# zuds-survey/zuds-pipeline

Hardware: AMD Instinct MI355X
Metric: Mpix/s resample->coadd->subtract, 3072x3072 frames (higher is better)
Workload: dtype f32; 1 GPU; configs[1]+[2]: 32x 3072x3072 TPV frames/GPU, mesh background + weight rescale + Lanczos-3 resample + WEIGHTED coadd (+ AND mask coadd, int16 masks); then 1 science frame/GPU: align ref, hotpants 3x3 regions x 10x10 stamps, r=10, ko=4, subtract; frames_per_gpu=32, size=3072, mask_dtype=int16, combine=WEIGHTED, subtract=True

## Files before the change

include/zudsmi.h:

```cpp
#ifndef ZUDSMI_H
#define ZUDSMI_H

#include <stdint.h>

#ifdef __cplusplus
extern "C" {
#endif

typedef struct zm_ctx zm_ctx;

#define ZM_NPV 40

typedef struct zm_wcs {
    double crpix[2];
    double crval[2];
    double cd[4];
    double pv1[ZM_NPV];
    double pv2[ZM_NPV];
    int32_t naxis[2];
    int32_t flags;
    int32_t pad_;
} zm_wcs;

enum { ZM_RESAMPLE_NEAREST = 0, ZM_RESAMPLE_BILINEAR = 1, ZM_RESAMPLE_LANCZOS3 = 3 };
// ... 42 lines not shown
    const float* img;
    const float* wgt;
    const void* mask;
    zm_wcs wcs;
    double flxscale;
    int32_t mask_type;
    int32_t pad_;
} zm_frame;

typedef struct zm_coadd_params {
    int32_t combine;
    int32_t mask_combine;
    int32_t resample;
    int32_t subtract_back;
    int32_t back_size;
    int32_t back_filtersize;
    int32_t rescale_weights;
    int32_t pad_;
    double clip_sigma;
    double clip_ampfrac;
    double weight_thresh;
} zm_coadd_params;

void zm_coadd_params_default(zm_coadd_params* p);

int zm_coadd(zm_ctx* ctx, int nframes, const zm_frame* frames,
             const zm_wcs* wout, const zm_coadd_params* params, float* out_img,
             float* out_wgt, int32_t* out_mask, float* out_mask_wgt);

typedef struct zm_hp_params {
    double tu, tl, iu, il;
    double r;
    double rss;
    double fin;
    double fi;
    int32_t nsx, nsy;
    int32_t nrx, nry;
    int32_t ko, bgo;
    int32_t nss;
    int32_t normalize;
    double ft;
    double ks;
    int32_t ngauss;
    int32_t deg[4];
    int32_t pad_[3];
    double sigma[4];
    const double* limits_dev;
    double limits_nsigma;
    int32_t* flag_mask_dev;
    int32_t flag_bit;
    int32_t async_info;
} zm_hp_params;

void zm_hp_params_default(zm_hp_params* p);

typedef struct zm_hp_info {
    int32_t nstamps_total, nstamps_used;
    int32_t niter, ncoeff;
    double kernel_sum;
    double chi2;
    int32_t nmasked;
    int32_t status;
    int32_t nunsolved;
    int32_t retries;
} zm_hp_info;
#define ZM_HP_UNSOLVED 1
#define ZM_HP_TIMEOUT 2
#define ZM_HP_PENDING 4

int zm_subtract(zm_ctx* ctx, const float* sci, const float* sci_rms,
                const float* ref, const float* ref_rms, const uint8_t* bpm,
                int nx, int ny, const zm_hp_params* params, float* out_diff,
                float* out_rms, zm_hp_info* out_info);

int zm_median_mad(zm_ctx* ctx, const float* img, const int32_t* mask, int64_t n,
                  double* out_median, double* out_mad_sigma);
int zm_median_mad_dev(zm_ctx* ctx, const float* img, const int32_t* mask,
                      int64_t n, double* out_median, double* out_mad_sigma);
int zm_median_mad2_dev(zm_ctx* ctx, const float* img_a, const int32_t* mask_a,
                       const float* img_b, const int32_t* mask_b, int64_t n,
                       double* out4);
int zm_median_mad2_async_dev(zm_ctx* ctx, const float* img_a, const int32_t* mask_a,
                             const float* img_b, const int32_t* mask_b, int64_t n, double* out6_dev);

int zm_aperture_photometry(zm_ctx* ctx, const float* img, const float* rms,
                           const int32_t* mask, int nx, int ny, int npos,
                           const double* x, const double* y, double radius,
                           double* out_flux, double* out_err, int32_t* out_flags);
int zm_aperture_photometry_dev(zm_ctx* ctx, const float* img, const float* rms,
                               const int32_t* mask, int nx, int ny, int npos,
                               const double* x, const double* y, double radius,
                               double* out_flux, double* out_err, int32_t* out_flags);

typedef struct zm_dframe {
    const float* img;
    const float* wgt;
    const void* mask;
    zm_wcs wcs;
    double flxscale;
    int32_t mask_type;
    int32_t pad_;
} zm_dframe;

int zm_coadd_dev(zm_ctx* ctx, int nframes, const zm_dframe* frames,
                 const zm_wcs* wout, const zm_coadd_params* params,
                 int partial, float* out_img, float* out_wgt, int32_t* out_mask,
                 float* out_mask_wgt);
int zm_coadd_finalize_dev(zm_ctx* ctx, float* s1_to_img, const float* s0,
                          int64_t npix);
int zm_mask_accum_dev(zm_ctx* ctx, int32_t* acc, const int32_t* m, int64_t npix,
                      int kind, int first);
int zm_mask_finalize_dev(zm_ctx* ctx, int32_t* acc, float* cov, int64_t npix);
#define ZM_COMM_ID_BYTES 128
typedef struct zm_comm zm_comm;
int zm_comm_unique_id(void* id128);
int zm_comm_init(zm_ctx* ctx, int nranks, int rank, const void* id128, zm_comm** out);
int zm_comm_destroy(zm_comm* comm);
int zm_coadd_reduce_dev(zm_ctx* ctx, zm_comm* comm, float* s1s0, int64_t npix);
int zm_mask_reduce_dev(zm_ctx* ctx, zm_comm* comm, int32_t* mask, int nx, int ny, int kind,
                       float* cov);
#define ZM_COMM_MAX_RANKS 64
typedef struct {
    int32_t world, rank;
    int64_t band_px;
    int64_t my_px;
    int64_t send_off[ZM_COMM_MAX_RANKS];
    int64_t send_cnt[ZM_COMM_MAX_RANKS];
    int64_t recv_off[ZM_COMM_MAX_RANKS];
    int64_t recv_cnt[ZM_COMM_MAX_RANKS];
    int64_t gather_off[ZM_COMM_MAX_RANKS];
} zm_mask_plan;
int zm_comm_band_bounds(int nrows, int world, int32_t* bounds);
int zm_comm_mask_plan(int nx, int ny, int world, int rank, zm_mask_plan* plan);
int zm_resample_stack_dev(zm_ctx* ctx, int nframes, const zm_dframe* frames,
                          const zm_wcs* wout, const zm_coadd_params* params,
                          float* stack, int32_t* out_mask_partial);
int zm_combine_stack_dev(zm_ctx* ctx, int nframes, const float* stack,
                         int64_t frame_stride_px, int64_t npix,
                         const zm_coadd_params* params, float* out_img,
                         float* out_wgt);
int zm_subtract_dev(zm_ctx* ctx, const float* sci, const float* sci_rms,
                    const float* ref, const float* ref_rms, const uint8_t* bpm,
                    int nx, int ny, const zm_hp_params* params, float* out_diff,
                    float* out_rms, zm_hp_info* out_info_host);
int zm_subtract_info(zm_ctx* ctx, zm_hp_info* out_info);
#define ZM_SUB_BATCH_MAX 64
typedef struct zm_sub_job {
    const float* sci;
    const float* sci_rms;
    const float* ref;
    const float* ref_rms;
    const uint8_t* bpm;
    const zm_hp_params* params;
    float* out_diff;
    float* out_rms;
} zm_sub_job;
int zm_subtract_batch_dev(zm_ctx* ctx, int njobs, const zm_sub_job* jobs, int nx, int ny,
                          zm_hp_info* out_info_host);
int zm_subtract_batch(zm_ctx* ctx, int njobs, const zm_sub_job* jobs, int nx, int ny,
                      zm_hp_info* out_info);
int zm_background_dev(zm_ctx* ctx, const float* img, const float* wgt, int nx,
                      int ny, int mesh, int filtersize, float* out_bkg,
                      float* out_rms, float* out_sub, double* out_stats_host);
int zm_resample_dev(zm_ctx* ctx, const float* img, const float* wgt,
                    const int32_t* mask, const zm_wcs* win, const zm_wcs* wout,
                    int kernel, double fscale, float* out_img, float* out_wgt,
                    int32_t* out_mask);

int zm_align_pair_dev(zm_ctx* ctx, const float* img_a, const float* img_b, const int32_t* mask,
                      const zm_wcs* win, const zm_wcs* wout, int kernel, double fscale_a, double fscale_b,
                      float* out_a, float* out_b, int32_t* out_mask);
int zm_resample_i16(zm_ctx* ctx, const float* img, const float* wgt,
                    const int16_t* mask, const zm_wcs* win, const zm_wcs* wout,
                    int kernel, double fscale, float* out_img, float* out_wgt,
                    int32_t* out_mask);
int zm_resample_i16_dev(zm_ctx* ctx, const float* img, const float* wgt,
                        const int16_t* mask, const zm_wcs* win, const zm_wcs* wout,
                        int kernel, double fscale, float* out_img, float* out_wgt,
                        int32_t* out_mask);
int zm_mask_widen_dev(zm_ctx* ctx, const int16_t* in, int64_t n, int32_t* out);

int zm_rms_from_weight_dev(zm_ctx* ctx, const float* wgt, const uint8_t* bad,
                           int64_t n, float big_rms, float* out);
int zm_weight_from_rms_dev(zm_ctx* ctx, const float* rms, const uint8_t* bad,
                           const float* img, float satur, int64_t n, float* out);
int zm_false_weight_dev(zm_ctx* ctx, const void* mask, int mask_type, int32_t badsum, int border,
                        int nx, int ny, float* out_wgt, uint8_t* out_bpm);
int zm_mask_bad_dev(zm_ctx* ctx, const int32_t* a, const int32_t* b,
                    int32_t badsum, int64_t n, int32_t* out_or, uint8_t* out_bpm);
int zm_mask_flag_dev(zm_ctx* ctx, int32_t* mask, const float* img, float value,
                     int32_t bit, int64_t n);
int zm_add_scalar_dev(zm_ctx* ctx, float* img, float v, int64_t n);
int zm_copy_probe_dev(zm_ctx* ctx, const void* src, void* dst, int64_t nbytes);

int zm_find_stars(zm_ctx* ctx, const float* img, const uint8_t* bad, int nx, int ny,
                  float thresh_lo, float thresh_hi, int isolation, int border,
                  int max_out, int* out_x, int* out_y, float* out_peak, int* out_n);
int zm_star_fwhm(zm_ctx* ctx, const float* img, int nx, int ny, int nstar,
                 const int* x, const int* y, int half, double* out_fwhm,
                 double* out_cx, double* out_cy);
int zm_negpix_test(zm_ctx* ctx, const float* img, int nx, int ny, int npos,
                   const double* x, const double* y, double median, double sigma,
                   int32_t* out_bad);
int zm_find_stars_dev(zm_ctx* ctx, const float* img, const uint8_t* bad, int nx, int ny,
                      float thresh_lo, float thresh_hi, int isolation, int border,
                      int max_out, int* out_x, int* out_y, float* out_peak, int* out_n);
int zm_star_fwhm_dev(zm_ctx* ctx, const float* img, int nx, int ny, int nstar,
                     const int* x, const int* y, int half, double* out_fwhm,
                     double* out_cx, double* out_cy);
int zm_candidate_cuts_dev(zm_ctx* ctx, const float* d_img, const float* d_rms, const int32_t* d_mask,
                          int32_t bad_bits, int nx, int ny, int npos, const double* x, const double* y,
                          double* out_bpmcut, double* out_rmscut, int32_t* out_negpix, double* out_stats);

typedef struct zm_extract_params {
    float detect_thresh;
    float satur_level;
    int32_t detect_minarea;
    int32_t filter;
    double aper_radius;
} zm_extract_params;
void zm_extract_params_default(zm_extract_params* p);

#define ZM_EXTRACT_CHAIN 1

typedef struct zm_object {
    int32_t number;
    int32_t npix;
    int32_t xmin, xmax, ymin, ymax;
    int32_t flags;
    int32_t flags_weight;
    int32_t imaflags_iso;
    int32_t first;
    int32_t nthresh;
    int32_t pad_;
    double x_image, y_image;
    double x2, y2, xy;
    double a_image, b_image, theta_image, elongation;
    double fwhm_image;
    double flux_iso, flux_max;
    double peak;
    double flux_aper, fluxerr_aper;
    double x_world, y_world;
} zm_object;

int zm_extract_dev(zm_ctx* ctx, const float* img, const float* sigma, const uint8_t* bad,
                   const int32_t* flag, int nx, int ny, const zm_wcs* wcs,
                   const zm_extract_params* params, int max_objects, zm_object* out_rows,
                   int32_t* segm_dev, float* filtered_dev, int* out_nwritten, int* out_nfound,
                   int* out_status);
int zm_extract(zm_ctx* ctx, const float* img, const float* sigma, const uint8_t* bad,
               const int32_t* flag, int nx, int ny, const zm_wcs* wcs,
               const zm_extract_params* params, int max_objects, zm_object* out_rows,
               int32_t* out_segm, float* out_filtered, int* out_nwritten, int* out_nfound,
               int* out_status);

typedef struct zm_measure_params {
    double kron_fact;
    double kron_min_radius;
    int32_t filter;
    int32_t pad_;
} zm_measure_params;
void zm_measure_params_default(zm_measure_params* p);

#define ZM_AUTO_SKIPPED 1
#define ZM_AUTO_OFFFRAME 2
#define ZM_AUTO_MINRADIUS 4
#define ZM_WIN_FALLBACK 1
#define ZM_WIN_NOTCONVERGED 2

typedef struct zm_object_ext {
    int32_t number;
    int32_t npix_auto;
// ... 60 lines not shown
```

zuds-pipeline_amd/_lib.py:

```python
import ctypes as C
from pathlib import Path

import numpy as np

HERE = Path(__file__).resolve().parent
LIBPATH = HERE / 'lib' / 'libzudsmi.so'

NPV = 40

RESAMPLE = {'NEAREST': 0, 'BILINEAR': 1, 'LANCZOS3': 3}
COMBINE = {'WEIGHTED': 0, 'MEDIAN': 1, 'CLIPPED': 2, 'AVERAGE': 3}
MASKCOMB = {'AND': 0, 'OR': 1}


class ZMError(RuntimeError):
    """A libzudsmi call returned non-zero (message from zm_last_error)."""


class zm_wcs(C.Structure):
    _fields_ = [('crpix', C.c_double * 2), ('crval', C.c_double * 2),
                ('cd', C.c_double * 4), ('pv1', C.c_double * NPV),
                ('pv2', C.c_double * NPV), ('naxis', C.c_int32 * 2),
                ('flags', C.c_int32), ('pad_', C.c_int32)]

# ... 51 lines not shown


COMM_MAX_RANKS = 64


class zm_mask_plan(C.Structure):
    _fields_ = [('world', C.c_int32), ('rank', C.c_int32), ('band_px', C.c_int64), ('my_px', C.c_int64),
                ('send_off', C.c_int64 * COMM_MAX_RANKS), ('send_cnt', C.c_int64 * COMM_MAX_RANKS),
                ('recv_off', C.c_int64 * COMM_MAX_RANKS), ('recv_cnt', C.c_int64 * COMM_MAX_RANKS),
                ('gather_off', C.c_int64 * COMM_MAX_RANKS)]


class zm_extract_params(C.Structure):
    _fields_ = [('detect_thresh', C.c_float), ('satur_level', C.c_float),
                ('detect_minarea', C.c_int32), ('filter', C.c_int32),
                ('aper_radius', C.c_double)]


class zm_object(C.Structure):
    _fields_ = [('number', C.c_int32), ('npix', C.c_int32), ('xmin', C.c_int32), ('xmax', C.c_int32),
                ('ymin', C.c_int32), ('ymax', C.c_int32), ('flags', C.c_int32), ('flags_weight', C.c_int32),
                ('imaflags_iso', C.c_int32), ('first', C.c_int32), ('nthresh', C.c_int32), ('pad_', C.c_int32),
                ('x_image', C.c_double), ('y_image', C.c_double), ('x2', C.c_double), ('y2', C.c_double),
                ('xy', C.c_double), ('a_image', C.c_double), ('b_image', C.c_double), ('theta_image', C.c_double),
                ('elongation', C.c_double), ('fwhm_image', C.c_double), ('flux_iso', C.c_double),
                ('flux_max', C.c_double), ('peak', C.c_double), ('flux_aper', C.c_double),
                ('fluxerr_aper', C.c_double), ('x_world', C.c_double), ('y_world', C.c_double)]


class zm_measure_params(C.Structure):
    _fields_ = [('kron_fact', C.c_double), ('kron_min_radius', C.c_double), ('filter', C.c_int32), ('pad_', C.c_int32)]


class zm_object_ext(C.Structure):
    _fields_ = [('number', C.c_int32), ('npix_auto', C.c_int32), ('nskip_auto', C.c_int32), ('flags_auto', C.c_int32),
                ('flags_win', C.c_int32), ('niter_win', C.c_int32),
                ('kron_radius', C.c_double), ('flux_auto', C.c_double), ('fluxerr_auto', C.c_double),
                ('mag_auto', C.c_double), ('magerr_auto', C.c_double), ('sigma_win', C.c_double),
                ('xwin_image', C.c_double), ('ywin_image', C.c_double),
                ('x2win', C.c_double), ('y2win', C.c_double), ('xywin', C.c_double),
                ('errx2win', C.c_double), ('erry2win', C.c_double), ('errxywin', C.c_double),
                ('awin_image', C.c_double), ('bwin_image', C.c_double), ('thetawin_image', C.c_double),
                ('errawin_image', C.c_double), ('errbwin_image', C.c_double), ('errthetawin_image', C.c_double),
                ('errx2', C.c_double), ('erry2', C.c_double), ('errxy', C.c_double),
                ('xwin_world', C.c_double), ('ywin_world', C.c_double),
                ('erra_world', C.c_double), ('errb_world', C.c_double), ('errtheta_world', C.c_double)]


class zm_stamp_plane(C.Structure):
    _fields_ = [('img', C.c_void_p), ('wcs', zm_wcs), ('fscale', C.c_double),
                ('on_grid', C.c_int32), ('pad_', C.c_int32)]


STAMP_MAX, STAMP_PLANES_MAX = 256, 8
STAMP_NOT_FINITE, STAMP_NO_OVERLAP = 1, 2
EXTRACT_CHAIN = 1
HP_UNSOLVED, HP_TIMEOUT, HP_PENDING = 1, 2, 4


_P = C.c_void_p
_SIGS = {
    'zm_ctx_create': (C.c_int, [C.c_int, C.POINTER(_P)]),
    'zm_ctx_destroy': (C.c_int, [_P]),
    'zm_ctx_set_stream': (C.c_int, [_P, _P]),
    'zm_ctx_synchronize': (C.c_int, [_P]),
    'zm_ctx_create_on_stream': (C.c_int, [C.c_int, _P, C.POINTER(C.c_void_p)]),
    'zm_ctx_set_share': (C.c_int, [_P, C.c_int]),
    'zm_ctx_query': (C.c_int, [_P, C.c_char_p, C.POINTER(C.c_int64)]),
    'zm_ctx_set_conventions': (C.c_int, [_P, C.c_int, C.c_int]),
    'zm_last_error': (C.c_char_p, []),
    'zm_version': (C.c_char_p, []),
    'zm_autogrid': (C.c_int, [C.c_int, C.POINTER(zm_wcs), C.POINTER(zm_wcs)]),
    'zm_wcs_pix2sky': (C.c_int, [C.POINTER(zm_wcs), C.c_int, _P, _P, _P, _P]),
    'zm_wcs_sky2pix': (C.c_int, [C.POINTER(zm_wcs), C.c_int, _P, _P, _P, _P]),
    'zm_wcs_map': (C.c_int, [C.POINTER(zm_wcs), C.POINTER(zm_wcs), C.c_int,
                             _P, _P, _P, _P]),
    'zm_flux_scale': (C.c_int, [C.POINTER(zm_wcs), C.POINTER(zm_wcs),
                                C.c_double, C.POINTER(C.c_double)]),
    'zm_resample': (C.c_int, [_P, _P, _P, _P, C.POINTER(zm_wcs),
                              C.POINTER(zm_wcs), C.c_int, C.c_double,
                              _P, _P, _P]),
    'zm_align_pair_dev': (C.c_int, [_P, _P, _P, _P, C.POINTER(zm_wcs), C.POINTER(zm_wcs), C.c_int, C.c_double,
                                    C.c_double, _P, _P, _P]),
    'zm_resample_dev': (C.c_int, [_P, _P, _P, _P, C.POINTER(zm_wcs),
                                  C.POINTER(zm_wcs), C.c_int, C.c_double,
                                  _P, _P, _P]),
    'zm_resample_i16': (C.c_int, [_P, _P, _P, _P, C.POINTER(zm_wcs),
                                  C.POINTER(zm_wcs), C.c_int, C.c_double,
                                  _P, _P, _P]),
    'zm_resample_i16_dev': (C.c_int, [_P, _P, _P, _P, C.POINTER(zm_wcs),
                                      C.POINTER(zm_wcs), C.c_int, C.c_double,
                                      _P, _P, _P]),
    'zm_mask_widen_dev': (C.c_int, [_P, _P, C.c_int64, _P]),
    'zm_coadd_params_default': (None, [C.POINTER(zm_coadd_params)]),
    'zm_coadd': (C.c_int, [_P, C.c_int, C.POINTER(zm_frame), C.POINTER(zm_wcs),
                           C.POINTER(zm_coadd_params), _P, _P, _P, _P]),
    'zm_coadd_dev': (C.c_int, [_P, C.c_int, C.POINTER(zm_frame),
                               C.POINTER(zm_wcs), C.POINTER(zm_coadd_params),
                               C.c_int, _P, _P, _P, _P]),
    'zm_coadd_finalize_dev': (C.c_int, [_P, _P, _P, C.c_int64]),
    'zm_resample_stack_dev': (C.c_int, [_P, C.c_int, C.POINTER(zm_frame),
                                        C.POINTER(zm_wcs),
                                        C.POINTER(zm_coadd_params), _P, _P]),
    'zm_combine_stack_dev': (C.c_int, [_P, C.c_int, _P, C.c_int64, C.c_int64,
                                       C.POINTER(zm_coadd_params), _P, _P]),
    'zm_background': (C.c_int, [_P, _P, _P, C.c_int, C.c_int, C.c_int, C.c_int,
                                _P, _P, _P, _P]),
    'zm_background_dev': (C.c_int, [_P, _P, _P, C.c_int, C.c_int, C.c_int,
                                    C.c_int, _P, _P, _P, _P]),
    'zm_hp_params_default': (None, [C.POINTER(zm_hp_params)]),
    'zm_subtract': (C.c_int, [_P, _P, _P, _P, _P, _P, C.c_int, C.c_int,
                              C.POINTER(zm_hp_params), _P, _P,
                              C.POINTER(zm_hp_info)]),
    'zm_subtract_dev': (C.c_int, [_P, _P, _P, _P, _P, _P, C.c_int, C.c_int,
                                  C.POINTER(zm_hp_params), _P, _P,
                                  C.POINTER(zm_hp_info)]),
    'zm_subtract_info': (C.c_int, [_P, C.POINTER(zm_hp_info)]),
    'zm_subtract_batch_dev': (C.c_int, [_P, C.c_int, C.POINTER(zm_sub_job), C.c_int, C.c_int,
                                        C.POINTER(zm_hp_info)]),
    'zm_subtract_batch': (C.c_int, [_P, C.c_int, C.POINTER(zm_sub_job), C.c_int, C.c_int,
                                    C.POINTER(zm_hp_info)]),
    'zm_median_mad': (C.c_int, [_P, _P, _P, C.c_int64, C.POINTER(C.c_double),
                                C.POINTER(C.c_double)]),
    'zm_median_mad_dev': (C.c_int, [_P, _P, _P, C.c_int64, C.POINTER(C.c_double),
                                    C.POINTER(C.c_double)]),
    'zm_find_stars': (C.c_int, [_P, _P, _P, C.c_int, C.c_int, C.c_float, C.c_float, C.c_int, C.c_int,
                                C.c_int, _P, _P, _P, C.POINTER(C.c_int)]),
    'zm_star_fwhm': (C.c_int, [_P, _P, C.c_int, C.c_int, C.c_int, _P, _P, C.c_int, _P, _P, _P]),
    'zm_find_stars_dev': (C.c_int, [_P, _P, _P, C.c_int, C.c_int, C.c_float, C.c_float, C.c_int, C.c_int,
                                    C.c_int, _P, _P, _P, C.POINTER(C.c_int)]),
    'zm_star_fwhm_dev': (C.c_int, [_P, _P, C.c_int, C.c_int, C.c_int, _P, _P, C.c_int, _P, _P, _P]),
    'zm_negpix_test': (C.c_int, [_P, _P, C.c_int, C.c_int, C.c_int, _P, _P, C.c_double, C.c_double, _P]),
    'zm_candidate_cuts_dev': (C.c_int, [_P, _P, _P, _P, C.c_int32, C.c_int, C.c_int, C.c_int, _P, _P, _P, _P, _P, _P]),
    'zm_fits_decode_dev': (C.c_int, [_P, _P, C.c_int, C.c_double, C.c_double, C.c_int64, C.c_int, _P]),
    'zm_fits_encode_dev': (C.c_int, [_P, _P, C.c_int, C.c_int64, _P]),
    'zm_mask_accum_dev': (C.c_int, [_P, _P, _P, C.c_int64, C.c_int, C.c_int]),
    'zm_mask_finalize_dev': (C.c_int, [_P, _P, _P, C.c_int64]),
    'zm_comm_unique_id': (C.c_int, [_P]),
    'zm_comm_init': (C.c_int, [_P, C.c_int, C.c_int, _P, C.POINTER(C.c_void_p)]),
    'zm_comm_destroy': (C.c_int, [_P]),
    'zm_coadd_reduce_dev': (C.c_int, [_P, _P, _P, C.c_int64]),
    'zm_mask_reduce_dev': (C.c_int, [_P, _P, _P, C.c_int, C.c_int, C.c_int, _P]),
    'zm_comm_band_bounds': (C.c_int, [C.c_int, C.c_int, _P]),
    'zm_comm_mask_plan': (C.c_int, [C.c_int, C.c_int, C.c_int, C.c_int, C.POINTER(zm_mask_plan)]),
    'zm_median_mad2_dev': (C.c_int, [_P, _P, _P, _P, _P, C.c_int64, C.POINTER(C.c_double)]),
    'zm_median_mad2_async_dev': (C.c_int, [_P, _P, _P, _P, _P, C.c_int64, _P]),
    'zm_rms_from_weight_dev': (C.c_int, [_P, _P, _P, C.c_int64, C.c_float, _P]),
    'zm_weight_from_rms_dev': (C.c_int, [_P, _P, _P, _P, C.c_float, C.c_int64, _P]),
    'zm_false_weight_dev': (C.c_int, [_P, _P, C.c_int, C.c_int32, C.c_int, C.c_int, C.c_int, _P, _P]),
    'zm_mask_bad_dev': (C.c_int, [_P, _P, _P, C.c_int32, C.c_int64, _P, _P]),
    'zm_mask_flag_dev': (C.c_int, [_P, _P, _P, C.c_float, C.c_int32, C.c_int64]),
    'zm_add_scalar_dev': (C.c_int, [_P, _P, C.c_float, C.c_int64]),
    'zm_copy_probe_dev': (C.c_int, [_P, _P, _P, C.c_int64]),
    'zm_aperture_photometry': (C.c_int, [_P, _P, _P, _P, C.c_int, C.c_int, C.c_int, _P, _P,
                                         C.c_double, _P, _P, _P]),
    'zm_aperture_photometry_dev': (C.c_int, [_P, _P, _P, _P, C.c_int, C.c_int, C.c_int, _P, _P,
                                             C.c_double, _P, _P, _P]),
    'zm_extract_params_default': (None, [C.POINTER(zm_extract_params)]),
    'zm_extract_dev': (C.c_int, [_P, _P, _P, _P, _P, C.c_int, C.c_int, C.POINTER(zm_wcs), C.POINTER(zm_extract_params),
                                 C.c_int, _P, _P, _P, C.POINTER(C.c_int), C.POINTER(C.c_int), C.POINTER(C.c_int)]),
    'zm_extract': (C.c_int, [_P, _P, _P, _P, _P, C.c_int, C.c_int, C.POINTER(zm_wcs), C.POINTER(zm_extract_params),
                             C.c_int, _P, _P, _P, C.POINTER(C.c_int), C.POINTER(C.c_int), C.POINTER(C.c_int)]),
    'zm_measure_params_default': (None, [C.POINTER(zm_measure_params)]),
    'zm_extract_measure_dev': (C.c_int, [_P, _P, _P, _P, _P, C.c_int, C.c_int, C.POINTER(zm_wcs),
                                         C.POINTER(zm_measure_params), C.c_int, _P, _P]),
    'zm_extract_measure': (C.c_int, [_P, _P, _P, _P, _P, C.c_int, C.c_int, C.POINTER(zm_wcs),
                                     C.POINTER(zm_measure_params), C.c_int, _P, _P]),
    'zm_stamp_origin': (C.c_int, [C.POINTER(zm_wcs), C.c_int, _P, _P, C.c_int, _P, _P, _P]),
    'zm_stamps_dev': (C.c_int, [_P, C.c_int, C.POINTER(zm_stamp_plane), C.POINTER(zm_wcs), C.c_int, C.c_int, _P, _P,
                                C.c_int, _P, _P]),
    'zm_stamps': (C.c_int, [_P, C.c_int, C.POINTER(zm_stamp_plane), C.POINTER(zm_wcs), C.c_int, C.c_int, _P, _P,
                            C.c_int, _P, _P]),
    'zm_timing_enable': (C.c_int, [_P, C.c_int]),
    'zm_timing_filter': (C.c_int, [_P, C.c_char_p]),
    'zm_timing_reset': (C.c_int, [_P]),
    'zm_timing_read': (C.c_int, [_P, C.c_char_p, C.POINTER(C.c_double),
                                 C.POINTER(C.c_int64)]),
    'zm_debug_lanczos3': (None, [C.c_float, _P]),
}

_lib = None


def exported_symbols():
    return [k for k in _SIGS if k != 'zm_debug_lanczos3']


def _one_hip_runtime():
    import importlib.util
    import os
    import sys
    if 'torch' in sys.modules:
        return
    try:
        spec = importlib.util.find_spec('torch')
    except (ImportError, ValueError):
        spec = None
    if not spec or not spec.origin:
        return
    if not os.environ.get('ZM_NO_TORCH'):
        try:
            import torch
            return
        except Exception:
            pass
    d = os.path.join(os.path.dirname(spec.origin), 'lib')
    for name in ('libhsa-runtime64.so', 'libamdhip64.so'):
        p = os.path.join(d, name)
        if os.path.exists(p):
            try:
                C.CDLL(p, mode=C.RTLD_GLOBAL)
            except OSError:
                return


def lib():
    global _lib
    if _lib is not None:
        return _lib
    _one_hip_runtime()
    if not LIBPATH.exists():
        raise ZMError(f'{LIBPATH} is missing: run __graft_entry__.build() '
                      f'(python zuds-pipeline_amd/build.py). There is no CPU '
                      f'fallback for this path.')
    L = C.CDLL(str(LIBPATH))
    for name, (res, args) in _SIGS.items():
        try:
            fn = getattr(L, name)
        except AttributeError:
            raise ZMError(f'{LIBPATH} does not export {name}; rebuild it '
                          f'(python zuds-pipeline_amd/build.py --force)')
        fn.restype = res
        fn.argtypes = args
# ... 54 lines not shown
```

zuds-pipeline_amd/csrc/api_coadd.hip:

```cpp
#include <algorithm>
#include <cmath>
#include <cstdlib>

#include "zm_internal.h"
#include "wcs_math.h"

extern "C" void zm_coadd_params_default(zm_coadd_params* p) {
    if (!p) return;
    memset(p, 0, sizeof(*p));
    p->combine = ZM_COMBINE_CLIPPED;
    p->mask_combine = ZM_MASK_AND;
    p->resample = ZM_RESAMPLE_LANCZOS3;
    p->subtract_back = 1;
    p->back_size = 128;
    p->back_filtersize = 3;
    p->rescale_weights = 1;
    p->clip_sigma = 4.0;
    p->clip_ampfrac = 0.3;
    p->weight_thresh = 1e-30;
}

static int check_wcs(const zm_wcs* w, const char* what) {
    ZM_CHECK(w != nullptr, "%s: WCS is NULL", what);
    ZM_CHECK(w->naxis[0] > 0 && w->naxis[1] > 0, "%s: NAXIS must be positive (got %d x %d)", what,
// ... 372 lines not shown
                                    const zm_coadd_params* params, float* out_img,
                                    float* out_wgt) {
    ZM_CHECK(ctx && stack && params && out_img && out_wgt, "zm_combine_stack_dev: null argument");
    ZM_HIP(hipSetDevice(ctx->device));
    return zm_launch_combine(ctx, nframes, (const float2*)stack, frame_stride_px, npix,
                             params->combine, (float)params->clip_sigma,
                             (float)params->clip_ampfrac, out_img, out_wgt, 0);
}

extern "C" int zm_coadd_dev(zm_ctx* ctx, int nframes, const zm_dframe* frames,
                            const zm_wcs* wout, const zm_coadd_params* params, int partial,
                            float* out_img, float* out_wgt, int32_t* out_mask,
                            float* out_mask_wgt) {
    ZM_CHECK(ctx && frames && wout && params && out_img && out_wgt, "zm_coadd_dev: null argument");
    ZM_CHECK(nframes >= 1, "zm_coadd_dev: need at least one frame");
    ZM_HIP(hipSetDevice(ctx->device));
    ZM_TRY(check_wcs(wout, "output grid"));
    const int64_t opix = (int64_t)wout->naxis[0] * wout->naxis[1];
    if (fused_ok(ctx, params))
        return coadd_fused(ctx, nframes, frames, wout, params, partial, out_img, out_wgt, out_mask, out_mask_wgt);
    float2* stack = nullptr;
    ZM_TRY(ctx->get("stack", sizeof(float2) * (size_t)opix * nframes, (void**)&stack));
    ZM_TRY(resample_frames(ctx, nframes, frames, wout, params, stack, out_mask, -1,
                           params->mask_combine));
    ZM_TRY(zm_launch_combine(ctx, nframes, stack, opix, opix, params->combine,
                             (float)params->clip_sigma, (float)params->clip_ampfrac, out_img,
                             out_wgt, partial));
    if (out_mask && !partial) ZM_TRY(zm_launch_mask_finalize(ctx, out_mask, out_mask_wgt, opix));
    return 0;
}

extern "C" int zm_mask_accum_dev(zm_ctx* ctx, int32_t* acc, const int32_t* m, int64_t npix, int kind,
                                 int first) {
    ZM_CHECK(ctx && acc && m, "zm_mask_accum_dev: null argument");
    ZM_CHECK(kind == ZM_MASK_AND || kind == ZM_MASK_OR, "zm_mask_accum_dev: unknown combine %d", kind);
    ZM_HIP(hipSetDevice(ctx->device));
    return zm_launch_mask_accum(ctx, acc, m, npix, kind, first);
}

extern "C" int zm_mask_finalize_dev(zm_ctx* ctx, int32_t* acc, float* cov, int64_t npix) {
    ZM_CHECK(ctx && acc, "zm_mask_finalize_dev: null argument");
    ZM_HIP(hipSetDevice(ctx->device));
    return zm_launch_mask_finalize(ctx, acc, cov, npix);
}

extern "C" int zm_resample_dev(zm_ctx* ctx, const float* img, const float* wgt,
                               const int32_t* mask, const zm_wcs* win, const zm_wcs* wout,
                               int kernel, double fscale, float* out_img, float* out_wgt,
                               int32_t* out_mask) {
    ZM_CHECK(ctx && win && wout, "zm_resample_dev: null argument");
    ZM_CHECK(img || mask, "zm_resample_dev: need an image or a mask");
    ZM_CHECK(!img || (out_img && out_wgt), "zm_resample_dev: out_img/out_wgt required");
    ZM_CHECK(!mask || out_mask, "zm_resample_dev: out_mask required");
    ZM_HIP(hipSetDevice(ctx->device));
    ZM_TRY(check_wcs(win, "input frame"));
    ZM_TRY(check_wcs(wout, "output grid"));
    ZM_CHECK(kernel == ZM_RESAMPLE_LANCZOS3 || kernel == ZM_RESAMPLE_BILINEAR ||
             kernel == ZM_RESAMPLE_NEAREST, "zm_resample_dev: unknown RESAMPLING_TYPE %d", kernel);
    const int onx = wout->naxis[0], ony = wout->naxis[1];
    const int nx = win->naxis[0], ny = win->naxis[1];
    const int64_t opix = (int64_t)onx * ony;
    const int lnx = (onx - 1) / ZM_LATTICE_STEP + 2, lny = (ony - 1) / ZM_LATTICE_STEP + 2;
    zm_map_params mp_host;
    zm_make_map(wout, win, &mp_host);
    int lds = std::min(plan_lds(&mp_host, onx, ony, ntaps_of(kernel)), 8000);
    double2* lat = nullptr;
    ZM_TRY(ctx->get("lattice", sizeof(double2) * (size_t)lnx * lny, (void**)&lat));
    ZM_TRY(zm_launch_lattice(ctx, &mp_host, lnx, lny, lat));
    if (img) {
        const int spitch = (nx + 1) & ~1;
        float2 *src = nullptr, *dst = nullptr;
        ZM_TRY(ctx->get("prep", sizeof(float2) * (size_t)spitch * ny, (void**)&src));
        ZM_TRY(ctx->get("stack", sizeof(float2) * (size_t)opix, (void**)&dst));
        ZM_TRY(zm_launch_prep(ctx, img, wgt, nx, ny, nullptr, 0, 0, 0, nullptr, 1e-30f, src, spitch));
        ZM_TRY(zm_launch_resample(ctx, src, nx, ny, spitch, lat, lnx, lny, kernel, (float)fscale,
                                  dst, onx, ony, lds, mask, out_mask, mask ? 1 : 0, 0, 1, out_img, out_wgt));
    } else if (mask) {
        ZM_TRY(zm_launch_resample_mask(ctx, mask, nx, ny, lat, lnx, lny, kernel, out_mask, onx,
                                       ony, 0));
    }
    return 0;
}

extern "C" int zm_align_pair_dev(zm_ctx* ctx, const float* img_a, const float* img_b, const int32_t* mask,
                                 const zm_wcs* win, const zm_wcs* wout, int kernel, double fscale_a, double fscale_b,
                                 float* out_a, float* out_b, int32_t* out_mask) {
    ZM_CHECK(ctx && img_a && img_b && win && wout && out_a && out_b, "zm_align_pair_dev: null argument");
    ZM_CHECK(!mask || out_mask, "zm_align_pair_dev: out_mask required");
    ZM_CHECK(kernel == ZM_RESAMPLE_LANCZOS3 || kernel == ZM_RESAMPLE_BILINEAR, "zm_align_pair_dev: LANCZOS3 or BILINEAR (got %d)", kernel);
    ZM_CHECK(fscale_b != 0.0, "zm_align_pair_dev: fscale_b must not be 0");
    ZM_CHECK(ctx->edge == ZM_EDGE_ZERO && ctx->mask_resample == ZM_MASKRES_OR, "zm_align_pair_dev: default conventions only");
    ZM_HIP(hipSetDevice(ctx->device));
    ZM_TRY(check_wcs(win, "input frame"));
    ZM_TRY(check_wcs(wout, "output grid"));
    const int onx = wout->naxis[0], ony = wout->naxis[1];
    const int nx = win->naxis[0], ny = win->naxis[1];
    const int lnx = (onx - 1) / ZM_LATTICE_STEP + 2, lny = (ony - 1) / ZM_LATTICE_STEP + 2;
    zm_map_params mp_host;
    zm_make_map(wout, win, &mp_host);
    const int lds = std::min(plan_lds(&mp_host, onx, ony, ntaps_of(kernel)), 8000);
    double2* lat = nullptr;
    ZM_TRY(ctx->get("lattice", sizeof(double2) * (size_t)lnx * lny, (void**)&lat));
    ZM_TRY(zm_launch_lattice(ctx, &mp_host, lnx, lny, lat));
    const int spitch = (nx + 1) & ~1;
    float2* src = nullptr;
    ZM_TRY(ctx->get("prep", sizeof(float2) * (size_t)spitch * ny, (void**)&src));
    ZM_TRY(zm_launch_prep_pair(ctx, img_a, img_b, nx, ny, src, spitch));
    return zm_launch_resample(ctx, src, nx, ny, spitch, lat, lnx, lny, kernel, (float)fscale_a, nullptr, onx, ony, lds,
                              mask, out_mask, mask ? 1 : 0, 0, 1, out_a, out_b, (float)fscale_b);
}

extern "C" int zm_resample_i16_dev(zm_ctx* ctx, const float* img, const float* wgt, const int16_t* mask,
                                   const zm_wcs* win, const zm_wcs* wout, int kernel, double fscale,
                                   float* out_img, float* out_wgt, int32_t* out_mask) {
    ZM_CHECK(ctx && win && wout, "zm_resample_i16_dev: null argument");
    ZM_HIP(hipSetDevice(ctx->device));
    int32_t* w = nullptr;
    if (mask) {
        ZM_TRY(check_wcs(win, "input frame"));
        const int64_t n = (int64_t)win->naxis[0] * win->naxis[1];
        ZM_TRY(ctx->get("mask_widen", sizeof(int32_t) * (size_t)n, (void**)&w));
        ZM_TRY(zm_launch_mask_widen(ctx, mask, n, w));
    }
    return zm_resample_dev(ctx, img, wgt, w, win, wout, kernel, fscale, out_img, out_wgt, out_mask);
}

static int resample_host(zm_ctx* ctx, const float* img, const float* wgt, const void* mask, int mask_type,
                         const zm_wcs* win, const zm_wcs* wout, int kernel, double fscale,
                         float* out_img, float* out_wgt, int32_t* out_mask);
extern "C" int zm_resample(zm_ctx* ctx, const float* img, const float* wgt, const int32_t* mask,
                           const zm_wcs* win, const zm_wcs* wout, int kernel, double fscale,
                           float* out_img, float* out_wgt, int32_t* out_mask) {
    return resample_host(ctx, img, wgt, mask, ZM_MASKTYPE_I32, win, wout, kernel, fscale, out_img, out_wgt, out_mask);
}
extern "C" int zm_resample_i16(zm_ctx* ctx, const float* img, const float* wgt, const int16_t* mask,
                               const zm_wcs* win, const zm_wcs* wout, int kernel, double fscale,
                               float* out_img, float* out_wgt, int32_t* out_mask) {
    return resample_host(ctx, img, wgt, mask, ZM_MASKTYPE_I16, win, wout, kernel, fscale, out_img, out_wgt, out_mask);
}
static int resample_host(zm_ctx* ctx, const float* img, const float* wgt, const void* mask, int mask_type,
                         const zm_wcs* win, const zm_wcs* wout, int kernel, double fscale,
                         float* out_img, float* out_wgt, int32_t* out_mask) {
    ZM_CHECK(ctx && win && wout, "zm_resample: null argument");
    ZM_HIP(hipSetDevice(ctx->device));
    ZM_TRY(check_wcs(win, "input frame"));
    ZM_TRY(check_wcs(wout, "output grid"));
    const size_t ipix = (size_t)win->naxis[0] * win->naxis[1];
    const size_t opix = (size_t)wout->naxis[0] * wout->naxis[1];
    const size_t mb = mask_type == ZM_MASKTYPE_I16 ? 2 : 4;
    float *d_img = nullptr, *d_wgt = nullptr, *d_oimg = nullptr, *d_owgt = nullptr;
    void* d_mask = nullptr;
    int32_t* d_omask = nullptr;
    if (img) {
        ZM_TRY(ctx->get("h_img", ipix * 4, (void**)&d_img));
        ZM_HIP(hipMemcpyAsync(d_img, img, ipix * 4, hipMemcpyHostToDevice, ctx->stream));
        if (wgt) {
            ZM_TRY(ctx->get("h_wgt", ipix * 4, (void**)&d_wgt));
            ZM_HIP(hipMemcpyAsync(d_wgt, wgt, ipix * 4, hipMemcpyHostToDevice, ctx->stream));
        }
        ZM_TRY(ctx->get("h_oimg", opix * 4, (void**)&d_oimg));
        ZM_TRY(ctx->get("h_owgt", opix * 4, (void**)&d_owgt));
    }
    if (mask) {
        ZM_TRY(ctx->get("h_mask", ipix * mb, &d_mask));
        ZM_HIP(hipMemcpyAsync(d_mask, mask, ipix * mb, hipMemcpyHostToDevice, ctx->stream));
        ZM_TRY(ctx->get("h_omask", opix * 4, (void**)&d_omask));
    }
    if (mask_type == ZM_MASKTYPE_I16)
        ZM_TRY(zm_resample_i16_dev(ctx, d_img, d_wgt, (const int16_t*)d_mask, win, wout, kernel, fscale, d_oimg,
                                   d_owgt, d_omask));
    else
        ZM_TRY(zm_resample_dev(ctx, d_img, d_wgt, (const int32_t*)d_mask, win, wout, kernel, fscale, d_oimg, d_owgt,
                               d_omask));
    if (img) {
        ZM_HIP(hipMemcpyAsync(out_img, d_oimg, opix * 4, hipMemcpyDeviceToHost, ctx->stream));
        ZM_HIP(hipMemcpyAsync(out_wgt, d_owgt, opix * 4, hipMemcpyDeviceToHost, ctx->stream));
    }
    if (mask)
        ZM_HIP(hipMemcpyAsync(out_mask, d_omask, opix * 4, hipMemcpyDeviceToHost, ctx->stream));
    ZM_HIP(hipStreamSynchronize(ctx->stream));
    return 0;
}

extern "C" int zm_coadd(zm_ctx* ctx, int nframes, const zm_frame* frames, const zm_wcs* wout,
                        const zm_coadd_params* params, float* out_img, float* out_wgt,
                        int32_t* out_mask, float* out_mask_wgt) {
    ZM_CHECK(ctx && frames && wout && params && out_img && out_wgt, "zm_coadd: null argument");
    ZM_CHECK(nframes >= 1, "zm_coadd: need at least one frame");
    ZM_HIP(hipSetDevice(ctx->device));
    ZM_TRY(check_wcs(wout, "output grid"));
    std::vector<zm_dframe> df(nframes);
    size_t total = 0;
// ... 55 lines not shown
```

zuds-pipeline_amd/csrc/api_subtract.hip:

```cpp
#include "select_dev.h"

#define RS_BINS 2048

struct rs_state {
    uint32_t prefix[2];
    uint32_t pmask;
    uint32_t pad_;
    unsigned long long k[2];
    unsigned long long count;
    float centre;
    float median;
    double out[3];
};

__global__ void k_rsel_init(rs_state* __restrict__ st, unsigned int* __restrict__ hist) {
    const int im = blockIdx.x;
    for (int k = threadIdx.x; k < 2 * RS_BINS; k += blockDim.x) hist[(size_t)im * 2 * RS_BINS + k] = 0;
    if (threadIdx.x == 0) {
        rs_state z;
        memset(&z, 0, sizeof(z));
        st[im] = z;
    }
}

__global__ __launch_bounds__(1024) void k_rsel_hist(const rs_batch B, int vec_ok, int mode, int shift,
                                                    int nbins, const rs_state* __restrict__ st,
                                                    unsigned int* __restrict__ hist,
                                                    unsigned long long* __restrict__ vbits, int vmode) {
    __shared__ unsigned int lh[2][RS_BINS];
    const int im = blockIdx.y;
    const float* __restrict__ img = B.im[im].img;
    const int32_t* __restrict__ mask = B.im[im].mask;
    const rs_state S = st[im];
    const bool two = S.prefix[1] != S.prefix[0];
    for (int k = threadIdx.x; k < nbins; k += blockDim.x) { lh[0][k] = 0; lh[1][k] = 0; }
    __syncthreads();
    int cur = -1;
    unsigned int run = 0;
    auto put = [&](float v, int32_t m) {
        if (m != 0 || !(v == v)) return;
        if (mode == 1) v = fabsf(v - S.centre);
        const uint32_t key = f2key(v);
        const uint32_t hi = key & S.pmask;
        const int b = (int)((key >> shift) & (uint32_t)(nbins - 1));
        if (hi == S.prefix[0]) {
            if (b == cur) { ++run; }
            else {
                if (run) atomicAdd(&lh[0][cur], run);
                cur = b;
                run = 1;
            }
        } else if (two && hi == S.prefix[1]) {
            atomicAdd(&lh[1][b], 1u);
        }
    };
    const int64_t n = B.n;
    const int64_t n4 = vec_ok ? n / 4 : 0;
    const int64_t stride = (int64_t)gridDim.x * blockDim.x;
    unsigned long long* vb = vbits ? vbits + (size_t)im * (size_t)((n4 + 63) / 64) * 4 : nullptr;
    const int lane = threadIdx.x & 63;
    const int64_t n4w = vb ? ((n4 + 63) / 64) * 64 : n4;
    for (int64_t q = (int64_t)blockIdx.x * blockDim.x + threadIdx.x; q < n4w; q += stride) {
        const bool in = q < n4;
        float4 v = make_float4(0.f, 0.f, 0.f, 0.f);
        if (in) v = reinterpret_cast<const float4*>(img)[q];
        int4 m = make_int4(0, 0, 0, 0);
        if (vb && vmode == 2) {
            const unsigned long long* w = vb + (q >> 6) * 4;
            m.x = ((w[0] >> lane) & 1ull) ? 0 : 1;
            m.y = ((w[1] >> lane) & 1ull) ? 0 : 1;
            m.z = ((w[2] >> lane) & 1ull) ? 0 : 1;
            m.w = ((w[3] >> lane) & 1ull) ? 0 : 1;
        } else {
            if (mask && in) m = reinterpret_cast<const int4*>(mask)[q];
            if (!in) m = make_int4(1, 1, 1, 1);
            if (vb) {
                const unsigned long long b0 = __ballot(m.x == 0 && v.x == v.x), b1 = __ballot(m.y == 0 && v.y == v.y);
                const unsigned long long b2 = __ballot(m.z == 0 && v.z == v.z), b3 = __ballot(m.w == 0 && v.w == v.w);
                if (lane == 0) {
                    unsigned long long* w = vb + (q >> 6) * 4;
                    w[0] = b0; w[1] = b1; w[2] = b2; w[3] = b3;
                }
            }
        }
        put(v.x, m.x); put(v.y, m.y); put(v.z, m.z); put(v.w, m.w);
    }
    for (int64_t p = 4 * n4 + (int64_t)blockIdx.x * blockDim.x + threadIdx.x; p < n; p += stride)
        put(img[p], mask ? mask[p] : 0);
    if (run) atomicAdd(&lh[0][cur], run);
    __syncthreads();
    unsigned int* h = hist + (size_t)im * 2 * RS_BINS;
    for (int k = threadIdx.x; k < nbins; k += blockDim.x) {
        if (lh[0][k]) atomicAdd(&h[k], lh[0][k]);
        if (two && lh[1][k]) atomicAdd(&h[RS_BINS + k], lh[1][k]);
    }
}

__global__ __launch_bounds__(256) void k_rsel_scan(int pass, int mode, int shift, int nbins,
                                                   rs_state* __restrict__ st,
                                                   unsigned int* __restrict__ hist) {
    __shared__ unsigned long long wtot[4];
    __shared__ rs_state S;
    const int im = blockIdx.x, tid = threadIdx.x;
    const int lane = tid & 63, wave = tid >> 6;
    unsigned int* h = hist + (size_t)im * 2 * RS_BINS;
    if (tid == 0) S = st[im];
    __syncthreads();
    const bool two = S.prefix[1] != S.prefix[0];
    const int per = nbins / 256;
    for (int t = 0; t < 2; ++t) {
        const unsigned int* ht = h + (two && t == 1 ? RS_BINS : 0);
        unsigned int hl[8];
        unsigned long long loc = 0;
#pragma unroll
        for (int j = 0; j < 8; ++j) {
            hl[j] = j < per ? ht[tid * per + j] : 0u;
            loc += hl[j];
        }
        unsigned long long inc = loc;
#pragma unroll
        for (int o = 1; o < 64; o <<= 1) {
            const unsigned long long up = __shfl_up(inc, o);
            if (lane >= o) inc += up;
        }
        if (lane == 63) wtot[wave] = inc;
        __syncthreads();
        unsigned long long off = 0, tot = 0;
#pragma unroll
        for (int w = 0; w < 4; ++w) {
            if (w < wave) off += wtot[w];
            tot += wtot[w];
        }
        const unsigned long long excl = off + inc - loc;
        if (pass == 0 && t == 0 && tid == 0) {
            S.count = tot;
            S.k[0] = tot ? (tot - 1) / 2 : 0;
            S.k[1] = tot / 2 < tot ? tot / 2 : (tot ? tot - 1 : 0);
        }
        __syncthreads();
        const unsigned long long k = S.k[t];
        __syncthreads();
        const bool hit = (tid == 255) ? (k >= excl) : (k >= excl && k < excl + loc);
        if (hit) {
            unsigned long long runsum = excl;
            int jsel = per - 1;
            bool found = false;
#pragma unroll
            for (int j = 0; j < 7; ++j)
                if (!found && j < per - 1) {
                    if (runsum + hl[j] > k) { jsel = j; found = true; }
                    else runsum += hl[j];
                }
            S.k[t] = k - runsum;
            S.prefix[t] |= (uint32_t)(tid * per + jsel) << shift;
        }
        __syncthreads();
    }
    for (int k = tid; k < 2 * RS_BINS; k += 256) h[k] = 0;
    if (tid == 0) {
        S.pmask |= (uint32_t)(nbins - 1) << shift;
        if (pass == 2) {
            const float a = key2f_dev(S.prefix[0]), b = key2f_dev(S.prefix[1]);
            const float med = S.count ? 0.5f * (a + b) : 0.f;
            if (mode == 0) {
                S.median = med;
                S.centre = med;
                S.out[0] = med;
                S.out[2] = (double)S.count;
            } else {
                S.out[1] = 1.4826 * (double)med;
            }
// ... 4 lines not shown
        st[im] = S;
    }
}

__global__ void k_rsel_out(const rs_state* __restrict__ st, int nimg, double* __restrict__ out) {
    const int t = threadIdx.x;
    if (t < 3 * nimg) out[t] = st[t / 3].out[t % 3];
}

static int median_mad_batch(zm_ctx* ctx, int nimg, const rs_image* ims, int64_t n, double* out3, double* out_dev = nullptr) {
    ZM_CHECK(nimg >= 1 && nimg <= ZM_RS_MAXIMG, "median_mad_batch: 1..%d images", ZM_RS_MAXIMG);
    rs_state* d_st = nullptr;
    unsigned int* d_hist = nullptr;
    ZM_TRY(ctx->get("rs_state", sizeof(rs_state) * ZM_RS_MAXIMG, (void**)&d_st));
    ZM_TRY(ctx->get("rs_hist", sizeof(unsigned int) * 2 * RS_BINS * ZM_RS_MAXIMG, (void**)&d_hist));
    unsigned long long* d_vbits = nullptr;
    rs_batch B;
    memset(&B, 0, sizeof(B));
    B.n = n;
    int vec_ok = 1;
    for (int i = 0; i < nimg; ++i) {
        B.im[i] = ims[i];
        if (((uintptr_t)ims[i].img & 15) || ((uintptr_t)ims[i].mask & 15)) vec_ok = 0;
    }
    static const int rs_threads = ZM_DEVENV("ZM_RS_THREADS") ? atoi(ZM_DEVENV("ZM_RS_THREADS")) : 1024;
    static const int rs_grid = ZM_DEVENV("ZM_RS_GRID") ? atoi(ZM_DEVENV("ZM_RS_GRID")) : 256;
    int grid = (int)std::min<int64_t>((n / 4 + rs_threads - 1) / rs_threads, rs_grid);
    if (grid < 1) grid = 1;
    bool any_mask = false;
    for (int i = 0; i < nimg; ++i) any_mask = any_mask || ims[i].mask != nullptr;
    static const bool bits_off = ZM_DEVENV("ZM_RS_BITS") && ZM_DEVENV("ZM_RS_BITS")[0] == '0';
    if (vec_ok && any_mask && n >= 4096 && !bits_off)
        ZM_TRY(ctx->get("rs_vbits", sizeof(unsigned long long) * 4 * (size_t)((n / 4 + 63) / 64) * ZM_RS_MAXIMG, (void**)&d_vbits));
    const int shifts[3] = {21, 10, 0}, bits[3] = {11, 11, 10};
    hipStream_t s = ctx->stream;
    static const bool classic = ZM_DEVENV("ZM_RS_CLASSIC") && ZM_DEVENV("ZM_RS_CLASSIC")[0] == '1';
    if (vec_ok && n >= ZM_RS2_MIN_N && !classic) {
        double* d_out = out_dev;
        if (!d_out) ZM_TRY(ctx->get("rs2_out", sizeof(double) * 3 * ZM_RS_MAXIMG, (void**)&d_out));
        {
            zm_scope_timer t(ctx, "median_mad");
            ZM_TRY(zm_rs2_median_mad(ctx, nimg, B, d_vbits, d_out));
        }
        if (!out3) return 0;
        double* h_out = nullptr;
        ZM_TRY(ctx->get_pinned("rs2_out_h", sizeof(double) * 3 * ZM_RS_MAXIMG, (void**)&h_out));
        ZM_HIP(hipMemcpyAsync(h_out, d_out, sizeof(double) * 3 * nimg, hipMemcpyDeviceToHost, s));
        ZM_HIP(hipStreamSynchronize(s));
        for (int k = 0; k < 3 * nimg; ++k) out3[k] = h_out[k];
        return 0;
    }
    {
        zm_scope_timer t(ctx, "median_mad");
        hipLaunchKernelGGL(k_rsel_init, dim3(nimg), dim3(256), 0, s, d_st, d_hist);
        for (int mode = 0; mode < 2; ++mode)
            for (int pass = 0; pass < 3; ++pass) {
                const int nb = 1 << bits[pass];
                hipLaunchKernelGGL(k_rsel_hist, dim3(grid, nimg), dim3(rs_threads), 0, s, B, vec_ok, mode,
                                   shifts[pass], nb, d_st, d_hist, d_vbits, (mode == 0 && pass == 0) ? 1 : 2);
                hipLaunchKernelGGL(k_rsel_scan, dim3(nimg), dim3(256), 0, s, pass, mode, shifts[pass], nb,
                                   d_st, d_hist);
            }
        ZM_HIP(hipGetLastError());
    }
    if (!out3) {
        hipLaunchKernelGGL(k_rsel_out, dim3(1), dim3(64), 0, s, d_st, nimg, out_dev);
        ZM_HIP(hipGetLastError());
        return 0;
    }
    rs_state* h_st = nullptr;
    ZM_TRY(ctx->get_pinned("rs_state_h", sizeof(rs_state) * ZM_RS_MAXIMG, (void**)&h_st));
    ZM_HIP(hipMemcpyAsync(h_st, d_st, sizeof(rs_state) * nimg, hipMemcpyDeviceToHost, s));
    ZM_HIP(hipStreamSynchronize(s));
    for (int i = 0; i < nimg; ++i)
        for (int k = 0; k < 3; ++k) out3[3 * i + k] = h_st[i].out[k];
    return 0;
}

extern "C" int zm_median_mad_dev(zm_ctx* ctx, const float* img, const int32_t* mask, int64_t n,
                                 double* out_median, double* out_mad_sigma) {
    ZM_CHECK(ctx && img && out_median && out_mad_sigma, "zm_median_mad_dev: null argument");
    ZM_CHECK(n > 0, "zm_median_mad_dev: empty image");
    ZM_HIP(hipSetDevice(ctx->device));
    rs_image im = {img, mask};
    double o[3];
    ZM_TRY(median_mad_batch(ctx, 1, &im, n, o));
    ZM_CHECK(o[2] > 0, "zm_median_mad: every pixel is masked");
    *out_median = o[0];
    *out_mad_sigma = o[1];
    return 0;
}

extern "C" int zm_median_mad2_dev(zm_ctx* ctx, const float* img_a, const int32_t* mask_a,
                                  const float* img_b, const int32_t* mask_b, int64_t n,
                                  double* out4) {
    ZM_CHECK(ctx && img_a && img_b && out4, "zm_median_mad2_dev: null argument");
    ZM_CHECK(n > 0, "zm_median_mad2_dev: empty image");
    ZM_HIP(hipSetDevice(ctx->device));
    rs_image im[2] = {{img_a, mask_a}, {img_b, mask_b}};
    double o[6];
    ZM_TRY(median_mad_batch(ctx, 2, im, n, o));
    ZM_CHECK(o[2] > 0 && o[5] > 0, "zm_median_mad2: every pixel is masked");
    out4[0] = o[0]; out4[1] = o[1]; out4[2] = o[3]; out4[3] = o[4];
    return 0;
}

extern "C" int zm_median_mad2_async_dev(zm_ctx* ctx, const float* img_a, const int32_t* mask_a,
                                        const float* img_b, const int32_t* mask_b, int64_t n,
                                        double* out6_dev) {
    ZM_CHECK(ctx && img_a && img_b && out6_dev, "zm_median_mad2_async_dev: null argument");
    ZM_CHECK(n > 0, "zm_median_mad2_async_dev: empty image");
    ZM_HIP(hipSetDevice(ctx->device));
    rs_image im[2] = {{img_a, mask_a}, {img_b, mask_b}};
    return median_mad_batch(ctx, 2, im, n, nullptr, out6_dev);
}

extern "C" int zm_median_mad(zm_ctx* ctx, const float* img, const int32_t* mask, int64_t n,
                             double* out_median, double* out_mad_sigma) {
    ZM_CHECK(ctx && img && out_median && out_mad_sigma, "zm_median_mad: null argument");
    ZM_CHECK(n > 0, "zm_median_mad: empty image");
    ZM_HIP(hipSetDevice(ctx->device));
    float* d_img = nullptr;
    int32_t* d_mask = nullptr;
    ZM_TRY(ctx->get("h_img", (size_t)n * 4, (void**)&d_img));
    ZM_HIP(hipMemcpyAsync(d_img, img, (size_t)n * 4, hipMemcpyHostToDevice, ctx->stream));
    if (mask) {
        ZM_TRY(ctx->get("h_mask", (size_t)n * 4, (void**)&d_mask));
        ZM_HIP(hipMemcpyAsync(d_mask, mask, (size_t)n * 4, hipMemcpyHostToDevice, ctx->stream));
    }
    return zm_median_mad_dev(ctx, d_img, d_mask, n, out_median, out_mad_sigma);
}
```

zuds-pipeline_amd/csrc/elementwise.hip:

```cpp
#include <algorithm>
#include "zm_internal.h"

#define EW_GRID(n) dim3((unsigned)(((n) + 255) / 256)), dim3(256), 0, ctx->stream

__global__ void k_rms_from_weight(const float* __restrict__ w, const uint8_t* __restrict__ bad,
                                  int64_t n, float big, float* __restrict__ out) {
    int64_t p = (int64_t)blockIdx.x * blockDim.x + threadIdx.x;
    if (p >= n) return;
    float ww = w[p];
    bool b = !(ww > 0.f) || (bad && bad[p]);
    out[p] = b ? big : 1.0f / sqrtf(ww);
}

__global__ void k_weight_from_rms(const float* __restrict__ rms, const uint8_t* __restrict__ bad,
                                  const float* __restrict__ img, float satur, int64_t n,
                                  float* __restrict__ out) {
    int64_t p = (int64_t)blockIdx.x * blockDim.x + threadIdx.x;
    if (p >= n) return;
    float r = rms[p];
    bool b = (bad && bad[p]) || (img && satur > 0.f && img[p] >= satur);
    out[p] = b ? 0.f : 1.0f / (r * r);
}

template <typename T>
__global__ void k_false_weight(const T* __restrict__ m, int32_t badsum, int border, int nx, int ny,
                               float* __restrict__ out_w, uint8_t* __restrict__ out_bpm) {
    const int64_t p = (int64_t)blockIdx.x * blockDim.x + threadIdx.x;
    if (p >= (int64_t)nx * ny) return;
    const int y = (int)(p / nx), x = (int)(p - (int64_t)y * nx);
    const bool bad = ((int32_t)m[p] & badsum) != 0;
    const bool edge = x < border || x >= nx - border || y < border || y >= ny - border;
    if (out_w) out_w[p] = (bad || edge) ? 0.f : 1.f;
    if (out_bpm) out_bpm[p] = bad ? 1 : 0;
}

extern "C" int zm_false_weight_dev(zm_ctx* ctx, const void* mask, int mask_type, int32_t badsum, int border,
                                   int nx, int ny, float* out_wgt, uint8_t* out_bpm) {
    ZM_CHECK(ctx && mask && nx > 0 && ny > 0 && border >= 0 && (out_wgt || out_bpm), "zm_false_weight_dev: bad argument");
    ZM_CHECK(mask_type == ZM_MASKTYPE_I32 || mask_type == ZM_MASKTYPE_I16, "zm_false_weight_dev: unknown mask_type %d", mask_type);
    ZM_HIP(hipSetDevice(ctx->device));
    const int64_t n = (int64_t)nx * ny;
    if (mask_type == ZM_MASKTYPE_I16)
        hipLaunchKernelGGL(k_false_weight<int16_t>, EW_GRID(n), (const int16_t*)mask, badsum, border, nx, ny, out_wgt, out_bpm);
    else
        hipLaunchKernelGGL(k_false_weight<int32_t>, EW_GRID(n), (const int32_t*)mask, badsum, border, nx, ny, out_wgt, out_bpm);
    ZM_HIP(hipGetLastError());
    return 0;
}

__global__ void k_mask_bad(const int32_t* __restrict__ a, const int32_t* __restrict__ b,
                           int32_t badsum, int64_t n, int32_t* __restrict__ out_or,
                           uint8_t* __restrict__ out_bpm) {
    int64_t p = (int64_t)blockIdx.x * blockDim.x + threadIdx.x;
    if (p >= n) return;
    int32_t m = a[p] | (b ? b[p] : 0);
    if (out_or) out_or[p] = m;
    if (out_bpm) out_bpm[p] = (m & badsum) != 0;
}

__global__ void k_mask_flag(int32_t* __restrict__ mask, const float* __restrict__ img, float value,
                            int32_t bit, int64_t n) {
    int64_t p = (int64_t)blockIdx.x * blockDim.x + threadIdx.x;
    if (p >= n) return;
    if (img[p] == value) mask[p] |= bit;
}

__global__ void k_add_scalar(float* __restrict__ img, float v, int64_t n) {
    int64_t p = (int64_t)blockIdx.x * blockDim.x + threadIdx.x;
    if (p >= n) return;
    img[p] += v;
}

extern "C" int zm_rms_from_weight_dev(zm_ctx* ctx, const float* wgt, const uint8_t* bad, int64_t n,
                                      float big_rms, float* out) {
    ZM_CHECK(ctx && wgt && out && n > 0, "zm_rms_from_weight_dev: bad argument");
    ZM_HIP(hipSetDevice(ctx->device));
    hipLaunchKernelGGL(k_rms_from_weight, EW_GRID(n), wgt, bad, n, big_rms, out);
    ZM_HIP(hipGetLastError());
    return 0;
}

extern "C" int zm_weight_from_rms_dev(zm_ctx* ctx, const float* rms, const uint8_t* bad,
                                      const float* img, float satur, int64_t n, float* out) {
    ZM_CHECK(ctx && rms && out && n > 0, "zm_weight_from_rms_dev: bad argument");
    ZM_HIP(hipSetDevice(ctx->device));
    hipLaunchKernelGGL(k_weight_from_rms, EW_GRID(n), rms, bad, img, satur, n, out);
    ZM_HIP(hipGetLastError());
    return 0;
}

extern "C" int zm_mask_bad_dev(zm_ctx* ctx, const int32_t* a, const int32_t* b, int32_t badsum,
                               int64_t n, int32_t* out_or, uint8_t* out_bpm) {
    ZM_CHECK(ctx && a && n > 0 && (out_or || out_bpm), "zm_mask_bad_dev: bad argument");
    ZM_HIP(hipSetDevice(ctx->device));
    hipLaunchKernelGGL(k_mask_bad, EW_GRID(n), a, b, badsum, n, out_or, out_bpm);
    ZM_HIP(hipGetLastError());
    return 0;
}

extern "C" int zm_mask_flag_dev(zm_ctx* ctx, int32_t* mask, const float* img, float value,
                                int32_t bit, int64_t n) {
    ZM_CHECK(ctx && mask && img && n > 0, "zm_mask_flag_dev: bad argument");
    ZM_HIP(hipSetDevice(ctx->device));
    hipLaunchKernelGGL(k_mask_flag, EW_GRID(n), mask, img, value, bit, n);
    ZM_HIP(hipGetLastError());
    return 0;
}

template <int U, bool NTL>
__global__ __launch_bounds__(256) void k_copy4(const float4* __restrict__ src, float4* __restrict__ dst, int64_t n4) {
    typedef float v4f __attribute__((ext_vector_type(4)));
    const v4f* s = reinterpret_cast<const v4f*>(src);
    v4f* d = reinterpret_cast<v4f*>(dst);
    const int64_t nslab = n4 / (256 * U);
    for (int64_t b = blockIdx.x; b < nslab; b += gridDim.x) {
        const int64_t o = b * (256 * U) + threadIdx.x;
        v4f r[U];
#pragma unroll
        for (int u = 0; u < U; ++u) r[u] = NTL ? __builtin_nontemporal_load(s + o + 256 * u) : s[o + 256 * u];
#pragma unroll
        for (int u = 0; u < U; ++u) __builtin_nontemporal_store(r[u], d + o + 256 * u);
    }
    for (int64_t p = nslab * (256 * U) + (int64_t)blockIdx.x * blockDim.x + threadIdx.x; p < n4;
         p += (int64_t)gridDim.x * blockDim.x)
        d[p] = s[p];
}

extern "C" int zm_copy_probe_dev(zm_ctx* ctx, const void* src, void* dst, int64_t nbytes) {
    ZM_CHECK(ctx && src && dst && nbytes > 0 && nbytes % 16 == 0 && ((uintptr_t)src & 15) == 0 &&
             ((uintptr_t)dst & 15) == 0, "zm_copy_probe_dev: bad argument");
    ZM_HIP(hipSetDevice(ctx->device));
    int ncu = 256;
    ZM_HIP(hipDeviceGetAttribute(&ncu, hipDeviceAttributeMultiprocessorCount, ctx->device));
    const int64_t n4 = nbytes / 16;
    const unsigned grid = (unsigned)std::min<int64_t>((n4 + 255) / 256, (int64_t)ncu * 8);
    const char* cf = ZM_DEVENV("ZM_COPY_FORM");
    const int u = cf ? atoi(cf) : 4;
    const bool ntl = cf ? strchr(cf, 'n') != nullptr : true;
    if (u == 8 && ntl) hipLaunchKernelGGL((k_copy4<8, true>), dim3(grid), dim3(256), 0, ctx->stream, (const float4*)src, (float4*)dst, n4);
    else if (u == 8) hipLaunchKernelGGL((k_copy4<8, false>), dim3(grid), dim3(256), 0, ctx->stream, (const float4*)src, (float4*)dst, n4);
    else if (ntl) hipLaunchKernelGGL((k_copy4<4, true>), dim3(grid), dim3(256), 0, ctx->stream, (const float4*)src, (float4*)dst, n4);
    else hipLaunchKernelGGL((k_copy4<4, false>), dim3(grid), dim3(256), 0, ctx->stream, (const float4*)src, (float4*)dst, n4);
    ZM_HIP(hipGetLastError());
    return 0;
}

extern "C" int zm_add_scalar_dev(zm_ctx* ctx, float* img, float v, int64_t n) {
    ZM_CHECK(ctx && img && n > 0, "zm_add_scalar_dev: bad argument");
    ZM_HIP(hipSetDevice(ctx->device));
    hipLaunchKernelGGL(k_add_scalar, EW_GRID(n), img, v, n);
    ZM_HIP(hipGetLastError());
    return 0;
}

__global__ __launch_bounds__(256) void k_mask_widen(const int16_t* __restrict__ in, int64_t n, int32_t* __restrict__ out) {
    const int64_t stride = (int64_t)gridDim.x * blockDim.x * 4;
    for (int64_t p = ((int64_t)blockIdx.x * blockDim.x + threadIdx.x) * 4; p < n; p += stride) {
        if (p + 4 <= n && ((uintptr_t)in & 7) == 0 && ((uintptr_t)out & 15) == 0) {
            const short4 v = *reinterpret_cast<const short4*>(in + p);
            *reinterpret_cast<int4*>(out + p) = make_int4(v.x, v.y, v.z, v.w);
        } else {
            for (int64_t q = p; q < n && q < p + 4; ++q) out[q] = in[q];
        }
    }
}

int zm_launch_mask_widen(zm_ctx* ctx, const int16_t* in, int64_t n, int32_t* out) {
    int ncu = 256;
    ZM_HIP(hipDeviceGetAttribute(&ncu, hipDeviceAttributeMultiprocessorCount, ctx->device));
    const unsigned grid = (unsigned)std::max<int64_t>(1, std::min<int64_t>((n / 4 + 255) / 256, (int64_t)ncu * 8));
    hipLaunchKernelGGL(k_mask_widen, dim3(grid), dim3(256), 0, ctx->stream, in, n, out);
    ZM_HIP(hipGetLastError());
    return 0;
}

extern "C" int zm_mask_widen_dev(zm_ctx* ctx, const int16_t* in, int64_t n, int32_t* out) {
    ZM_CHECK(ctx && in && out && n > 0, "zm_mask_widen_dev: bad argument");
    ZM_HIP(hipSetDevice(ctx->device));
// ... 3 lines not shown
```

zuds-pipeline_amd/csrc/hotpants.hip:

```cpp
#include "hp_dev.h"
#include <sched.h>
#include "chol_diag.h"

__global__ void k_hp_valid(const float* __restrict__ sci, const float* __restrict__ ref,
                           const uint8_t* __restrict__ bpm, int64_t n, float il, float iu,
                           float tl, float tu, uint8_t* __restrict__ bad,
                           const double* __restrict__ lim, double nsig) {
    int64_t p = (int64_t)blockIdx.x * blockDim.x + threadIdx.x;
    if (lim) {
        il = (float)(lim[0] - nsig * lim[1]);
        tl = (float)(lim[3] - nsig * lim[4]);
    }
    if (p >= n) return;
    float s = sci[p], t = ref[p];
    bool ok = (s == s) && (t == t) && fabsf(s) < 3e38f && fabsf(t) < 3e38f;
    ok = ok && s >= il && s <= iu && t >= tl && t <= tu;
    if (bpm) ok = ok && bpm[p] == 0;
    bad[p] = ok ? 0 : 1;
}

#define HP_ROWMAX 16384
__global__ __launch_bounds__(256) void k_hp_rowany(const uint8_t* __restrict__ in, int nx, int ny, int hw,
                                                   uint8_t* __restrict__ out) {
    extern __shared__ int ra_pre[];
// ... 70 lines not shown
        int off = inc - v;
        for (int w = 0; w < wave; ++w) off += wtot[w];
        if (tid < 4 * nch) wsum[tid] = off;
    }
    __syncthreads();
    for (int c = 0; c < nch; ++c) {
        const int x = 256 * c + tid;
        if (x < nx) ra_pre[x + 1] += wsum[4 * c + wave];
    }
    __syncthreads();
    for (int x = tid; x < nx; x += 256) {
        const int a1 = max(x - hw1, 0), b1 = min(x + hw1, nx - 1);
        const int a2 = max(x - hw2, 0), b2 = min(x + hw2, nx - 1);
        out1[r0 + x] = (ra_pre[b1 + 1] - ra_pre[a1]) > 0;
        out2[r0 + x] = (ra_pre[b2 + 1] - ra_pre[a2]) > 0;
    }
}

#define HP_COLSTRIP 96
__global__ __launch_bounds__(256) void k_hp_colany(const uint8_t* __restrict__ in, int nx, int ny, int hw,
                                                   int edge, uint8_t* __restrict__ out) {
    const int x = blockIdx.x * blockDim.x + threadIdx.x;
    const int y0 = blockIdx.y * HP_COLSTRIP, y1 = min(y0 + HP_COLSTRIP, ny);
    if (x >= nx) return;
    int cnt = 0;
    for (int j = max(y0 - hw, 0); j <= min(y0 + hw, ny - 1); ++j) cnt += in[(size_t)j * nx + x] ? 1 : 0;
    for (int y = y0; y < y1; ++y) {
        uint8_t v = cnt > 0;
        if (edge && (x < hw || x >= nx - hw || y < hw || y >= ny - hw)) v = 1;
        out[(size_t)y * nx + x] = v;
        const int add = y + 1 + hw, sub = y - hw;
        if (add < ny) cnt += in[(size_t)add * nx + x] ? 1 : 0;
        if (sub >= 0) cnt -= in[(size_t)sub * nx + x] ? 1 : 0;
    }
}

#define HP_COLSTRIP4 32
__global__ __launch_bounds__(256) void k_hp_colany4(const uint8_t* __restrict__ in, int nx, int ny, int hw,
                                                    int edge, uint8_t* __restrict__ out) {
    const int x = (blockIdx.x * blockDim.x + threadIdx.x) * 4;
    const int y0 = blockIdx.y * HP_COLSTRIP4, y1 = min(y0 + HP_COLSTRIP4, ny);
    if (x >= nx) return;
    const unsigned* in4 = reinterpret_cast<const unsigned*>(in + x);
    const size_t pitch = (size_t)nx / 4;
    auto nz = [](unsigned w, int k) -> int { return ((w >> (8 * k)) & 0xffu) ? 1 : 0; };
    int cnt[4] = {0, 0, 0, 0};
    {
        const int j0 = max(y0 - hw, 0), j1 = min(y0 + hw, ny - 1);
        for (int jb = j0; jb <= j1; jb += 8) {
            unsigned w[8];
#pragma unroll
            for (int u = 0; u < 8; ++u) w[u] = (jb + u <= j1) ? in4[(size_t)(jb + u) * pitch] : 0u;
#pragma unroll
            for (int u = 0; u < 8; ++u)
#pragma unroll
                for (int k = 0; k < 4; ++k) cnt[k] += nz(w[u], k);
        }
    }
    for (int yb = y0; yb < y1; yb += 8) {
        unsigned wa[8], ws[8];
#pragma unroll
        for (int u = 0; u < 8; ++u) {
            const int add = yb + u + 1 + hw, sub = yb + u - hw;
            wa[u] = (add < ny) ? in4[(size_t)add * pitch] : 0u;
            ws[u] = (sub >= 0) ? in4[(size_t)sub * pitch] : 0u;
        }
#pragma unroll
        for (int u = 0; u < 8; ++u) {
            const int y = yb + u;
            if (y < y1) {
                unsigned o = 0;
#pragma unroll
                for (int k = 0; k < 4; ++k) {
                    unsigned v = cnt[k] > 0;
                    if (edge && (x + k < hw || x + k >= nx - hw || y < hw || y >= ny - hw)) v = 1;
                    o |= v << (8 * k);
                }
                *reinterpret_cast<unsigned*>(out + (size_t)y * nx + x) = o;
            }
#pragma unroll
            for (int k = 0; k < 4; ++k) cnt[k] += nz(wa[u], k) - nz(ws[u], k);
        }
    }
}

__global__ __launch_bounds__(256) void k_hp_cells(const hp_plan P, const float* __restrict__ ref,
                                                  const uint8_t* __restrict__ bad,
                                                  const uint8_t* __restrict__ dirty,
                                                  int2* __restrict__ centres) {
    __shared__ double red[4];
    __shared__ float bval[4];
    __shared__ int bidx[4];
    __shared__ int2 chosen[HP_MAXNSS];
    const int cell = blockIdx.x, tid = threadIdx.x;
    const int r = cell / P.ncellr, c = cell - r * P.ncellr;
    const int sy = c / P.nsx, sx = c - sy * P.nsx;
    const int cw = (P.rx1[r] - P.rx0[r]) / P.nsx, ch = (P.ry1[r] - P.ry0[r]) / P.nsy;
    const int cx0 = P.rx0[r] + sx * cw, cy0 = P.ry0[r] + sy * ch;
    const int n = cw * ch;
    double m = 0.0, s = 0.0;
    for (int pass = 0; pass < 4; ++pass) {
        double s0 = 0, s1 = 0;
        for (int k = tid; k < n; k += 256) {
            int yy = k / cw, xx = k - yy * cw;
            size_t idx = (size_t)(cy0 + yy) * P.nx + cx0 + xx;
            if (bad[idx]) continue;
            double v = ref[idx];
            if (pass == 0 || fabs(v - m) <= 3.0 * s) { s0 += 1.0; s1 += v; }
        }
        s0 = block_sum256(s0, red);
        s1 = block_sum256(s1, red);
        if (s0 < 1.0) break;
        double mn = s1 / s0;
        double s2 = 0;
        for (int k = tid; k < n; k += 256) {
            int yy = k / cw, xx = k - yy * cw;
            size_t idx = (size_t)(cy0 + yy) * P.nx + cx0 + xx;
            if (bad[idx]) continue;
            double v = ref[idx];
            if (pass == 0 || fabs(v - m) <= 3.0 * s) s2 += (v - mn) * (v - mn);
        }
        s2 = block_sum256(s2, red);
        m = mn;
        s = sqrt(s2 / s0);
    }
    const double thr = m + P.ft * s;
    for (int k = 0; k < P.nss; ++k) {
        float best = -__builtin_inff();
        int bi = 0x7fffffff;
        for (int q = tid; q < n; q += 256) {
            int yy = q / cw, xx = q - yy * cw;
            int x = cx0 + xx, y = cy0 + yy;
            size_t idx = (size_t)y * P.nx + x;
            if (dirty[idx]) continue;
            float v = ref[idx];
            if (!((double)v >= thr)) continue;
            bool excl = false;
            for (int e = 0; e < k; ++e)
                excl |= (abs(x - chosen[e].x) <= P.hwss) && (abs(y - chosen[e].y) <= P.hwss);
            if (excl) continue;
            if (v > best || (v == best && q < bi)) { best = v; bi = q; }
        }
#pragma unroll
        for (int o = 32; o >= 1; o >>= 1) {
            float ov = __shfl_xor(best, o);
            int oi = __shfl_xor(bi, o);
            if (ov > best || (ov == best && oi < bi)) { best = ov; bi = oi; }
        }
        __syncthreads();
        if ((tid & 63) == 0) { bval[tid >> 6] = best; bidx[tid >> 6] = bi; }
        __syncthreads();
        if (tid == 0) {
            for (int w = 1; w < 4; ++w)
                if (bval[w] > best || (bval[w] == best && bidx[w] < bi)) { best = bval[w]; bi = bidx[w]; }
            int2 cc = make_int2(-1, -1);
            if (bi != 0x7fffffff) { int yy = bi / cw; cc = make_int2(cx0 + bi - yy * cw, cy0 + yy); }
            chosen[k] = cc;
            centres[cell * P.nss + k] = cc;
        }
        __syncthreads();
        if (chosen[k].x < 0) {
            if (tid == 0)
                for (int e = k + 1; e < P.nss; ++e) centres[cell * P.nss + e] = make_int2(-1, -1);
            break;
        }
    }
// ... 2135 lines not shown
                P->tsub0[nc] = (ee && nc > 0) ? 1 : 0;
                ++nc;
            }
    P->nc = nc;
    for (int f = 0; f < HP_MAXF1; ++f) { P->tf0[f] = 0; P->tfn[f] = 0; }
    for (int n = 0; n < nc; ++n) {
        const int f = P->tfx[n];
        if (P->tfn[f] == 0) P->tf0[f] = n;
        P->tfn[f] += 1;
    }
    int nkp = 0;
    for (int i = 0; i <= P->ko; ++i)
        for (int j = 0; j <= P->ko - i; ++j) { P->kpi[nkp] = i; P->kpj[nkp] = j; ++nkp; }
    P->nkp = nkp;
    int nbg = 0;
    for (int i = 0; i <= P->bgo; ++i)
        for (int j = 0; j <= P->bgo - i; ++j) { P->bpi[nbg] = i; P->bpj[nbg] = j; ++nbg; }
    P->nbg = nbg;
    P->nE = nc + nbg;
    P->nX = P->nE + 1;
    ZM_CHECK(P->nX <= HP_MAXX, "zm_subtract: %d basis + %d background terms exceed the %d-row Gram tile", nc, nbg, HP_MAXX);
    P->nunk = 1 + (nc - 1) * nkp + nbg;
    basis->assign((size_t)nc * step * step, 0.0);
    for (int n = 0; n < nc; ++n) {
        const double* fx = filt->data() + (size_t)P->tfx[n] * step;
        const double* fy = filt->data() + (size_t)P->tfy[n] * step;
        for (int v = 0; v < step; ++v)
            for (int u = 0; u < step; ++u) {
                double k = fy[v] * fx[u] * P->tscale[n];
                if (P->tsub0[n]) k -= (*basis)[(size_t)v * step + u];
                (*basis)[((size_t)n * step + v) * step + u] = k;
            }
    }
    return 0;
}

static __device__ __forceinline__ void hp_solved_body(int nreg, int nunk, const double* __restrict__ stats, const int* __restrict__ fail,
                            const int* __restrict__ tmo, const double* __restrict__ x,
                            unsigned long long* __restrict__ mask, double* __restrict__ x0out = nullptr) {
    unsigned long long m = 0;
    const int reg = threadIdx.x;
    if (reg < nreg) {
        const double x0 = x[(size_t)reg * nunk];
        if (x0out) x0out[reg] = x0;
        const bool ok = stats[2 * reg + 1] >= 1.0 && fail[reg] == 0 && tmo[reg] == 0 && isfinite(x0);
        m = ok ? 1ull << reg : 0ull;
    }
#pragma unroll
    for (int o = 32; o >= 1; o >>= 1) m |= __shfl_xor(m, o);
    if (threadIdx.x == 0) *mask = m;
}
__global__ void k_hp_solved(int nreg, int nunk, const double* __restrict__ stats, const int* __restrict__ fail,
                            const int* __restrict__ tmo, const double* __restrict__ x,
                            unsigned long long* __restrict__ mask, double* __restrict__ x0out = nullptr) {
    hp_solved_body(nreg, nunk, stats, fail, tmo, x, mask, x0out);
}


static int hp_launch_masks(zm_ctx* ctx, const hp_plan& P, const zm_hp_params* hp, const float* sci, const float* ref,
                           const uint8_t* bpm, uint8_t* bad, uint8_t* tmp8, uint8_t* dirty, uint8_t* outbad) {
    const int nx = P.nx, ny = P.ny;
    const int64_t np = (int64_t)nx * ny;
    hipStream_t st = ctx->stream;
    const dim3 b256(256);
    zm_scope_timer t(ctx, "hp_masks");
    ZM_CHECK(nx <= HP_ROWMAX, "zm_subtract: frames wider than %d pixels are not supported", HP_ROWMAX);
    const size_t rsh = sizeof(int) * ((size_t)nx + 1);
    dim3 gc(zm_div_up(nx, 256), zm_div_up(ny, HP_COLSTRIP));
    if (!ctx->hp_rset && rsh > 65536) {
        ZM_HIP(hipFuncSetAttribute((const void*)k_hp_rowany, hipFuncAttributeMaxDynamicSharedMemorySize,
                                   (int)(sizeof(int) * (HP_ROWMAX + 1))));
        ZM_HIP(hipFuncSetAttribute((const void*)k_hp_valid_rows, hipFuncAttributeMaxDynamicSharedMemorySize,
                                   (int)(sizeof(int) * (HP_ROWMAX + 1))));
        ctx->hp_rset = true;
    }
    const bool col4 = (nx % 4 == 0) && (((uintptr_t)tmp8 | (uintptr_t)dirty | (uintptr_t)outbad) & 3) == 0;
    dim3 gc4(zm_div_up(nx / 4, 256), zm_div_up(ny, HP_COLSTRIP4));
    static const bool split = ZM_DEVENV("ZM_HP_MASKS") && !strcmp(ZM_DEVENV("ZM_HP_MASKS"), "split");
    uint8_t* tmp8b = nullptr;
    if (!split) ZM_TRY(ctx->get("hp_tmp8b", np, (void**)&tmp8b));
    if (!split && (((uintptr_t)tmp8b & 3) == 0)) {
        hipLaunchKernelGGL(k_hp_valid_rows, dim3(ny), b256, rsh, st, sci, ref, bpm, nx, ny, (float)P.il, (float)P.iu,
                           (float)P.tl, (float)P.tu, hp->limits_dev, hp->limits_nsigma, P.hw, P.hwk, bad, tmp8, tmp8b);
        if (col4) {
            hipLaunchKernelGGL(k_hp_colany4, gc4, b256, 0, st, tmp8, nx, ny, P.hw, 1, dirty);
            hipLaunchKernelGGL(k_hp_colany4, gc4, b256, 0, st, tmp8b, nx, ny, P.hwk, 1, outbad);
        } else {
            hipLaunchKernelGGL(k_hp_colany, gc, b256, 0, st, tmp8, nx, ny, P.hw, 1, dirty);
            hipLaunchKernelGGL(k_hp_colany, gc, b256, 0, st, tmp8b, nx, ny, P.hwk, 1, outbad);
        }
    } else {
        hipLaunchKernelGGL(k_hp_valid, dim3((unsigned)((np + 255) / 256)), b256, 0, st, sci, ref, bpm, np,
                           (float)P.il, (float)P.iu, (float)P.tl, (float)P.tu, bad, hp->limits_dev, hp->limits_nsigma);
        hipLaunchKernelGGL(k_hp_rowany, dim3(ny), b256, rsh, st, bad, nx, ny, P.hw, tmp8);
        if (col4) hipLaunchKernelGGL(k_hp_colany4, gc4, b256, 0, st, tmp8, nx, ny, P.hw, 1, dirty);
        else hipLaunchKernelGGL(k_hp_colany, gc, b256, 0, st, tmp8, nx, ny, P.hw, 1, dirty);
        hipLaunchKernelGGL(k_hp_rowany, dim3(ny), b256, rsh, st, bad, nx, ny, P.hwk, tmp8);
        if (col4) hipLaunchKernelGGL(k_hp_colany4, gc4, b256, 0, st, tmp8, nx, ny, P.hwk, 1, outbad);
        else hipLaunchKernelGGL(k_hp_colany, gc, b256, 0, st, tmp8, nx, ny, P.hwk, 1, outbad);
    }
    ZM_HIP(hipGetLastError());
    return 0;
}

static int hp_launch_cells(zm_ctx* ctx, const hp_plan& P, const float* ref, const uint8_t* bad, const uint8_t* dirty,
                           int2* centres, int* active, int* need, int* ntotal) {
    hipStream_t st = ctx->stream;
    const dim3 b256(256);
    zm_scope_timer t(ctx, "hp_cells");
    int maxcell = 0;
    for (int r = 0; r < P.nreg; ++r)
        maxcell = std::max(maxcell, ((P.rx1[r] - P.rx0[r]) / P.nsx) * ((P.ry1[r] - P.ry0[r]) / P.nsy));
    const char* cf = getenv("ZM_CELLS_FORM");
    if (maxcell <= HC_THREADS * HC_PX && !(cf && !strcmp(cf, "global")))
        hipLaunchKernelGGL(k_hp_cells_reg, dim3(P.ncell), dim3(HC_THREADS), 0, st, P, ref, bad, dirty, centres);
    else
        hipLaunchKernelGGL(k_hp_cells, dim3(P.ncell), b256, 0, st, P, ref, bad, dirty, centres);
    hipLaunchKernelGGL(k_hp_init_active, dim3(zm_div_up(P.ncell, 256)), b256, 0, st, P, centres, active, need, ntotal);
    ZM_HIP(hipGetLastError());
    return 0;
}

static std::atomic<int> g_hp_fitting[64];
struct hp_fit_guard {
    std::atomic<int>* c;
    int others;
    explicit hp_fit_guard(std::atomic<int>* cc) : c(cc), others(cc->fetch_add(1)) {}
    bool shared() const { return c && (others > 0 || c->load(std::memory_order_relaxed) > 1); }
    void release() { if (c) c->fetch_sub(1); c = nullptr; }
    ~hp_fit_guard() { release(); }
};

#define HP_NIBUF_ (4 * HP_MAXREG + 4)
#define HP_SUMBYTES_ (sizeof(int) * HP_NIBUF_ + sizeof(double) * 3 * HP_MAXREG)
static void hp_fill_info(const char* h_sum, int nreg, int nunk, int rounds, int retries, zm_hp_info* info) {
    const int* h_int = reinterpret_cast<const int*>(h_sum);
    const double* h_stats = reinterpret_cast<const double*>(h_sum + sizeof(int) * HP_NIBUF_);
    const double* h_x0 = h_stats + 2 * HP_MAXREG;
    auto reg_solved = [&](int reg) {
        return h_stats[2 * reg + 1] >= 1.0 && h_int[2 * HP_MAXREG + reg] == 0 &&
               h_int[3 * HP_MAXREG + 4 + reg] == 0 && std::isfinite(h_x0[reg]);
    };
    memset(info, 0, sizeof(*info));
    double ks = 0, chi = 0;
    int nsolved = 0;
    for (int r = 0; r < nreg; ++r) {
        info->nstamps_total += h_int[HP_MAXREG + r];
        info->nstamps_used += (int)h_stats[2 * r + 1];
        if (reg_solved(r)) {
            ks += h_x0[r];
            chi += h_stats[2 * r];
            ++nsolved;
        }
    }
    info->niter = rounds;
    info->ncoeff = nunk;
    info->kernel_sum = nsolved ? ks / nsolved : 0.0;
    info->chi2 = nsolved ? chi / nsolved : 0.0;
    info->nmasked = h_int[3 * HP_MAXREG];
    info->status = (nsolved == nreg ? 0 : ZM_HP_UNSOLVED);
    info->nunsolved = nreg - nsolved;
    info->retries = retries;
}

extern "C" int zm_subtract_dev(zm_ctx* ctx, const float* sci, const float* sci_rms, const float* ref,
                               const float* ref_rms, const uint8_t* bpm, int nx, int ny,
                               const zm_hp_params* hp, float* out_diff, float* out_rms,
// ... 713 lines not shown
```

zuds-pipeline_amd/csrc/resample.hip:

```cpp
#include "resample_dev.h"

__global__ __launch_bounds__(256) void k_lattice(const zm_map_params mp, int lnx, int lny, double2* __restrict__ lat) {
    int gx = blockIdx.x * blockDim.x + threadIdx.x;
    int gy = blockIdx.y * blockDim.y + threadIdx.y;
    if (gx >= lnx || gy >= lny) return;
    double xi, yi;
    zm_map_out_to_in(&mp.wout, &mp.win, mp.rot, 1.0 + (double)gx * LSTEP,
                     1.0 + (double)gy * LSTEP, &xi, &yi);
    lat[(size_t)gy * lnx + gx] = make_double2(xi - 1.0, yi - 1.0);
}

__global__ void k_lattice_batch(const zm_map_params* __restrict__ mps, int lnx, int lny,
                                double2* __restrict__ lat) {
    int gx = blockIdx.x * blockDim.x + threadIdx.x;
    int gy = blockIdx.y * blockDim.y + threadIdx.y;
    if (gx >= lnx || gy >= lny) return;
    const zm_map_params* mp = mps + blockIdx.z;
    double xi, yi;
    zm_map_out_to_in(&mp->wout, &mp->win, mp->rot, 1.0 + (double)gx * LSTEP,
                     1.0 + (double)gy * LSTEP, &xi, &yi);
    lat[((size_t)blockIdx.z * lny + gy) * lnx + gx] = make_double2(xi - 1.0, yi - 1.0);
}

int zm_launch_lattice_batch(zm_ctx* ctx, const zm_map_params* mp_host, int n, int lnx, int lny,
// ... 183 lines not shown
            if (x + 2 < spitch) __builtin_nontemporal_store((zm_nt4){o[1].x, o[1].y, o[1].z, o[1].w}, &d4[1]);
        }
    }
#pragma unroll
    for (int q = 0; q < NLD; ++q) {
        const int e = tid + 256 * q;
        if (e < IH * IW) t0[(e / IW) * IP + (e % IW)] = mm[q];
    }
    __syncthreads();
    for (int e = tid; e < IH * TWB; e += 256) {
        const int r = e / TWB, c = e - r * TWB;
        int32_t o = 0;
#pragma unroll
        for (int k = 0; k < NT; ++k) o |= t0[r * IP + c + k];
        h[e] = o;
    }
    __syncthreads();
    for (int e = tid; e < THB * TWB; e += 256) {
        const int r = e / TWB, c = e - r * TWB;
        const int x = x0 + c, y = y0 + r;
        if (x + NT <= nx && y + NT <= ny) {
            int32_t o = 0;
#pragma unroll
            for (int k = 0; k < NT; ++k) o |= h[(r + k) * TWB + c];
            B[(size_t)y * bpitch + x] = box_entry(o);
        }
    }
}

int zm_launch_prep(zm_ctx* ctx, const float* img, const float* wgt, int nx, int ny,
                   const float* bknodes, int nbx, int nby, int mesh, const float* var_scale_dev,
                   float wthresh, float2* dst, int spitch, const int32_t* mask_for_box, int box_nt,
                   uint16_t* mbox_out, int mbox_pitch) {
    if (mbox_pitch <= 0) mbox_pitch = nx;
    const float invmesh = mesh > 0 ? 1.0f / mesh : 0.f;
    const int vec_ok = (nx % 4 == 0) && (((uintptr_t)img & 15) == 0) && (((uintptr_t)wgt & 15) == 0);
    ctx->box_ready_for = nullptr;
    if (mask_for_box && (box_nt == 6 || box_nt == 2)) {
        uint16_t* mbox = mbox_out;
        if (!mbox) ZM_TRY(ctx->get("mask_box", sizeof(uint16_t) * (size_t)nx * ny, (void**)&mbox));
        dim3 grd(zm_div_up(spitch, 64), zm_div_up(ny, 16), 1);
        zm_scope_timer t(ctx, "prep");
        if (box_nt == 6)
            hipLaunchKernelGGL(k_prep_box<6>, grd, dim3(256), 0, ctx->stream, img, wgt, nx, ny, bknodes, nbx,
                               nby, invmesh, var_scale_dev, wthresh, vec_ok, dst, spitch, mask_for_box, mbox, mbox_pitch);
        else
            hipLaunchKernelGGL(k_prep_box<2>, grd, dim3(256), 0, ctx->stream, img, wgt, nx, ny, bknodes, nbx,
                               nby, invmesh, var_scale_dev, wthresh, vec_ok, dst, spitch, mask_for_box, mbox, mbox_pitch);
        ZM_HIP(hipGetLastError());
        if (!mbox_out) {
            ctx->box_ready_for = mask_for_box;
            ctx->box_ready_nt = box_nt;
        }
        return 0;
    }
    dim3 blk(256, 1, 1), grd(zm_div_up(zm_div_up(spitch, 4), 256), ny, 1);
    zm_scope_timer t(ctx, "prep");
    hipLaunchKernelGGL(k_prep, grd, blk, 0, ctx->stream, img, wgt, nx, ny, bknodes, nbx, nby, invmesh,
                       var_scale_dev, wthresh, vec_ok, dst, spitch);
    ZM_HIP(hipGetLastError());
    return 0;
}

__global__ __launch_bounds__(256) void k_prep_pair(const float* __restrict__ a, const float* __restrict__ b, int nx, int ny,
                                                   float2* __restrict__ dst, int spitch) {
    const int x = blockIdx.x * 256 + threadIdx.x, y = blockIdx.y;
    if (x >= spitch) return;
    const size_t k = (size_t)y * nx + x;
    dst[(size_t)y * spitch + x] = x < nx ? make_float2(a[k], b[k]) : make_float2(0.f, 0.f);
}
int zm_launch_prep_pair(zm_ctx* ctx, const float* a, const float* b, int nx, int ny, float2* dst, int spitch) {
    zm_scope_timer t(ctx, "prep");
    hipLaunchKernelGGL(k_prep_pair, dim3(zm_div_up(spitch, 256), ny), dim3(256), 0, ctx->stream, a, b, nx, ny, dst, spitch);
    ZM_HIP(hipGetLastError());
    return 0;
}

template <int KIND, int MASKOP>
__global__ __launch_bounds__(256, 4) void k_resample(
    const float2* __restrict__ src, int nx, int ny, int spitch, const double2* __restrict__ lat,
    int lnx, int lny, float fscale, float2* __restrict__ dst, int onx, int ony, int lds_cap,
    const int32_t* __restrict__ mask, const uint16_t* __restrict__ mbox, int32_t* __restrict__ macc,
    int mkind, int mfirst, int ntx, int ntiles, const float* __restrict__ taptab,
    float* __restrict__ plane_a, float* __restrict__ plane_b, float pair_scale) {
    extern __shared__ float4 smem4[];
    rs_hdr* HR = reinterpret_cast<rs_hdr*>(smem4);
    constexpr int TABF = (KIND == ZM_RESAMPLE_LANCZOS3) ? LZ_FLOATS : 0;
    const float* ltab = reinterpret_cast<const float*>(smem4) + HDR_FLOATS;
    float2* tile = reinterpret_cast<float2*>(smem4) + (HDR_FLOATS + TABF) / 2;
    constexpr int NT = taps_traits<KIND>::N;
    constexpr int OFF = taps_traits<KIND>::OFF;
    constexpr int CI = -OFF;
    const int tid = threadIdx.x;
    const int G = gridDim.x;
    const float fscale2 = fscale * fscale;
    const float4 fill = make_float4(0.f, ZM_BIGVAR, 0.f, ZM_BIGVAR);

    float4 pf[RS_PF];
    auto prefetch = [&](const rs_hdr* H) {
        if (!H->use_lds) return;
        const int bx0 = H->h.bx0, by0 = H->h.by0, bw2 = H->h.bw >> 1;
        const int n4 = bw2 * H->h.bh;
        const float inv = 1.0f / (float)bw2;
#pragma unroll
        for (int k = 0; k < RS_PF; ++k) {
            const int e = tid + 256 * k;
            pf[k] = fill;
            if (e < n4) {
                const int r = (int)(((float)e + 0.5f) * inv);
                const int c2 = e - r * bw2;
                const int gy = by0 + r, gx = bx0 + 2 * c2;
                if (gy >= 0 && gy < ny && gx >= 0 && gx < spitch)
                    pf[k] = *reinterpret_cast<const float4*>(src + (size_t)gy * spitch + gx);
            }
        }
    };
    auto store = [&](const rs_hdr* H) {
        if (!H->use_lds) return;
        const int n4 = (H->h.bw >> 1) * H->h.bh;
#pragma unroll
        for (int k = 0; k < RS_PF; ++k) {
            const int e = tid + 256 * k;
            if (e < n4)
                *reinterpret_cast<float4*>(tile + 2 * e) = pf[k];
        }
    };

    int t = blockIdx.x;
    if (t >= ntiles) return;
    if (KIND == ZM_RESAMPLE_LANCZOS3) {
        for (int e = tid; e < LZ_FLOATS / 4; e += 256)
            smem4[HDR_FLOATS / 4 + e] = reinterpret_cast<const float4*>(taptab)[e];
    }
    if (tid < 64) {
        rs_build_header<KIND>(lat, lnx, lny, t, ntx, nx, ny, lds_cap, &HR[0]);
        if (t + G < ntiles) rs_build_header<KIND>(lat, lnx, lny, t + G, ntx, nx, ny, lds_cap, &HR[1]);
    }
    __syncthreads();
    prefetch(&HR[0]);
    int slot = 0;
    for (; t < ntiles; t += G) {
        const rs_hdr* H = &HR[slot];
        const int nslot = slot == 2 ? 0 : slot + 1;
        const int nnslot = nslot == 2 ? 0 : nslot + 1;
        store(H);
        __syncthreads();
        const bool use_lds = H->use_lds, touches = H->touches;
        const int bx0 = H->h.bx0, by0 = H->h.by0, bw = H->h.bw, bh = H->h.bh;
        const int tyi = t / ntx, txi = t - tyi * ntx;
        const int ox0 = txi * TW, oy0 = tyi * RTH;
        const int tx = tid & 63, tyb = tid >> 6;
        const int ox = ox0 + tx;
        int32_t aprev[RTH / 4];
#pragma unroll
        for (int q = 0; q < RTH / 4; ++q) aprev[q] = -1;
        if (MASKOP == 2 && !mfirst) {
#pragma unroll
            for (int q = 0; q < RTH / 4; ++q) {
                const int oy = oy0 + tyb + 4 * q;
                if (ox < onx && oy < ony) aprev[q] = macc[(size_t)oy * onx + ox];
            }
        }
        if (t + G < ntiles) prefetch(&HR[nslot]);
        if (tid < 64 && t + 2 * G < ntiles)
            rs_build_header<KIND>(lat, lnx, lny, t + 2 * G, ntx, nx, ny, lds_cap, &HR[nnslot]);

        float xr[3], yr[3];
// ... 96 lines not shown
                                }
                            }
                        }
                        acc = fmaf(tw[r].y, ra, acc);
                        vacc = fmaf(tw[r].y, rv, vacc);
                        p += spitch;
                    }
                }
                if (MASKOP != 2 && pair_scale != 0.f) {
                    bool bada = false, badb = false;
                    if (!(__builtin_isfinite(acc) && __builtin_isfinite(vacc))) {
                        if (use_lds) {
                            const float2* p = tile + (iyr + OFF) * bw + (ixr + OFF);
                            zm_v2f av = (zm_v2f){0.f, 0.f};
#pragma unroll
                            for (int r = 0; r < NT; ++r) {
                                float2 s[NT];
                                lds_row<NT>::read(p, s);
                                zm_v2f rv2 = (zm_v2f){0.f, 0.f};
#pragma unroll
                                for (int c = 0; c < NT; ++c) {
                                    const bool nz = tw[c].x != 0.f && tw[r].y != 0.f;
                                    const bool fa = __builtin_isfinite(s[c].x), fb = __builtin_isfinite(s[c].y);
                                    bada = bada || (nz && !fa);
                                    badb = badb || (nz && !fb);
                                    rv2 = __builtin_elementwise_fma((zm_v2f){tw[c].x, tw[c].x},
                                                                    (zm_v2f){fa ? s[c].x : 0.f, fb ? s[c].y : 0.f}, rv2);
                                }
                                av = __builtin_elementwise_fma((zm_v2f){tw[r].y, tw[r].y}, rv2, av);
                                p += bw;
                            }
                            acc = av.x;
                            vacc = av.y;
                        } else {
                            const float2* p = src + (size_t)iy * spitch + ix;
                            acc = 0.f;
                            vacc = 0.f;
                            for (int r = 0; r < NT; ++r) {
                                float ra = 0.f, rv = 0.f;
                                if (tw[r].y != 0.f) {
                                    for (int c = 0; c < NT; ++c) {
                                        if (tw[c].x != 0.f) {
                                            const float2 s = p[c];
                                            const bool fa = __builtin_isfinite(s.x), fb = __builtin_isfinite(s.y);
                                            bada = bada || !fa;
                                            badb = badb || !fb;
                                            ra = fmaf(tw[c].x, fa ? s.x : 0.f, ra);
                                            rv = fmaf(tw[c].x, fb ? s.y : 0.f, rv);
                                        }
                                    }
                                }
                                acc = fmaf(tw[r].y, ra, acc);
                                vacc = fmaf(tw[r].y, rv, vacc);
                                p += spitch;
                            }
                        }
                    }
                    res.x = bada ? 0.f : acc * fscale;
                    res.y = badb ? 0.f : vacc * pair_scale;
                } else if (vacc > 0.f && vacc < ZM_BADVAR_TEST) {
                    res.x = acc * fscale;
                    res.y = __builtin_amdgcn_rcpf(vacc * fscale2);
                }
                if (MASKOP && !(ddx || ddy)) {
                    if (m16 != ZM_BOX_RAW) {
                        mres = (int32_t)m16;
                    } else {
                        for (int r = 0; r < NT; ++r) {
                            const int32_t* mp = mask + (size_t)(iy + r) * nx + ix;
                            for (int c = 0; c < NT; ++c) mres |= mp[c];
                        }
                    }
                }
            }
            const size_t oidx = (size_t)oy * onx + ox;
            if (plane_a) {
                plane_a[oidx] = res.x;
                plane_b[oidx] = res.y;
            } else {
                dst[oidx] = res;
            }
            if (MASKOP == 1) {
                macc[oidx] = mres;
            } else if (MASKOP == 2) {
                int32_t a = aprev[0];
#pragma unroll
                for (int k = 1; k < RTH / 4; ++k) a = (q == k) ? aprev[k] : a;
                if (inb) {
                    if (a == -1) a = mres;
                    else a = (mkind == ZM_MASK_AND) ? (a & mres) : (a | mres);
                }
                macc[oidx] = a;
            }
        }
        __syncthreads();
        slot = nslot;
    }
}

__global__ __launch_bounds__(256) void k_resample_nearest(const float2* __restrict__ src, int nx,
                                                          int ny, int spitch,
                                                          const double2* __restrict__ lat,
                                                          int lnx, int lny, float fscale,
                                                          float2* __restrict__ dst, int onx,
                                                          int ony) {
    __shared__ tile_hdr hdr;
    const int tid = threadIdx.x;
    const int ox0 = blockIdx.x * TW, oy0 = blockIdx.y * TH;
    if (tid < 64) build_tile_header(lat, lnx, lny, ox0 / LSTEP, oy0 / LSTEP, 0, 0, &hdr);
    __syncthreads();
    const int tx = tid & 63, tyb = tid >> 6;
    const int ox = ox0 + tx;
    for (int q = 0; q < 4; ++q) {
        const int ty = tyb + 4 * q, oy = oy0 + ty;
        if (ox >= onx || oy >= ony) continue;
        float px, py;
        tile_position(&hdr, tx, ty, &px, &py);
        int ix = hdr.bx0 + (int)floorf(px + 0.5f), iy = hdr.by0 + (int)floorf(py + 0.5f);
        float2 res = make_float2(0.f, 0.f);
        if (ix >= 0 && ix < nx && iy >= 0 && iy < ny) {
            float2 s = src[(size_t)iy * spitch + ix];
            if (s.y > 0.f && s.y < ZM_BADVAR_TEST) {
                res.x = s.x * fscale;
                res.y = 1.f / (s.y * fscale * fscale);
            }
        }
        dst[(size_t)oy * onx + ox] = res;
    }
}

template <int KIND>
static int launch_resample_kind(zm_ctx* ctx, dim3 grd, size_t shmem, const float2* src, int nx, int ny,
                                int spitch, const double2* lat, int lnx, int lny, float fscale,
                                float2* dst, int onx, int ony, int lds_elems, const int32_t* mask,
                                int32_t* macc, int mop, int mkind, int mfirst, float* plane_a, float* plane_b,
                                float pair_scale) {
    dim3 blk(256, 1, 1);
    const int ntx = grd.x, ntiles = grd.x * grd.y;
    uint16_t* mbox = nullptr;
    if (mop) {
        constexpr int NT = taps_traits<KIND>::N;
        ZM_TRY(ctx->get("mask_box", sizeof(uint16_t) * (size_t)nx * ny, (void**)&mbox));
        if (ctx->box_ready_for != (const void*)mask || ctx->box_ready_nt != NT) {
            zm_scope_timer tb(ctx, "mask_box");
            hipLaunchKernelGGL(k_mask_box<NT>, dim3(zm_div_up(nx, 64), zm_div_up(ny, 16)), blk, 0, ctx->stream,
                               mask, nx, ny, mbox);
        }
        ctx->box_ready_for = nullptr;
    }
    const float* taptab = nullptr;
    if (KIND == ZM_RESAMPLE_LANCZOS3) {
        ZM_TRY(zm_get_lanczos_table(ctx, &taptab));
        shmem += sizeof(float) * LZ_FLOATS;
    }
    zm_scope_timer t(ctx, "resample");
    dim3 pgrd(std::min(ntiles, 256 * 4), 1, 1);
    if (mop == 0)
        hipLaunchKernelGGL((k_resample<KIND, 0>), pgrd, blk, shmem, ctx->stream, src, nx, ny, spitch, lat,
                           lnx, lny, fscale, dst, onx, ony, lds_elems, mask, mbox, macc, mkind, mfirst, ntx, ntiles, taptab, plane_a, plane_b, pair_scale);
    else if (mop == 1)
        hipLaunchKernelGGL((k_resample<KIND, 1>), pgrd, blk, shmem, ctx->stream, src, nx, ny, spitch, lat,
                           lnx, lny, fscale, dst, onx, ony, lds_elems, mask, mbox, macc, mkind, mfirst, ntx, ntiles, taptab, plane_a, plane_b, pair_scale);
    else
        hipLaunchKernelGGL((k_resample<KIND, 2>), pgrd, blk, shmem, ctx->stream, src, nx, ny, spitch, lat,
                           lnx, lny, fscale, dst, onx, ony, lds_elems, mask, mbox, macc, mkind, mfirst, ntx, ntiles, taptab, plane_a, plane_b, pair_scale);
    ZM_HIP(hipGetLastError());
    return 0;
}

int zm_launch_resample(zm_ctx* ctx, const float2* src, int nx, int ny, int spitch,
                       const double2* lat, int lnx, int lny, int kernel, float fscale,
                       float2* dst, int onx, int ony, int lds_elems, const int32_t* mask,
                       int32_t* macc, int mop, int mkind, int mfirst, float* plane_a, float* plane_b, float pair_scale) {
    dim3 blk(256, 1, 1), grd(zm_div_up(onx, TW), zm_div_up(ony, TH), 1);
    ZM_CHECK(pair_scale == 0.f || (kernel != ZM_RESAMPLE_NEAREST && plane_a && plane_b && ctx->edge == ZM_EDGE_ZERO && mop != 2),
             "zm_launch_resample: a pair of images takes LANCZOS3 / BILINEAR, two output planes, the default edge rule and no mask accumulation");
    dim3 rgrd(zm_div_up(onx, TW), zm_div_up(ony, RTH), 1);
    if (!mask || !macc) mop = 0;
    if (lds_elems > RS_PFCAP) lds_elems = RS_PFCAP;
    size_t shmem = (size_t)HDR_FLOATS * 4 + (size_t)lds_elems * sizeof(float2);
    if (kernel == ZM_RESAMPLE_LANCZOS3 || kernel == ZM_RESAMPLE_BILINEAR) {
        const bool lz = mop && ctx->mask_resample == ZM_MASKRES_LANCZOS_ROUND, trunc = ctx->edge == ZM_EDGE_TRUNCATE;
        const int mop_img = lz ? 0 : mop;
        if (kernel == ZM_RESAMPLE_LANCZOS3)
            ZM_TRY(launch_resample_kind<ZM_RESAMPLE_LANCZOS3>(ctx, rgrd, shmem, src, nx, ny, spitch, lat, lnx,
                                                              lny, fscale, dst, onx, ony, lds_elems, mask,
                                                              macc, mop_img, mkind, mfirst, plane_a, plane_b, pair_scale));
        else
            ZM_TRY(launch_resample_kind<ZM_RESAMPLE_BILINEAR>(ctx, rgrd, shmem, src, nx, ny, spitch, lat, lnx,
                                                              lny, fscale, dst, onx, ony, lds_elems, mask,
                                                              macc, mop_img, mkind, mfirst, plane_a, plane_b, pair_scale));
        if (trunc)
            ZM_TRY(zm_launch_resample_rim(ctx, src, nx, ny, spitch, lat, lnx, lny, kernel, fscale, dst, plane_a, plane_b, onx,
                                          ony, mask, macc, mop_img, mkind));
        if (lz) {
            const int64_t opix = (int64_t)onx * ony;
            if (mop == 1) return zm_launch_resample_mask_opts(ctx, mask, nx, ny, lat, lnx, lny, kernel, macc, onx, ony, 0, 1, trunc);
            int32_t* tmp = nullptr;
            ZM_TRY(ctx->get("mask_tmp", sizeof(int32_t) * opix, (void**)&tmp));
            ZM_TRY(zm_launch_resample_mask_opts(ctx, mask, nx, ny, lat, lnx, lny, kernel, tmp, onx, ony, -1, 1, trunc));
            return zm_launch_mask_accum(ctx, macc, tmp, opix, mkind, mfirst);
        }
        return 0;
    }
    if (kernel == ZM_RESAMPLE_NEAREST) {
        zm_scope_timer t(ctx, "resample");
        hipLaunchKernelGGL(k_resample_nearest, grd, blk, 0, ctx->stream, src, nx, ny, spitch, lat, lnx,
                           lny, fscale, dst, onx, ony);
        ZM_HIP(hipGetLastError());
        if (plane_a) ZM_TRY(zm_launch_split_pairs(ctx, dst, (int64_t)onx * ony, plane_a, plane_b));
        if (mop) {
            int32_t* tmp = nullptr;
            const int64_t opix = (int64_t)onx * ony;
            if (mop == 1) return zm_launch_resample_mask(ctx, mask, nx, ny, lat, lnx, lny, kernel, macc,
                                                         onx, ony, 0);
            ZM_TRY(ctx->get("mask_tmp", sizeof(int32_t) * opix, (void**)&tmp));
            ZM_TRY(zm_launch_resample_mask(ctx, mask, nx, ny, lat, lnx, lny, kernel, tmp, onx, ony, -1));
            return zm_launch_mask_accum(ctx, macc, tmp, opix, mkind, mfirst);
        }
        return 0;
    }
    zm_set_error("zm_launch_resample: unknown kernel %d", kernel);
    return 2;
}

template <int KIND>
__global__ __launch_bounds__(256) void k_resample_mask(const int32_t* __restrict__ mask, int nx,
                                                       int ny, const double2* __restrict__ lat,
                                                       int lnx, int lny,
                                                       int32_t* __restrict__ dst, int onx,
                                                       int ony, int32_t fill) {
    __shared__ tile_hdr hdr;
    constexpr int NT = taps_traits<KIND>::N;
    constexpr int OFF = taps_traits<KIND>::OFF;
    const int tid = threadIdx.x;
    const int ox0 = blockIdx.x * TW, oy0 = blockIdx.y * TH;
    if (tid < 64) build_tile_header(lat, lnx, lny, ox0 / LSTEP, oy0 / LSTEP, OFF, OFF + NT - 1, &hdr);
    __syncthreads();
    const int tx = tid & 63, tyb = tid >> 6;
    const int ox = ox0 + tx;
    for (int q = 0; q < 4; ++q) {
        const int ty = tyb + 4 * q, oy = oy0 + ty;
        if (ox >= onx || oy >= ony) continue;
        float px, py;
        tile_position(&hdr, tx, ty, &px, &py);
        int ixr, iyr;
        float dx, dy;
        bool ddx, ddy;
        split_pos(px, &ixr, &dx, &ddx);
        split_pos(py, &iyr, &dy, &ddy);
        const int ix = hdr.bx0 + ixr + OFF, iy = hdr.by0 + iyr + OFF;
        int32_t m = fill;
        const bool inbx = ddx ? (ix - OFF >= 0 && ix - OFF < nx) : (ix >= 0 && ix + NT <= nx);
        const bool inby = ddy ? (iy - OFF >= 0 && iy - OFF < ny) : (iy >= 0 && iy + NT <= ny);
        if (inbx && inby) {
            m = 0;
            int c0 = ddx ? -OFF : 0, c1 = ddx ? -OFF + 1 : NT;
            int r0 = ddy ? -OFF : 0, r1 = ddy ? -OFF + 1 : NT;
            if (KIND == ZM_RESAMPLE_BILINEAR) {
                c0 = 0; c1 = ddx ? 1 : 2; r0 = 0; r1 = ddy ? 1 : 2;
            }
            for (int r = r0; r < r1; ++r) {
                const int32_t* p = mask + (size_t)(iy + r) * nx + ix;
                for (int c = c0; c < c1; ++c) m |= p[c];
            }
        }
        dst[(size_t)oy * onx + ox] = m;
    }
}

__global__ __launch_bounds__(256) void k_resample_mask_nearest(const int32_t* __restrict__ mask,
                                                               int nx, int ny,
                                                               const double2* __restrict__ lat,
                                                               int lnx, int lny,
// ... 47 lines not shown
```

zuds-pipeline_amd/csrc/select_bracket.hip:

```cpp
#include "select_dev.h"

#define RS2_THREADS 1024
#define RS2_WAVES 16
#define RS2_NK 4
#define RS2_SAMPLE4 RS2_THREADS
#define RS2_SBINS 2048
#define RS2_GRID 256
#define RS2_BINS 256
#define RS2_SUB 40
#define RS2_LIST 8192
#define RS2_UNROLL 2
#define RS2_FAIL_MED 1u
#define RS2_FAIL_MAD 2u

struct rs2_state {
    uint32_t lo, span_m1, mul, fail;
    unsigned long long below, valid, count;
    float centre, median;
    double out[3];
    unsigned int hist[RS2_BINS];
    uint32_t kmin[RS2_BINS], kmax[RS2_BINS];
    uint32_t ovf[RS2_BINS / 32];
};

// ... 91 lines not shown
    if (cnt && uniform) atomicAdd(&L.lh[first], cnt);
    else if (cnt) {
#pragma unroll
        for (int j = 0; j < RS2_NK; ++j)
            if ((vm >> j) & 1u) {
                const uint32_t k = key[j];
                if (k >= lo && k - lo <= span_m1) atomicAdd(&L.lh[(k - lo) >> shift], 1u);
            }
    }
    __syncthreads();
    find_ranks_2048<unsigned int>(L.lh, r0, r1, L.wtot, L.res);
    const unsigned int b0 = L.res[0], e0 = L.res[1], b1 = L.res[2];
    const uint32_t new_lo = lo + (b0 << shift);
    const unsigned long long top = (unsigned long long)lo + (((unsigned long long)b1 + 1ull) << shift) - 1ull;
    const unsigned long long lim = (unsigned long long)lo + span_m1;
    const uint32_t hi = (uint32_t)(top < lim ? top : lim);
    r0 -= e0;
    r1 -= e0;
    span_m1 = hi - new_lo;
    lo = new_lo;
    shift_used = shift;
    __syncthreads();
}

__device__ inline void bracket_from_sample(const uint32_t (&key)[RS2_NK], uint32_t vm, rs2_state* S, rs2_lds& L) {
    const int tid = threadIdx.x, lane = tid & 63, wave = tid >> 6;
    unsigned int nv = __popc(vm);
    uint32_t kmin = 0xffffffffu, kmax = 0u;
#pragma unroll
    for (int j = 0; j < RS2_NK; ++j)
        if ((vm >> j) & 1u) { kmin = min(kmin, key[j]); kmax = max(kmax, key[j]); }
#pragma unroll
    for (int o = 32; o; o >>= 1) {
        nv += __shfl_xor(nv, o);
        kmin = min(kmin, (uint32_t)__shfl_xor(kmin, o));
        kmax = max(kmax, (uint32_t)__shfl_xor(kmax, o));
    }
    if (lane == 0) { L.red[0][wave] = nv; L.red[1][wave] = kmin; L.red[2][wave] = kmax; }
    __syncthreads();
    nv = 0; kmin = 0xffffffffu; kmax = 0u;
#pragma unroll
    for (int w = 0; w < RS2_WAVES; ++w) {
        nv += L.red[0][w];
        kmin = min(kmin, L.red[1][w]);
        kmax = max(kmax, L.red[2][w]);
    }
    __syncthreads();
    uint32_t lo = 0u, hi = 0xffffffffu;
    if (nv > 0) {
        const float half = 0.5f * (float)(nv - 1), d = 2.75f * sqrtf((float)nv) + 1.f;
        const unsigned int rl = (unsigned int)fmaxf(0.f, floorf(half - d));
        const unsigned int rh = (unsigned int)fminf((float)(nv - 1), ceilf(half + d));
        uint32_t rlo = kmin, span_m1 = kmax - kmin;
        unsigned int r0 = rl, r1 = rh;
        int sh = 0;
        narrow_sample(key, vm, rlo, span_m1, r0, r1, sh, L);
        if (sh > 0) narrow_sample(key, vm, rlo, span_m1, r0, r1, sh, L);
        lo = rlo;
        hi = rlo + span_m1;
        if (rl == 0) lo = 0u;
        if (rh == nv - 1) hi = 0xffffffffu;
    }
    for (int k = tid; k < RS2_BINS; k += RS2_THREADS) {
        S->hist[k] = 0;
        S->kmin[k] = 0xffffffffu;
        S->kmax[k] = 0u;
    }
    if (tid < RS2_BINS / 32) S->ovf[tid] = 0;
    if (tid == 0) {
        S->lo = lo;
        S->span_m1 = hi - lo;
        S->mul = (hi - lo) < (uint32_t)RS2_BINS ? 0u
                                                : (uint32_t)(((unsigned long long)RS2_BINS << 32) / ((unsigned long long)(hi - lo) + 1ull));
        S->below = 0;
        S->valid = 0;
    }
}

__global__ __launch_bounds__(RS2_THREADS) void k_rsel2_sample(const rs_batch B, rs2_state* __restrict__ st,
                                                              float* __restrict__ samp) {
    __shared__ rs2_lds L;
    const int im = blockIdx.x, tid = threadIdx.x;
    const float4* __restrict__ img = reinterpret_cast<const float4*>(B.im[im].img);
    const int4* __restrict__ mask = reinterpret_cast<const int4*>(B.im[im].mask);
    float4* __restrict__ sp = reinterpret_cast<float4*>(samp) + (size_t)im * RS2_SAMPLE4;
    const int64_t stride = (B.n / 4) / RS2_SAMPLE4;
    const int64_t q = rs2_sample_pos(tid, stride);
    const float4 v = img[q];
    const int4 m = mask ? mask[q] : make_int4(0, 0, 0, 0);
    uint32_t key[RS2_NK];
    uint32_t vm = 0;
    const float qnan = __uint_as_float(0x7fc00000u);
    const float a[4] = {v.x, v.y, v.z, v.w};
    const int b[4] = {m.x, m.y, m.z, m.w};
    float o[4];
#pragma unroll
    for (int c = 0; c < 4; ++c) {
        const bool ok = b[c] == 0 && a[c] == a[c];
        key[c] = f2key(a[c]);
        if (ok) vm |= 1u << c;
        o[c] = ok ? a[c] : qnan;
    }
    sp[tid] = make_float4(o[0], o[1], o[2], o[3]);
    rs2_state* S = st + im;
    if (tid == 0) {
        S->fail = 0;
        S->count = 0;
        S->centre = 0.f;
        S->median = 0.f;
        S->out[0] = S->out[1] = S->out[2] = 0.0;
    }
    bracket_from_sample(key, vm, S, L);
}

template <int VMODE, int MODE>
__global__ __launch_bounds__(RS2_THREADS) __attribute__((amdgpu_waves_per_eu(8, 8)))
void k_rsel2_pass(const rs_batch B, rs2_state* __restrict__ st, uint32_t* __restrict__ seg,
                  unsigned int* __restrict__ wcnt, unsigned long long* __restrict__ vbits) {
    __shared__ unsigned int lh[RS2_BINS];
    __shared__ uint32_t lmin[RS2_BINS], lmax[RS2_BINS];
    __shared__ unsigned int red[2][RS2_WAVES];
    __shared__ __attribute__((aligned(16))) uint32_t stage[RS2_BINS * RS2_SUB];
    const int im = blockIdx.y, tid = threadIdx.x, lane = tid & 63, wave = tid >> 6;
    const float* __restrict__ img = B.im[im].img;
    const int32_t* __restrict__ mask = B.im[im].mask;
    rs2_state* S = st + im;
    const uint32_t lo = S->lo, span_m1 = S->span_m1, mul = S->mul;
    const float centre = S->centre;
    uint32_t* __restrict__ sg = seg + ((size_t)im * RS2_GRID + blockIdx.x) * (RS2_BINS * RS2_SUB);
    for (int k = tid; k < RS2_BINS; k += RS2_THREADS) { lh[k] = 0; lmin[k] = 0xffffffffu; lmax[k] = 0u; }
    __syncthreads();
    unsigned int nvalid = 0, nbelow = 0;
    auto group = [&](const float4 v, const unsigned long long (&ok)[4]) {
        const float a[4] = {v.x, v.y, v.z, v.w};
        uint32_t d[4];
        unsigned long long cm[4], anym = 0ull;
#pragma unroll
        for (int c = 0; c < 4; ++c) {
            const float x = MODE == 1 ? fabsf(a[c] - centre) : a[c];
            const uint32_t u = __float_as_uint(x);
            const uint32_t key = u ^ ((uint32_t)((int32_t)u >> 31) | 0x80000000u);
            nbelow += (unsigned int)__popcll(ok[c] & __builtin_amdgcn_ballot_w64(key < lo));
            d[c] = key - lo;
            cm[c] = ok[c] & __builtin_amdgcn_ballot_w64(d[c] <= span_m1);
            anym |= cm[c];
            nvalid += (unsigned int)__popcll(ok[c]);
        }
        if (anym) {
            unsigned int bin[4], slot[4];
#pragma unroll
            for (int c = 0; c < 4; ++c) {
                bin[c] = mul ? __umulhi(d[c], mul) : d[c];
                slot[c] = 0u;
                if (__builtin_amdgcn_inverse_ballot_w64(cm[c])) slot[c] = atomicAdd(&lh[bin[c]], 1u);
            }
            if (mul) {
#pragma unroll
                for (int c = 0; c < 4; ++c)
                    if (__builtin_amdgcn_inverse_ballot_w64(cm[c])) {
                        const uint32_t key = d[c] + lo;
                        if (slot[c] < RS2_SUB) stage[bin[c] * RS2_SUB + slot[c]] = key;
                        else { atomicMin(&lmin[bin[c]], key); atomicMax(&lmax[bin[c]], key); }
                    }
            }
        }
    };
    const int64_t n = B.n;
    const int64_t n4 = n / 4;
    const int64_t stride = (int64_t)gridDim.x * blockDim.x;
    unsigned long long* vb = VMODE ? vbits + (size_t)im * (size_t)((n4 + 63) / 64) * 4 : nullptr;
    const int64_t n4w = ((n4 + 63) / 64) * 64;
    auto load = [&](int64_t q0, float4 (&v)[RS2_UNROLL], int4 (&m)[RS2_UNROLL], uint32_t& xw) {
        xw = 0u;
        if (VMODE == 2) {
            const int64_t qu = q0 + (int64_t)(lane >> 3) * stride;
            if (lane < 8 * RS2_UNROLL && qu < n4w)
                xw = reinterpret_cast<const uint32_t*>(vb)[(qu >> 6) * 8 + (lane & 7)];
        }
#pragma unroll
        for (int u = 0; u < RS2_UNROLL; ++u) {
            const int64_t q = q0 + u * stride;
            v[u] = make_float4(0.f, 0.f, 0.f, 0.f);
            m[u] = make_int4(0, 0, 0, 0);
            if (q < n4) v[u] = reinterpret_cast<const float4*>(img)[q];
            if (VMODE != 2 && mask && q < n4) m[u] = reinterpret_cast<const int4*>(mask)[q];
        }
    };
    auto work = [&](int64_t q0, const float4 (&v)[RS2_UNROLL], const int4 (&m)[RS2_UNROLL], uint32_t xw) {
#pragma unroll
        for (int u = 0; u < RS2_UNROLL; ++u) {
            const int64_t q = q0 + u * stride;
            if (q >= n4w) break;
            unsigned long long w[4];
            if (VMODE == 2) {
#pragma unroll
                for (int c = 0; c < 4; ++c)
                    w[c] = ((unsigned long long)(uint32_t)__builtin_amdgcn_readlane((int)xw, 8 * u + 2 * c + 1) << 32) |
                           (unsigned long long)(uint32_t)__builtin_amdgcn_readlane((int)xw, 8 * u + 2 * c);
            } else {
                const unsigned long long inm = __builtin_amdgcn_ballot_w64(q < n4);
                w[0] = inm & __builtin_amdgcn_ballot_w64(m[u].x == 0) & __builtin_amdgcn_ballot_w64(v[u].x == v[u].x);
                w[1] = inm & __builtin_amdgcn_ballot_w64(m[u].y == 0) & __builtin_amdgcn_ballot_w64(v[u].y == v[u].y);
                w[2] = inm & __builtin_amdgcn_ballot_w64(m[u].z == 0) & __builtin_amdgcn_ballot_w64(v[u].z == v[u].z);
                w[3] = inm & __builtin_amdgcn_ballot_w64(m[u].w == 0) & __builtin_amdgcn_ballot_w64(v[u].w == v[u].w);
                if (VMODE == 1 && lane == 0) {
                    unsigned long long* wp = vb + (q >> 6) * 4;
                    wp[0] = w[0]; wp[1] = w[1]; wp[2] = w[2]; wp[3] = w[3];
                }
            }
            group(v[u], w);
        }
    };
    {
        float4 vA[RS2_UNROLL], vB[RS2_UNROLL];
        int4 mA[RS2_UNROLL], mB[RS2_UNROLL];
        uint32_t xA, xB;
        const int64_t step = RS2_UNROLL * stride;
        int64_t q = (int64_t)blockIdx.x * blockDim.x + tid;
        if (q < n4w) {
            load(q, vA, mA, xA);
            while (true) {
                const bool more = q + step < n4w;
                if (more) load(q + step, vB, mB, xB);
                work(q, vA, mA, xA);
                if (!more) break;
                q += step;
                const bool more2 = q + step < n4w;
                if (more2) load(q + step, vA, mA, xA);
                work(q, vB, mB, xB);
                if (!more2) break;
                q += step;
            }
        }
    }
    if (blockIdx.x == 0 && wave == 0 && (n & 3)) {
        const int64_t p = 4 * n4 + lane;
        const bool in = lane < (int)(n & 3);
        const float x = in ? img[p] : 0.f;
        const int mk = (in && mask) ? mask[p] : 0;
        unsigned long long ok[4] = {__builtin_amdgcn_ballot_w64(in && mk == 0 && x == x), 0ull, 0ull, 0ull};
        group(make_float4(x, 0.f, 0.f, 0.f), ok);
    }
    if (lane == 0) { red[0][wave] = nvalid; red[1][wave] = nbelow; }
    __syncthreads();
    if (tid == 0) {
        unsigned long long a = 0, b = 0;
        for (int w = 0; w < RS2_WAVES; ++w) { a += red[0][w]; b += red[1][w]; }
        if (a) atomicAdd(&S->valid, a);
        if (b) atomicAdd(&S->below, b);
    }
    unsigned int* __restrict__ wc = wcnt + ((size_t)im * RS2_GRID + blockIdx.x) * RS2_BINS;
    for (int k = tid; k < RS2_BINS; k += RS2_THREADS) {
        const unsigned int c = lh[k];
        wc[k] = c;
        if (c) {
            atomicAdd(&S->hist[k], c);
            if (mul && c > RS2_SUB) {
                uint32_t mn = lmin[k], mx = lmax[k];
                for (unsigned int i = 0; i < RS2_SUB; ++i) {
                    const uint32_t kk = stage[k * RS2_SUB + i];
                    mn = min(mn, kk);
                    mx = max(mx, kk);
                }
                atomicMin(&S->kmin[k], mn);
                atomicMax(&S->kmax[k], mx);
                atomicOr(&S->ovf[k >> 5], 1u << (k & 31));
            }
        }
    }
    if (mul) {
        uint4* __restrict__ o4 = reinterpret_cast<uint4*>(sg);
        const uint4* s4 = reinterpret_cast<const uint4*>(stage);
        for (int k = tid; k < RS2_BINS * RS2_SUB / 4; k += RS2_THREADS) o4[k] = s4[k];
    }
}

__device__ inline uint32_t select_in_list(const uint32_t* list, unsigned int m, uint32_t base, int rem,
                                          unsigned long long r, unsigned int* h256, unsigned long long* res) {
    const int tid = threadIdx.x;
    while (rem > 0) {
        const int nb = rem < 8 ? rem : 8, sh = rem - nb;
        for (int k = tid; k < RS2_BINS; k += RS2_THREADS) h256[k] = 0;
        if (tid == 0) { res[0] = 0; res[1] = 0; }
        __syncthreads();
        const uint32_t width_m1 = (rem >= 32) ? 0xffffffffu : ((1u << rem) - 1u);
        for (unsigned int i = tid; i < m; i += RS2_THREADS) {
            const uint32_t k = list[i];
            if (k >= base && k - base <= width_m1) atomicAdd(&h256[(k - base) >> sh], 1u);
        }
        __syncthreads();
        if (tid < 64) wave_find_256(h256, r, res);
        __syncthreads();
        base += (uint32_t)res[0] << sh;
        r -= res[1];
        rem = sh;
        __syncthreads();
    }
    return base;
}

struct rs2_rescue_lds {
    unsigned int lh[2][RS2_SBINS];
    unsigned long long wtot[RS2_WAVES];
    unsigned long long res[5];
};

__device__ inline float rescue_select(const float* __restrict__ img, const int32_t* __restrict__ mask, int64_t n,
                                      int mode, float centre, unsigned long long& count, rs2_rescue_lds& L) {
    const int tid = threadIdx.x;
    uint32_t prefix[2] = {0u, 0u}, pmask = 0u;
    unsigned long long k[2] = {0ull, 0ull};
    const int shifts[3] = {21, 10, 0}, bits[3] = {11, 11, 10};
    for (int pass = 0; pass < 3; ++pass) {
        const int shift = shifts[pass];
        const uint32_t bm = (1u << bits[pass]) - 1u;
        const bool two = prefix[1] != prefix[0];
        for (int q = tid; q < 2 * RS2_SBINS; q += RS2_THREADS) (&L.lh[0][0])[q] = 0;
        if (tid == 0) for (int q = 0; q < 5; ++q) L.res[q] = 0;
        __syncthreads();
        int cur = -1;
        unsigned int run = 0;
        for (int64_t p = tid; p < n; p += RS2_THREADS) {
            float v = img[p];
            if ((mask && mask[p] != 0) || !(v == v)) continue;
            if (mode == 1) v = fabsf(v - centre);
            const uint32_t key = f2key(v);
            const uint32_t hi = key & pmask;
            const int b = (int)((key >> shift) & bm);
            if (hi == prefix[0]) {
                if (b == cur) ++run;
                else {
                    if (run) atomicAdd(&L.lh[0][cur], run);
                    cur = b;
                    run = 1;
                }
            } else if (two && hi == prefix[1]) {
                atomicAdd(&L.lh[1][b], 1u);
            }
        }
        if (run) atomicAdd(&L.lh[0][cur], run);
        __syncthreads();
        if (pass == 0) {
            find_ranks_2048<unsigned long long>(L.lh[0], ~0ull, ~0ull, L.wtot, L.res);
            count = L.res[4];
            __syncthreads();
            if (count == 0) return 0.f;
            k[0] = (count - 1) / 2;
            k[1] = count / 2;
        }
        if (!two) {
            find_ranks_2048<unsigned long long>(L.lh[0], k[0], k[1], L.wtot, L.res);
            const unsigned long long b0 = L.res[0], e0 = L.res[1], b1 = L.res[2], e1 = L.res[3];
            __syncthreads();
            prefix[0] |= (uint32_t)b0 << shift;
            prefix[1] |= (uint32_t)b1 << shift;
            k[0] -= e0;
            k[1] -= e1;
        } else {
            find_ranks_2048<unsigned long long>(L.lh[0], k[0], ~0ull, L.wtot, L.res);
            const unsigned long long b0 = L.res[0], e0 = L.res[1];
            __syncthreads();
            find_ranks_2048<unsigned long long>(L.lh[1], k[1], ~0ull, L.wtot, L.res);
            const unsigned long long b1 = L.res[0], e1 = L.res[1];
            __syncthreads();
            prefix[0] |= (uint32_t)b0 << shift;
            prefix[1] |= (uint32_t)b1 << shift;
            k[0] -= e0;
            k[1] -= e1;
        }
        pmask |= bm << shift;
    }
    return 0.5f * (key2f_dev(prefix[0]) + key2f_dev(prefix[1]));
}

__global__ __launch_bounds__(RS2_THREADS) void k_rsel2_finish(int mode, const rs_batch B, rs2_state* __restrict__ st,
                                                              const uint32_t* __restrict__ seg,
                                                              const unsigned int* __restrict__ wcnt,
                                                              const float* __restrict__ samp, double* __restrict__ out) {
    __shared__ rs2_lds L;
    __shared__ rs2_rescue_lds R;
    __shared__ uint32_t lfail;
    __shared__ unsigned int h256[RS2_BINS];
    __shared__ uint32_t list[RS2_LIST];
    __shared__ unsigned int ln;
    __shared__ unsigned long long res[2][3];
    __shared__ unsigned long long res2[3];
    __shared__ int failed;
    const int im = blockIdx.x, tid = threadIdx.x;
    rs2_state* S = st + im;
    const uint32_t lo = S->lo, mul = S->mul;
    const unsigned long long below = S->below;
    const unsigned long long count = mode == 0 ? S->valid : S->count;
    const uint32_t failbit = mode ? RS2_FAIL_MAD : RS2_FAIL_MED;
    for (int k = tid; k < RS2_BINS; k += RS2_THREADS) h256[k] = S->hist[k];
    if (tid == 0) {
        failed = (S->fail & failbit) ? 1 : 0;
        for (int t = 0; t < 2; ++t) { res[t][0] = 0; res[t][1] = 0; res[t][2] = 0; }
    }
    __syncthreads();
    const unsigned long long k0 = count ? (count - 1) / 2 : 0, k1 = count ? count / 2 : 0;
    float med = 0.f;
    if (count > 0) {
        if (tid < 64) {
            wave_find_256(h256, k0 >= below ? k0 - below : ~0ull, res[0]);
            wave_find_256(h256, k1 >= below ? k1 - below : ~0ull, res[1]);
        }
        __syncthreads();
// ... 4 lines not shown
        int have = -1;
        unsigned int m = 0;
        uint32_t bmin = 0u, bmax = 0u;
        bool whole = false;
        for (int t = 0; t < 2 && !failed; ++t) {
            if (t == 1 && k1 == k0) { keyout[1] = keyout[0]; break; }
            const unsigned int b = (unsigned int)res[t][0];
            const unsigned long long r = (t ? k1 : k0) - below - res[t][1];
            if (mul == 0) { keyout[t] = lo + b; continue; }
            if ((int)b != have) {
                const bool over = (S->ovf[b >> 5] >> (b & 31)) & 1u;
                __syncthreads();
                if (tid == 0) ln = 0;
                __syncthreads();
                uint32_t mn = 0xffffffffu, mx = 0u;
                {
                    const int w = tid >> 2, part = tid & 3;
                    const uint32_t* __restrict__ sgb = seg + (((size_t)im * RS2_GRID + w) * RS2_BINS + b) * RS2_SUB;
                    unsigned int c = wcnt[((size_t)im * RS2_GRID + w) * RS2_BINS + b];
                    uint32_t first[4];
#pragma unroll
                    for (int j = 0; j < 4; ++j) first[j] = sgb[part + 4 * j];
                    c = c < RS2_SUB ? c : RS2_SUB;
                    auto take = [&](uint32_t kk) {
                        mn = min(mn, kk);
                        mx = max(mx, kk);
                        const unsigned int slot = atomicAdd(&ln, 1u);
                        if (slot < RS2_LIST) list[slot] = kk;
                    };
#pragma unroll
                    for (int j = 0; j < 4; ++j)
                        if ((unsigned int)(part + 4 * j) < c) take(first[j]);
                    for (unsigned int i = part + 16; i < c; i += 4) take(sgb[i]);
                }
#pragma unroll
                for (int o = 32; o; o >>= 1) {
                    mn = min(mn, (uint32_t)__shfl_xor(mn, o));
                    mx = max(mx, (uint32_t)__shfl_xor(mx, o));
                }
                if ((tid & 63) == 0) { L.red[1][tid >> 6] = mn; L.red[2][tid >> 6] = mx; }
                __syncthreads();
                mn = 0xffffffffu; mx = 0u;
#pragma unroll
                for (int w = 0; w < RS2_WAVES; ++w) { mn = min(mn, L.red[1][w]); mx = max(mx, L.red[2][w]); }
                if (over) { mn = min(mn, S->kmin[b]); mx = max(mx, S->kmax[b]); }
                m = ln;
                bmin = mn;
                bmax = mx;
                whole = !over && m <= RS2_LIST;
                have = (int)b;
                __syncthreads();
            }
            if (bmin == bmax) { keyout[t] = bmin; continue; }
            if (!whole) {
                __syncthreads();
                if (tid == 0) failed = 1;
                __syncthreads();
                break;
            }
            keyout[t] = select_in_list(list, m, bmin, nbits(bmax - bmin), r, h256, res2);
        }
        if (!failed) med = 0.5f * (key2f_dev(keyout[0]) + key2f_dev(keyout[1]));
    }
    __syncthreads();
    if (tid == 0) {
        lfail = S->fail | (failed ? failbit : 0u);
        if (failed) atomicOr(&S->fail, failbit);
        if (mode == 0) {
            S->count = count;
            S->median = med;
            S->centre = med;
            S->out[0] = med;
            S->out[2] = (double)count;
        } else {
            S->out[1] = 1.4826 * (double)med;
        }
    }
    if (mode == 1) {
        __syncthreads();
        double o[3] = {S->out[0], 1.4826 * (double)med, S->out[2]};
        if (lfail) {
            unsigned long long cnt = S->count;
            float m0 = S->median;
            if (lfail & RS2_FAIL_MED) m0 = rescue_select(B.im[im].img, B.im[im].mask, B.n, 0, 0.f, cnt, R);
            __syncthreads();
            unsigned long long c2 = 0;
            const float mad = cnt ? rescue_select(B.im[im].img, B.im[im].mask, B.n, 1, m0, c2, R) : 0.f;
            o[0] = m0;
            o[1] = 1.4826 * (double)mad;
            o[2] = (double)cnt;
            if (tid == 0) {
                S->count = cnt;
                S->median = m0;
                S->out[0] = o[0]; S->out[1] = o[1]; S->out[2] = o[2];
            }
        }
        if (tid < 3) out[3 * im + tid] = o[tid];
        return;
    }
    const float4 v = (reinterpret_cast<const float4*>(samp) + (size_t)im * RS2_SAMPLE4)[tid];
    const float a[4] = {v.x, v.y, v.z, v.w};
    uint32_t key[RS2_NK];
    uint32_t vm = 0;
#pragma unroll
    for (int c = 0; c < 4; ++c) {
        if (a[c] == a[c]) vm |= 1u << c;
        key[c] = f2key(fabsf(a[c] - med));
    }
    __syncthreads();
    bracket_from_sample(key, vm, S, L);
}

int zm_rs2_median_mad(zm_ctx* ctx, int nimg, const rs_batch& B, unsigned long long* d_vbits, double* out_dev) {
    ZM_CHECK(nimg >= 1 && nimg <= ZM_RS_MAXIMG && B.n >= ZM_RS2_MIN_N, "zm_rs2_median_mad: shape");
    rs2_state* d_st = nullptr;
    float* d_samp = nullptr;
    uint32_t* d_seg = nullptr;
    unsigned int* d_wcnt = nullptr;
    ZM_TRY(ctx->get("rs2_state", sizeof(rs2_state) * ZM_RS_MAXIMG, (void**)&d_st));
    ZM_TRY(ctx->get("rs2_samp", sizeof(float) * 4 * RS2_SAMPLE4 * (size_t)nimg, (void**)&d_samp));
    ZM_TRY(ctx->get("rs2_seg", sizeof(uint32_t) * (size_t)RS2_SUB * RS2_BINS * RS2_GRID * (size_t)nimg, (void**)&d_seg));
    ZM_TRY(ctx->get("rs2_wcnt", sizeof(unsigned int) * (size_t)RS2_BINS * RS2_GRID * (size_t)nimg, (void**)&d_wcnt));
    const int grid = RS2_GRID;
    hipStream_t s = ctx->stream;
    hipLaunchKernelGGL(k_rsel2_sample, dim3(nimg), dim3(RS2_THREADS), 0, s, B, d_st, d_samp);
    if (d_vbits) hipLaunchKernelGGL((k_rsel2_pass<1, 0>), dim3(grid, nimg), dim3(RS2_THREADS), 0, s, B, d_st, d_seg, d_wcnt, d_vbits);
    else hipLaunchKernelGGL((k_rsel2_pass<0, 0>), dim3(grid, nimg), dim3(RS2_THREADS), 0, s, B, d_st, d_seg, d_wcnt, d_vbits);
    hipLaunchKernelGGL(k_rsel2_finish, dim3(nimg), dim3(RS2_THREADS), 0, s, 0, B, d_st, d_seg, d_wcnt, d_samp, out_dev);
    if (d_vbits) hipLaunchKernelGGL((k_rsel2_pass<2, 1>), dim3(grid, nimg), dim3(RS2_THREADS), 0, s, B, d_st, d_seg, d_wcnt, d_vbits);
    else hipLaunchKernelGGL((k_rsel2_pass<0, 1>), dim3(grid, nimg), dim3(RS2_THREADS), 0, s, B, d_st, d_seg, d_wcnt, d_vbits);
    hipLaunchKernelGGL(k_rsel2_finish, dim3(nimg), dim3(RS2_THREADS), 0, s, 1, B, d_st, d_seg, d_wcnt, d_samp, out_dev);
    ZM_HIP(hipGetLastError());
    return 0;
}
```

zuds-pipeline_amd/csrc/select_dev.h:

```cpp
#pragma once
#include "zm_internal.h"

#define ZM_RS_MAXIMG 4

__device__ inline uint32_t f2key(float f) {
    uint32_t u = __float_as_uint(f);
    return (u & 0x80000000u) ? ~u : (u | 0x80000000u);
}

__device__ inline float key2f_dev(uint32_t k) {
    uint32_t u = (k & 0x80000000u) ? (k & 0x7fffffffu) : ~k;
    return __uint_as_float(u);
}

struct rs_image {
    const float* img;
    const int32_t* mask;
};

struct rs_batch {
    rs_image im[ZM_RS_MAXIMG];
    int64_t n;
};

#define ZM_RS2_MIN_N (1 << 20)
int zm_rs2_median_mad(zm_ctx* ctx, int nimg, const rs_batch& B, unsigned long long* d_vbits, double* out_dev);
```

zuds-pipeline_amd/csrc/zm_internal.h:

```cpp
#pragma once
#include <hip/hip_runtime.h>
#include <cstdint>
#include <cstdio>
#include <cstring>
#include <map>
#include <string>
#include <vector>
#include <stdexcept>

#include "../../include/zudsmi.h"

#define ZM_BIGVAR 1e30f
#define ZM_BADVAR_TEST 1e14f
#define ZM_SNAP 1e-5f

void zm_set_error(const char* fmt, ...);

#ifdef ZM_DEV
#define ZM_DEVENV(name) getenv(name)
#define ZM_DEV_BUILD 1
#else
#define ZM_DEVENV(name) ((const char*)nullptr)
#define ZM_DEV_BUILD 0
#endif
// ... 83 lines not shown
struct zm_map_params {
    zm_wcs wout;
    zm_wcs win;
    double rot[9];
};

void zm_wcs_frame(const zm_wcs* w, double fr[9]);
void zm_make_map(const zm_wcs* wout, const zm_wcs* win, zm_map_params* mp);
void zm_map_point(const zm_map_params* mp, double xo, double yo, double* xi, double* yi);
double zm_pixel_area(const zm_wcs* w, double x, double y);

int zm_launch_lattice(zm_ctx* ctx, const zm_map_params* mp, int lnx, int lny, double2* lat_dev);
int zm_launch_lattice_batch(zm_ctx* ctx, const zm_map_params* mp_host, int n, int lnx, int lny,
                            double2* lat_dev, hipEvent_t after = nullptr);
int zm_launch_prep(zm_ctx* ctx, const float* img, const float* wgt, int nx, int ny,
                   const float* bknodes, int nbx, int nby, int mesh,
                   const float* var_scale_dev, float wthresh, float2* dst, int spitch,
                   const int32_t* mask_for_box = nullptr, int box_nt = 0, uint16_t* mbox_out = nullptr,
                   int mbox_pitch = 0);
struct zm_ff {
    const float* img;
    const float* wgt;
    const float4* ytab;
    const float4* xtab;
    const float* vscale;
    const float2* src;
    const double2* lat;
    const void* mask;
    const uint16_t* mbox;
    const float* bk;
    const int* mboxflag;
    int nx, ny, spitch, nbx, nby, ytp;
    float invmesh, wthresh, fscale, fscale2;
    int vec_ok, mpitch;
    int mask16, pad_;
};
struct zm_bkrows {
    const float* bk;
    float4* out;
    int nbx, nby, ny, ytp;
    float invmesh;
    int nx;
    float4* xout;
};
struct zm_boxjob {
    const void* m;
    uint16_t* B;
    int* rawflag;
    int nx, ny, pitch, is16;
};
void zm_fused_geometry(int* tile_h, int* lds_cap);
int zm_launch_fused_prepass(zm_ctx* ctx, const zm_bkrows* rows, int nrows);
int zm_launch_mask_boxes(zm_ctx* ctx, const zm_boxjob* boxes, int nboxes, hipEvent_t after, hipEvent_t* joined,
                         hipEvent_t after2 = nullptr);
int zm_launch_fused_headers_early(zm_ctx* ctx, const zm_ff* frames_host, int nfr, int lnx, int lny, int onx, int ony,
                                  int lds_elems, bool fits_own);
int zm_launch_coadd_fused(zm_ctx* ctx, const zm_ff* frames_host, int nfr, int lnx, int lny, int onx, int ony,
                          int lds_elems, int combine, int mask_kind, float* out_img, float* out_wgt,
                          int32_t* out_mask, float* out_cov, int partial, int32_t* unmasked_out,
                          float2* stack = nullptr, int64_t fstride = 0, bool fits_own = false);
int zm_get_lanczos_table(zm_ctx* ctx, const float** out);
int zm_check_wcs(const zm_wcs* w, const char* what);
int zm_resample_lds_plan(const zm_map_params* mp, int onx, int ony, int kernel);
int zm_frame_background(zm_ctx* ctx, const float* img, const float* wgt, int nx, int ny,
                        int mesh, int fsize, float wthresh, int mode0, int nmode,
                        float** nodes_dev, float** stats_dev, int* nbx_out, int* nby_out,
                        const char* slot, int index = 0, int count = 1);
int zm_batch_stats(zm_ctx* ctx, int nf, const float* const* imgs, const float* const* wgts, int nx,
                   int ny, int mesh, float wthresh, int mode0, int nmode, const char* slot, int index0,
                   int count, int nslot);
int zm_batch_filter(zm_ctx* ctx, int nf, int nx, int ny, int mesh, int fsize, int nmode,
                    const char* slot, int index0, int count, int nslot);
int zm_frame_products(zm_ctx* ctx, int nx, int ny, int mesh, const char* slot, int index, int count,
                      int nslot, float** nodes_dev, float** stats_dev, int* nbx_out, int* nby_out);
int zm_batch_var_scale(zm_ctx* ctx, int nf, const float* stats, float* out);
int zm_frame_stats(zm_ctx* ctx, const float* img, const float* wgt, int nx, int ny, int mesh,
                   float wthresh, int mode0, int nmode, const char* slot, int index, int count);
int zm_frame_filter(zm_ctx* ctx, int nx, int ny, int mesh, int fsize, int nmode, float** nodes_dev,
                    float** stats_dev, int* nbx_out, int* nby_out, const char* slot, int index,
                    int count);
int zm_get_sync_events(zm_ctx* ctx, int n, hipEvent_t** out);
hipStream_t zm_ctx_aux(zm_ctx* ctx);
int zm_launch_var_scale(zm_ctx* ctx, const float* bstats, const float* vstats, float* out);
int zm_launch_resample(zm_ctx* ctx, const float2* src, int nx, int ny, int spitch,
                       const double2* lat, int lnx, int lny, int kernel, float fscale,
                       float2* dst, int onx, int ony, int lds_elems, const int32_t* mask,
                       int32_t* macc, int mop, int mkind, int mfirst,
                       float* plane_a = nullptr, float* plane_b = nullptr, float pair_scale = 0.f);
int zm_launch_prep_pair(zm_ctx* ctx, const float* a, const float* b, int nx, int ny, float2* dst, int spitch);
int zm_launch_resample_mask(zm_ctx* ctx, const int32_t* mask, int nx, int ny,
                            const double2* lat, int lnx, int lny, int kernel,
                            int32_t* dst, int onx, int ony, int32_t fill);
int zm_launch_combine(zm_ctx* ctx, int n, const float2* stack, int64_t frame_stride,
                      int64_t npix, int kind, float clip_sigma, float clip_ampfrac,
                      float* out_img, float* out_wgt, int partial);
int zm_launch_resample_rim(zm_ctx* ctx, const float2* src, int nx, int ny, int spitch, const double2* lat, int lnx,
                           int lny, int kernel, float fscale, float2* dst, float* plane_a, float* plane_b, int onx,
                           int ony, const int32_t* mask, int32_t* macc, int mop, int mkind);
int zm_launch_resample_mask_opts(zm_ctx* ctx, const int32_t* mask, int nx, int ny, const double2* lat, int lnx, int lny,
                                 int kernel, int32_t* dst, int onx, int ony, int32_t fill, int lanczos, int trunc);
int zm_launch_mask_accum(zm_ctx* ctx, int32_t* acc, const int32_t* m, int64_t npix, int kind,
                         int first);
int zm_launch_mask_finalize(zm_ctx* ctx, int32_t* acc, float* cov, int64_t npix);
int zm_launch_split_pairs(zm_ctx* ctx, const float2* src, int64_t npix, float* a, float* b);
int zm_launch_mask_widen(zm_ctx* ctx, const int16_t* in, int64_t n, int32_t* out);
```

zuds-pipeline_amd/device.py:

```python
import ctypes as C
import os

import numpy as np

from . import _lib
from ._lib import check, wcs_struct
from .engine import coadd_params, get_engine


def _torch():
    import torch
    return torch


class DeviceFrames(object):

    def __init__(self, frames, device):
        torch = _torch()
        self.n = len(frames)
        self.tensors = []
        self.arr = (_lib.zm_dframe * self.n)()
        for i, f in enumerate(frames):
            img = self._dev(f['img'], torch.float32, device)
            wgt = self._dev(f.get('wgt'), torch.float32, device)
            m = f.get('mask')
            m16 = m is not None and (m.dtype == torch.int16 if isinstance(m, torch.Tensor) else np.asarray(m).dtype == np.int16)
            msk = self._dev(m, torch.int16 if m16 else torch.int32, device)
            self.tensors.append((img, wgt, msk))
            self.arr[i].img = img.data_ptr()
            self.arr[i].wgt = wgt.data_ptr() if wgt is not None else None
            self.arr[i].mask = msk.data_ptr() if msk is not None else None
            self.arr[i].mask_type = _lib.MASKTYPE_I16 if m16 else _lib.MASKTYPE_I32
            self.arr[i].wcs = wcs_struct(f['wcs'])
            self.arr[i].flxscale = float(f.get('flxscale', 1.0))

    @staticmethod
    def _dev(a, dtype, device):
        torch = _torch()
        if a is None:
            return None
        if isinstance(a, torch.Tensor):
            return a.to(device=device, dtype=dtype).contiguous()
        return torch.from_numpy(np.ascontiguousarray(a)).to(device=device, dtype=dtype)


class DeviceCoadd(object):

    def __init__(self, wout, params=None, device=0, engine=None, want_mask=False, stream=None):
        torch = _torch()
        self.torch = torch
        self.device = torch.device('cuda', device)
        self.engine = engine or get_engine(device)
        self.stream = stream if stream is not None else torch.cuda.Stream(self.device)
        self.engine.set_stream(self.stream.cuda_stream)
        self.params = params or coadd_params()
        self.wout = wcs_struct(wout)
        onx, ony = self.wout.naxis[0], self.wout.naxis[1]
        self.shape = (ony, onx)
        self._planes = torch.empty((2,) + self.shape, dtype=torch.float32, device=self.device)
        self.img, self.wgt = self._planes[0], self._planes[1]
        self.mask = self.mask_wgt = None
        if want_mask:
            self.mask = torch.empty(self.shape, dtype=torch.int32, device=self.device)
            self.mask_wgt = torch.empty(self.shape, dtype=torch.float32, device=self.device)

    def run(self, dframes, partial=False):
        L = self.engine.L
        self.engine.set_stream(self.stream.cuda_stream)
        self.stream.wait_stream(self.torch.cuda.current_stream(self.device))
        with self.torch.cuda.stream(self.stream):
            check(L.zm_coadd_dev(self.engine.ctx, dframes.n, dframes.arr,
                                 C.byref(self.wout), C.byref(self.params),
                                 int(bool(partial)), self.img.data_ptr(),
                                 self.wgt.data_ptr(),
                                 self.mask.data_ptr() if self.mask is not None else None,
                                 self.mask_wgt.data_ptr() if self.mask_wgt is not None else None),
                  'zm_coadd_dev')
        return self.img, self.wgt

    def run_sharded_weighted(self, dframes, group=None):
        import torch.distributed as dist
        if self.params.combine not in (_lib.COMBINE['WEIGHTED'], _lib.COMBINE['AVERAGE']):
            raise ValueError('a sum-reduce coadd needs COMBINE_TYPE WEIGHTED or AVERAGE; '
                             'use run_sharded_exact for CLIPPED / MEDIAN')
        from .parallel import reduce_masks
        L, ctx = self.engine.L, self.engine.ctx
        self.run(dframes, partial=True)
        import os
        from . import parallel
        if os.environ.get('ZM_NATIVE_RCCL') == '1':
# ... 98 lines not shown
        self.result()
        ny, nx = self.shape
        kw = dict(params)
        if max_objects is not None:
            kw['max_objects'] = max_objects
        with torch.cuda.stream(self.stream):
            bad = ((self.submask & self.BAD_SUM) != 0).to(torch.uint8)
            segm = torch.empty(self.shape, dtype=torch.int32, device=self.device)
            tab, nfound = self.engine.extract_dev(self.diff.data_ptr(), self.noise.data_ptr(), bad.data_ptr(),
                                                  self.submask.data_ptr(), nx, ny,
                                                  wcs=self.wsci if wcs is None else wcs, segm=segm.data_ptr(), **kw)
        return tab, nfound, segm

    def candidates(self, seeing, wcs=None, max_objects=None, **extract_params):
        from .filterobjects import filter_table, pixel_cuts_dev
        tab, nfound, _ = self.extract(wcs=wcs, max_objects=max_objects, **extract_params)
        tab = tab[((tab['IMAFLAGS_ISO'] & self.BAD_SUM) == 0) & (tab['FLAGS_WEIGHT'] == 0)]
        self.engine.set_stream(self.stream.cuda_stream)
        with self.torch.cuda.stream(self.stream):
            pix = pixel_cuts_dev(self.engine, self.diff, self.noise, self.submask, tab['X_IMAGE'], tab['Y_IMAGE'],
                                 bad_bits=self.BAD_SUM)
        return filter_table(tab, float(seeing), pix), nfound

    def stamps(self, ra, dec, sci, ref, size=63, ref_flxscale=1.0, sci_flxscale=1.0, kernel='LANCZOS3'):
        self.result()
        fs = self.engine.flux_scale(self.wsci, self.wref, float(sci_flxscale))
        self.engine.set_stream(self.stream.cuda_stream)
        self.stream.wait_stream(self.torch.cuda.current_stream(self.device))
        planes = [dict(img=self.diff, wcs=self.wsci, fscale=fs), dict(img=sci.contiguous(), wcs=self.wsci, fscale=fs),
                  dict(img=ref.contiguous(), wcs=self.wref, on_grid=True)]
        return self.engine.stamps(planes, self.wref, ra, dec, size=size, kernel=kernel, stream=self.stream)

    def release_overlap(self):
        if self._bk_engine is not None:
            self._bk_stream.synchronize()
            self._bk_engine.close()
        self._bk_engine = self._bk_stream = None

    def job(self, scim, sci_rms, p):
        return _lib.zm_sub_job(scim.data_ptr(), sci_rms.data_ptr(), self.ref_al.data_ptr(),
                               self.refrms_al.data_ptr(), self.bpm.data_ptr(), C.pointer(p),
                               self.diff.data_ptr(), self.noise.data_ptr())

    def finish(self):
        return self.diff, self.noise, self.submask

    def prepare(self, sci, sci_rms, sci_mask, sci_wgt, ref, ref_rms, ref_mask, seeing,
                nreg_side=3, subtract_back=True, hotpants_kws=None, ref_flxscale=1.0,
                ref_rms_flxscale=None, sci_ready=None):
        from .engine import hp_params
        from .hotpants import job_params
        L, ctx = self.engine.L, self.engine.ctx
        ny, nx = self.shape
        LAN = _lib.RESAMPLE['LANCZOS3']
        fs = C.c_double()
        check(L.zm_flux_scale(C.byref(self.wref), C.byref(self.wsci), float(ref_flxscale),
                              C.byref(fs)), 'zm_flux_scale')
        fs_rms = C.c_double()
        check(L.zm_flux_scale(C.byref(self.wref), C.byref(self.wsci),
                              float(ref_flxscale if ref_rms_flxscale is None else ref_rms_flxscale),
                              C.byref(fs_rms)), 'zm_flux_scale')
        self.engine.set_stream(self.stream.cuda_stream)
        self.stream.wait_stream(self.torch.cuda.current_stream(self.device))
        side = self.overlap and subtract_back
        bk_done = None
        if side:
            if self._bk_engine is None:
                from .engine import Engine
                self._bk_stream = self.torch.cuda.Stream(self.device)
                self._bk_engine = Engine(self.device.index, stream=self._bk_stream.cuda_stream)
            e2 = self._bk_engine
            if sci_ready is None:
                self._bk_stream.wait_stream(self.stream)
            else:
                if sci_ready is not False:
                    self._bk_stream.wait_event(sci_ready)
                if self._last_done is not None:
                    self._bk_stream.wait_event(self._last_done)
            with self.torch.cuda.stream(self._bk_stream):
                check(L.zm_background_dev(e2.ctx, sci.data_ptr(), sci_wgt.data_ptr() if sci_wgt is not None else None,
                                          nx, ny, 128, 3, None, None, self.scibkgsub.data_ptr(), None), 'sci background')
                check(L.zm_add_scalar_dev(e2.ctx, self.scibkgsub.data_ptr(), self.BKG_VAL, self.n), 'pedestal')
                bk_done = self._bk_stream.record_event()
        with self.torch.cuda.stream(self.stream):
            if sci_mask.dtype == self.torch.int16:
                if getattr(self, '_scimask32', None) is None:
                    self._scimask32 = self.torch.empty(self.shape, dtype=self.torch.int32, device=self.device)
                check(L.zm_mask_widen_dev(ctx, sci_mask.data_ptr(), self.n, self._scimask32.data_ptr()),
                      'zm_mask_widen_dev')
                sci_mask = self._scimask32
            pair = os.environ.get('ZM_ALIGN_PAIR', '1') != '0' and int(self.engine.query('edge')) == 0 and \
                int(self.engine.query('mask_resample')) == 0
            if pair:
                check(L.zm_align_pair_dev(ctx, ref.data_ptr(), ref_rms.data_ptr(), ref_mask.data_ptr(),
                                          C.byref(self.wref), C.byref(self.wsci), LAN, fs.value, fs_rms.value,
                                          self.ref_al.data_ptr(), self.refrms_al.data_ptr(),
                                          self.refmask_al.data_ptr()), 'align ref + rms')
            else:
                check(L.zm_resample_dev(ctx, ref.data_ptr(), None, ref_mask.data_ptr(),
                                        C.byref(self.wref), C.byref(self.wsci), LAN, fs.value,
                                        self.ref_al.data_ptr(), self.ref_al_w.data_ptr(),
                                        self.refmask_al.data_ptr()), 'align ref')
            check(L.zm_mask_bad_dev(ctx, self.refmask_al.data_ptr(), sci_mask.data_ptr(),
                                    self.BAD_SUM, self.n, self.submask.data_ptr(),
                                    self.bpm.data_ptr()), 'submask')
            if subtract_back and not side:
                check(L.zm_background_dev(ctx, sci.data_ptr(),
                                          sci_wgt.data_ptr() if sci_wgt is not None else None,
                                          nx, ny, 128, 3, None, None, self.scibkgsub.data_ptr(),
                                          None), 'sci background')
                check(L.zm_add_scalar_dev(ctx, self.scibkgsub.data_ptr(), self.BKG_VAL, self.n),
                      'pedestal')
                scim = self.scibkgsub
            elif subtract_back:
                self.stream.wait_event(bk_done)
                scim = self.scibkgsub
            else:
                scim = sci
            if not pair:
                check(L.zm_resample_dev(ctx, ref_rms.data_ptr(), None, None, C.byref(self.wref),
                                        C.byref(self.wsci), LAN, fs_rms.value, self.refrms_al.data_ptr(),
                                        self.refrms_al_w.data_ptr(), None), 'align ref rms')
            kws = dict(hotpants_kws or {})
            user_limits = 'il' in kws or 'tl' in kws
            if os.environ.get('ZM_HOST_LIMITS') == '1' or user_limits:
                mm = (C.c_double * 4)()
                check(L.zm_median_mad2_dev(ctx, scim.data_ptr(), sci_mask.data_ptr(),
                                           self.ref_al.data_ptr(), self.refmask_al.data_ptr(),
                                           self.n, mm), 'sci / ref bkg')
                m1, s1, m2, s2 = (float(v) for v in mm)
                self._limits = dict(il=m1 - 10 * s1, tl=m2 - 10 * s2)
                p = hp_params(**job_params(seeing, nx, ny, nreg_side, self._limits['il'],
                                           self._limits['tl'], hotpants_kws))
            else:
                if getattr(self, '_lim_dev', None) is None:
                    self._lim_dev = self.torch.zeros(6, dtype=self.torch.float64, device=self.device)
                check(L.zm_median_mad2_async_dev(ctx, scim.data_ptr(), sci_mask.data_ptr(),
                                                 self.ref_al.data_ptr(), self.refmask_al.data_ptr(),
                                                 self.n, self._lim_dev.data_ptr()), 'sci / ref bkg')
                if getattr(self, '_lim_host', None) is None:
                    self._lim_host = self.torch.zeros(6, dtype=self.torch.float64).pin_memory()
                self._lim_host.copy_(self._lim_dev, non_blocking=True)
                self._limits = None
                p = hp_params(**job_params(seeing, nx, ny, nreg_side, 0.0, 0.0, hotpants_kws))
                p.limits_dev = self._lim_dev.data_ptr()
                p.limits_nsigma = 10.0
        p.flag_mask_dev = self.submask.data_ptr()
        p.flag_bit = 1 << 17
        self._sci_rms = sci_rms
        return scim, p

    @property
    def limits(self):
        if getattr(self, '_limits', None) is None:
            self.stream.synchronize()
            self.check_limits()
            m1, s1, _, m2, s2, _ = (float(v) for v in self._lim_host)
            self._limits = dict(il=m1 - 10 * s1, tl=m2 - 10 * s2)
        return self._limits

    def check_limits(self):
        if getattr(self, '_limits', None) is None and getattr(self, '_lim_host', None) is not None:
            if not (float(self._lim_host[2]) > 0 and float(self._lim_host[5]) > 0):
                raise _lib.ZMError('zm_median_mad2: every pixel is masked')


_KIND = {'f32': 0, 'i32': 1, 'u8': 2, 'i16': 3}


class FITSDeviceIO(object):

    def __init__(self, device=0, engine=None, stream=None):
        torch = _torch()
        self.torch = torch
        self.device = torch.device('cuda', device)
        self.engine = engine or get_engine(device)
        if stream is None:
            stream = torch.cuda.Stream(self.device)
            self.engine.set_stream(stream.cuda_stream)
        self.stream = stream
        self._pin = [None, None]
        self._busy = [None, None]
        self._turn = 0

    def _staging(self, nbytes):
        torch = self.torch
        k = self._turn
        self._turn ^= 1
        if self._busy[k] is not None:
            self._busy[k].synchronize()
        if self._pin[k] is None or self._pin[k].numel() < nbytes:
            self._pin[k] = torch.empty(int(nbytes * 1.1) + 4096, dtype=torch.uint8, pin_memory=True)
        return k, self._pin[k]

    def load(self, path, kind='f32'):
        from . import fits
        torch = self.torch
        hdr, _, off = fits.read_header(path)
        nbytes = abs(int(hdr['BITPIX'])) // 8 * int(np.prod([int(hdr[f'NAXIS{i}'])
                                                             for i in range(1, int(hdr['NAXIS']) + 1)]))
        k, pin = self._staging(nbytes)
        raw, hdr, _, info = fits.read_raw(path, out=pin.numpy())
        if kind == 'mask':
            kind = 'i16' if (info['bitpix'] == 16 and info['bscale'] == 1.0 and info['bzero'] == 0.0) else 'i32'
        dt = {'f32': torch.float32, 'i32': torch.int32, 'u8': torch.uint8, 'i16': torch.int16}[kind]
        out = torch.empty(info['shape'], dtype=dt, device=self.device)
        self.engine.set_stream(self.stream.cuda_stream)
        with torch.cuda.stream(self.stream):
            d_raw = pin[:info['nbytes']].to(self.device, non_blocking=True)
            ev = torch.cuda.Event()
            ev.record(self.stream)
            self._busy[k] = ev
            check(self.engine.L.zm_fits_decode_dev(self.engine.ctx, d_raw.data_ptr(), info['bitpix'],
                                                   info['bscale'], info['bzero'], info['count'],
                                                   _KIND[kind], out.data_ptr()), 'zm_fits_decode_dev')
            d_raw.record_stream(self.stream)
        return out, hdr

    def save(self, path, tensor, header=None, comments=None, bitpix=None):
        from . import fits
        torch = self.torch
        t = tensor.contiguous()
# ... 117 lines not shown
```

Before: 48790 Mpix/s.

## Fold submask into pair resample and move sci median/MAD to side stream

Reads int16 science masks directly in the median/MAD and mask-combine kernels instead of widening them to int32 first. Folds the ref-mask OR/bad-pixel map computation into the paired Lanczos resample launch. Moves the science-frame median/MAD estimate onto the background side stream so it overlaps with the ref alignment. This cuts a few full-frame passes and kernel launches in the subtraction front-end, at the cost of more kernel variants and extra cross-stream ordering. It only affects the single-science-frame subtract stage, which is a small part of the workload next to the 32-frame coadd.

```diff
diff --git a/include/zudsmi.h b/include/zudsmi.h
--- a/include/zudsmi.h
+++ b/include/zudsmi.h
@@ -148,6 +148,11 @@
                        double* out4);
 int zm_median_mad2_async_dev(zm_ctx* ctx, const float* img_a, const int32_t* mask_a,
                              const float* img_b, const int32_t* mask_b, int64_t n, double* out6_dev);
+int zm_median_mad2_typed_async_dev(zm_ctx* ctx, const float* img_a, const void* mask_a, int mask_type_a,
+                                   const float* img_b, const void* mask_b, int mask_type_b, int64_t n,
+                                   double* out6_dev);
+int zm_median_mad_async_dev(zm_ctx* ctx, const float* img, const void* mask, int mask_type, int64_t n,
+                            double* out3_dev);
 
 int zm_aperture_photometry(zm_ctx* ctx, const float* img, const float* rms,
                            const int32_t* mask, int nx, int ny, int npos,
@@ -236,6 +241,10 @@
 int zm_align_pair_dev(zm_ctx* ctx, const float* img_a, const float* img_b, const int32_t* mask,
                       const zm_wcs* win, const zm_wcs* wout, int kernel, double fscale_a, double fscale_b,
                       float* out_a, float* out_b, int32_t* out_mask);
+int zm_align_sub_dev(zm_ctx* ctx, const float* img_a, const float* img_b, const int32_t* mask,
+                     const zm_wcs* win, const zm_wcs* wout, int kernel, double fscale_a, double fscale_b,
+                     float* out_a, float* out_b, int32_t* out_mask, const void* sci_mask, int sci_mask_type,
+                     int32_t badsum, int32_t* out_or, uint8_t* out_bpm);
 int zm_resample_i16(zm_ctx* ctx, const float* img, const float* wgt,
                     const int16_t* mask, const zm_wcs* win, const zm_wcs* wout,
                     int kernel, double fscale, float* out_img, float* out_wgt,
@@ -254,6 +263,10 @@
                         int nx, int ny, float* out_wgt, uint8_t* out_bpm);
 int zm_mask_bad_dev(zm_ctx* ctx, const int32_t* a, const int32_t* b,
                     int32_t badsum, int64_t n, int32_t* out_or, uint8_t* out_bpm);
+int zm_mask_bad_typed_dev(zm_ctx* ctx, const int32_t* a, const void* b, int b_type,
+                          int32_t badsum, int64_t n, int32_t* out_or, uint8_t* out_bpm);
+int zm_dilate_cols2_dev(zm_ctx* ctx, const uint8_t* in1, const uint8_t* in2, int nx, int ny, int hw1, int hw2,
+                        int edge, uint8_t* out1, uint8_t* out2);
 int zm_mask_flag_dev(zm_ctx* ctx, int32_t* mask, const float* img, float value,
                      int32_t bit, int64_t n);
 int zm_add_scalar_dev(zm_ctx* ctx, float* img, float v, int64_t n);
diff --git a/zuds-pipeline_amd/_lib.py b/zuds-pipeline_amd/_lib.py
--- a/zuds-pipeline_amd/_lib.py
+++ b/zuds-pipeline_amd/_lib.py
@@ -157,6 +157,8 @@
                               _P, _P, _P]),
     'zm_align_pair_dev': (C.c_int, [_P, _P, _P, _P, C.POINTER(zm_wcs), C.POINTER(zm_wcs), C.c_int, C.c_double,
                                     C.c_double, _P, _P, _P]),
+    'zm_align_sub_dev': (C.c_int, [_P, _P, _P, _P, C.POINTER(zm_wcs), C.POINTER(zm_wcs), C.c_int, C.c_double,
+                                   C.c_double, _P, _P, _P, _P, C.c_int, C.c_int32, _P, _P]),
     'zm_resample_dev': (C.c_int, [_P, _P, _P, _P, C.POINTER(zm_wcs),
                                   C.POINTER(zm_wcs), C.c_int, C.c_double,
                                   _P, _P, _P]),
@@ -220,10 +222,14 @@
     'zm_comm_mask_plan': (C.c_int, [C.c_int, C.c_int, C.c_int, C.c_int, C.POINTER(zm_mask_plan)]),
     'zm_median_mad2_dev': (C.c_int, [_P, _P, _P, _P, _P, C.c_int64, C.POINTER(C.c_double)]),
     'zm_median_mad2_async_dev': (C.c_int, [_P, _P, _P, _P, _P, C.c_int64, _P]),
+    'zm_median_mad2_typed_async_dev': (C.c_int, [_P, _P, _P, C.c_int, _P, _P, C.c_int, C.c_int64, _P]),
+    'zm_median_mad_async_dev': (C.c_int, [_P, _P, _P, C.c_int, C.c_int64, _P]),
+    'zm_dilate_cols2_dev': (C.c_int, [_P, _P, _P, C.c_int, C.c_int, C.c_int, C.c_int, C.c_int, _P, _P]),
     'zm_rms_from_weight_dev': (C.c_int, [_P, _P, _P, C.c_int64, C.c_float, _P]),
     'zm_weight_from_rms_dev': (C.c_int, [_P, _P, _P, _P, C.c_float, C.c_int64, _P]),
     'zm_false_weight_dev': (C.c_int, [_P, _P, C.c_int, C.c_int32, C.c_int, C.c_int, C.c_int, _P, _P]),
     'zm_mask_bad_dev': (C.c_int, [_P, _P, _P, C.c_int32, C.c_int64, _P, _P]),
+    'zm_mask_bad_typed_dev': (C.c_int, [_P, _P, _P, C.c_int, C.c_int32, C.c_int64, _P, _P]),
     'zm_mask_flag_dev': (C.c_int, [_P, _P, _P, C.c_float, C.c_int32, C.c_int64]),
     'zm_add_scalar_dev': (C.c_int, [_P, _P, C.c_float, C.c_int64]),
     'zm_copy_probe_dev': (C.c_int, [_P, _P, _P, C.c_int64]),
diff --git a/zuds-pipeline_amd/csrc/api_coadd.hip b/zuds-pipeline_amd/csrc/api_coadd.hip
--- a/zuds-pipeline_amd/csrc/api_coadd.hip
+++ b/zuds-pipeline_amd/csrc/api_coadd.hip
@@ -478,9 +478,9 @@
     return 0;
 }
 
-extern "C" int zm_align_pair_dev(zm_ctx* ctx, const float* img_a, const float* img_b, const int32_t* mask,
-                                 const zm_wcs* win, const zm_wcs* wout, int kernel, double fscale_a, double fscale_b,
-                                 float* out_a, float* out_b, int32_t* out_mask) {
+static int align_pair(zm_ctx* ctx, const float* img_a, const float* img_b, const int32_t* mask,
+                      const zm_wcs* win, const zm_wcs* wout, int kernel, double fscale_a, double fscale_b,
+                      float* out_a, float* out_b, int32_t* out_mask, const zm_rs_fold* fold) {
     ZM_CHECK(ctx && img_a && img_b && win && wout && out_a && out_b, "zm_align_pair_dev: null argument");
     ZM_CHECK(!mask || out_mask, "zm_align_pair_dev: out_mask required");
     ZM_CHECK(kernel == ZM_RESAMPLE_LANCZOS3 || kernel == ZM_RESAMPLE_BILINEAR, "zm_align_pair_dev: LANCZOS3 or BILINEAR (got %d)", kernel);
@@ -503,7 +503,23 @@
     ZM_TRY(ctx->get("prep", sizeof(float2) * (size_t)spitch * ny, (void**)&src));
     ZM_TRY(zm_launch_prep_pair(ctx, img_a, img_b, nx, ny, src, spitch));
     return zm_launch_resample(ctx, src, nx, ny, spitch, lat, lnx, lny, kernel, (float)fscale_a, nullptr, onx, ony, lds,
-                              mask, out_mask, mask ? 1 : 0, 0, 1, out_a, out_b, (float)fscale_b);
+                              mask, out_mask, mask ? 1 : 0, 0, 1, out_a, out_b, (float)fscale_b, fold);
+}
+
+extern "C" int zm_align_pair_dev(zm_ctx* ctx, const float* img_a, const float* img_b, const int32_t* mask,
+                                 const zm_wcs* win, const zm_wcs* wout, int kernel, double fscale_a, double fscale_b,
+                                 float* out_a, float* out_b, int32_t* out_mask) {
+    return align_pair(ctx, img_a, img_b, mask, win, wout, kernel, fscale_a, fscale_b, out_a, out_b, out_mask, nullptr);
+}
+
+extern "C" int zm_align_sub_dev(zm_ctx* ctx, const float* img_a, const float* img_b, const int32_t* mask,
+                                const zm_wcs* win, const zm_wcs* wout, int kernel, double fscale_a, double fscale_b,
+                                float* out_a, float* out_b, int32_t* out_mask, const void* sci_mask, int sci_mask_type,
+                                int32_t badsum, int32_t* out_or, uint8_t* out_bpm) {
+    ZM_CHECK(mask && out_mask && out_or, "zm_align_sub_dev: mask, out_mask and out_or are required");
+    ZM_CHECK(sci_mask_type == ZM_MASKTYPE_I32 || sci_mask_type == ZM_MASKTYPE_I16, "zm_align_sub_dev: unknown mask type %d", sci_mask_type);
+    const zm_rs_fold fold = {sci_mask, out_or, out_bpm, badsum, sci_mask_type == ZM_MASKTYPE_I16};
+    return align_pair(ctx, img_a, img_b, mask, win, wout, kernel, fscale_a, fscale_b, out_a, out_b, out_mask, &fold);
 }
 
 extern "C" int zm_resample_i16_dev(zm_ctx* ctx, const float* img, const float* wgt, const int16_t* mask,
diff --git a/zuds-pipeline_amd/csrc/api_subtract.hip b/zuds-pipeline_amd/csrc/api_subtract.hip
--- a/zuds-pipeline_amd/csrc/api_subtract.hip
+++ b/zuds-pipeline_amd/csrc/api_subtract.hip
@@ -30,7 +30,8 @@
     __shared__ unsigned int lh[2][RS_BINS];
     const int im = blockIdx.y;
     const float* __restrict__ img = B.im[im].img;
-    const int32_t* __restrict__ mask = B.im[im].mask;
+    const void* __restrict__ mask = B.im[im].mask;
+    const int m16 = B.im[im].m16;
     const rs_state S = st[im];
     const bool two = S.prefix[1] != S.prefix[0];
     for (int k = threadIdx.x; k < nbins; k += blockDim.x) { lh[0][k] = 0; lh[1][k] = 0; }
@@ -72,7 +73,7 @@
             m.z = ((w[2] >> lane) & 1ull) ? 0 : 1;
             m.w = ((w[3] >> lane) & 1ull) ? 0 : 1;
         } else {
-            if (mask && in) m = reinterpret_cast<const int4*>(mask)[q];
+            if (mask && in) m = rs_mask4(mask, m16, q);
             if (!in) m = make_int4(1, 1, 1, 1);
             if (vb) {
                 const unsigned long long b0 = __ballot(m.x == 0 && v.x == v.x), b1 = __ballot(m.y == 0 && v.y == v.y);
@@ -86,7 +87,7 @@
         put(v.x, m.x); put(v.y, m.y); put(v.z, m.z); put(v.w, m.w);
     }
     for (int64_t p = 4 * n4 + (int64_t)blockIdx.x * blockDim.x + threadIdx.x; p < n; p += stride)
-        put(img[p], mask ? mask[p] : 0);
+        put(img[p], mask ? rs_mask1(mask, m16, p) : 0);
     if (run) atomicAdd(&lh[0][cur], run);
     __syncthreads();
     unsigned int* h = hist + (size_t)im * 2 * RS_BINS;
@@ -257,7 +258,7 @@
     ZM_CHECK(ctx && img && out_median && out_mad_sigma, "zm_median_mad_dev: null argument");
     ZM_CHECK(n > 0, "zm_median_mad_dev: empty image");
     ZM_HIP(hipSetDevice(ctx->device));
-    rs_image im = {img, mask};
+    rs_image im = {img, mask, 0};
     double o[3];
     ZM_TRY(median_mad_batch(ctx, 1, &im, n, o));
     ZM_CHECK(o[2] > 0, "zm_median_mad: every pixel is masked");
@@ -272,7 +273,7 @@
     ZM_CHECK(ctx && img_a && img_b && out4, "zm_median_mad2_dev: null argument");
     ZM_CHECK(n > 0, "zm_median_mad2_dev: empty image");
     ZM_HIP(hipSetDevice(ctx->device));
-    rs_image im[2] = {{img_a, mask_a}, {img_b, mask_b}};
+    rs_image im[2] = {{img_a, mask_a, 0}, {img_b, mask_b, 0}};
     double o[6];
     ZM_TRY(median_mad_batch(ctx, 2, im, n, o));
     ZM_CHECK(o[2] > 0 && o[5] > 0, "zm_median_mad2: every pixel is masked");
@@ -286,8 +287,30 @@
     ZM_CHECK(ctx && img_a && img_b && out6_dev, "zm_median_mad2_async_dev: null argument");
     ZM_CHECK(n > 0, "zm_median_mad2_async_dev: empty image");
     ZM_HIP(hipSetDevice(ctx->device));
-    rs_image im[2] = {{img_a, mask_a}, {img_b, mask_b}};
+    rs_image im[2] = {{img_a, mask_a, 0}, {img_b, mask_b, 0}};
     return median_mad_batch(ctx, 2, im, n, nullptr, out6_dev);
+}
+
+extern "C" int zm_median_mad2_typed_async_dev(zm_ctx* ctx, const float* img_a, const void* mask_a, int mask_type_a,
+                                              const float* img_b, const void* mask_b, int mask_type_b, int64_t n,
+                                              double* out6_dev) {
+    ZM_CHECK(ctx && img_a && img_b && out6_dev, "zm_median_mad2_typed_async_dev: null argument");
+    ZM_CHECK(n > 0, "zm_median_mad2_typed_async_dev: empty image");
+    ZM_CHECK((mask_type_a == ZM_MASKTYPE_I32 || mask_type_a == ZM_MASKTYPE_I16) &&
+             (mask_type_b == ZM_MASKTYPE_I32 || mask_type_b == ZM_MASKTYPE_I16), "zm_median_mad2_typed_async_dev: unknown mask type");
+    ZM_HIP(hipSetDevice(ctx->device));
+    rs_image im[2] = {{img_a, mask_a, mask_type_a == ZM_MASKTYPE_I16}, {img_b, mask_b, mask_type_b == ZM_MASKTYPE_I16}};
+    return median_mad_batch(ctx, 2, im, n, nullptr, out6_dev);
+}
+
+extern "C" int zm_median_mad_async_dev(zm_ctx* ctx, const float* img, const void* mask, int mask_type, int64_t n,
+                                       double* out3_dev) {
+    ZM_CHECK(ctx && img && out3_dev, "zm_median_mad_async_dev: null argument");
+    ZM_CHECK(n > 0, "zm_median_mad_async_dev: empty image");
+    ZM_CHECK(mask_type == ZM_MASKTYPE_I32 || mask_type == ZM_MASKTYPE_I16, "zm_median_mad_async_dev: unknown mask type %d", mask_type);
+    ZM_HIP(hipSetDevice(ctx->device));
+    rs_image im = {img, mask, mask_type == ZM_MASKTYPE_I16};
+    return median_mad_batch(ctx, 1, &im, n, nullptr, out3_dev);
 }
 
 extern "C" int zm_median_mad(zm_ctx* ctx, const float* img, const int32_t* mask, int64_t n,
diff --git a/zuds-pipeline_amd/csrc/elementwise.hip b/zuds-pipeline_amd/csrc/elementwise.hip
--- a/zuds-pipeline_amd/csrc/elementwise.hip
+++ b/zuds-pipeline_amd/csrc/elementwise.hip
@@ -48,12 +48,13 @@
     return 0;
 }
 
-__global__ void k_mask_bad(const int32_t* __restrict__ a, const int32_t* __restrict__ b,
+template <typename T>
+__global__ void k_mask_bad(const int32_t* __restrict__ a, const T* __restrict__ b,
                            int32_t badsum, int64_t n, int32_t* __restrict__ out_or,
                            uint8_t* __restrict__ out_bpm) {
     int64_t p = (int64_t)blockIdx.x * blockDim.x + threadIdx.x;
     if (p >= n) return;
-    int32_t m = a[p] | (b ? b[p] : 0);
+    int32_t m = a[p] | (b ? (int32_t)b[p] : 0);
     if (out_or) out_or[p] = m;
     if (out_bpm) out_bpm[p] = (m & badsum) != 0;
 }
@@ -93,7 +94,20 @@
                                int64_t n, int32_t* out_or, uint8_t* out_bpm) {
     ZM_CHECK(ctx && a && n > 0 && (out_or || out_bpm), "zm_mask_bad_dev: bad argument");
     ZM_HIP(hipSetDevice(ctx->device));
-    hipLaunchKernelGGL(k_mask_bad, EW_GRID(n), a, b, badsum, n, out_or, out_bpm);
+    hipLaunchKernelGGL(k_mask_bad<int32_t>, EW_GRID(n), a, b, badsum, n, out_or, out_bpm);
+    ZM_HIP(hipGetLastError());
+    return 0;
+}
+
+extern "C" int zm_mask_bad_typed_dev(zm_ctx* ctx, const int32_t* a, const void* b, int b_type, int32_t badsum,
+                                     int64_t n, int32_t* out_or, uint8_t* out_bpm) {
+    ZM_CHECK(ctx && a && n > 0 && (out_or || out_bpm), "zm_mask_bad_typed_dev: bad argument");
+    ZM_CHECK(b_type == ZM_MASKTYPE_I32 || b_type == ZM_MASKTYPE_I16, "zm_mask_bad_typed_dev: unknown mask type %d", b_type);
+    ZM_HIP(hipSetDevice(ctx->device));
+    if (b_type == ZM_MASKTYPE_I16)
+        hipLaunchKernelGGL(k_mask_bad<int16_t>, EW_GRID(n), a, (const int16_t*)b, badsum, n, out_or, out_bpm);
+    else
+        hipLaunchKernelGGL(k_mask_bad<int32_t>, EW_GRID(n), a, (const int32_t*)b, badsum, n, out_or, out_bpm);
     ZM_HIP(hipGetLastError());
     return 0;
 }
diff --git a/zuds-pipeline_amd/csrc/hotpants.hip b/zuds-pipeline_amd/csrc/hotpants.hip
--- a/zuds-pipeline_amd/csrc/hotpants.hip
+++ b/zuds-pipeline_amd/csrc/hotpants.hip
@@ -176,6 +176,111 @@
             for (int k = 0; k < 4; ++k) cnt[k] += nz(wa[u], k) - nz(ws[u], k);
         }
     }
+}
+
+__global__ __launch_bounds__(256) void k_hp_colany_x2(const uint8_t* __restrict__ in1, const uint8_t* __restrict__ in2,
+                                                      int nx, int ny, int hw1, int hw2, int edge,
+                                                      uint8_t* __restrict__ out1, uint8_t* __restrict__ out2) {
+    const int x = blockIdx.x * blockDim.x + threadIdx.x;
+    const int y0 = blockIdx.y * HP_COLSTRIP, y1 = min(y0 + HP_COLSTRIP, ny);
+    if (x >= nx) return;
+    int c1 = 0, c2 = 0;
+    for (int j = max(y0 - hw1, 0); j <= min(y0 + hw1, ny - 1); ++j) c1 += in1[(size_t)j * nx + x] ? 1 : 0;
+    for (int j = max(y0 - hw2, 0); j <= min(y0 + hw2, ny - 1); ++j) c2 += in2[(size_t)j * nx + x] ? 1 : 0;
+    for (int y = y0; y < y1; ++y) {
+        uint8_t v1 = c1 > 0, v2 = c2 > 0;
+        if (edge && (x < hw1 || x >= nx - hw1 || y < hw1 || y >= ny - hw1)) v1 = 1;
+        if (edge && (x < hw2 || x >= nx - hw2 || y < hw2 || y >= ny - hw2)) v2 = 1;
+        out1[(size_t)y * nx + x] = v1;
+        out2[(size_t)y * nx + x] = v2;
+        const int a1 = y + 1 + hw1, s1 = y - hw1, a2 = y + 1 + hw2, s2 = y - hw2;
+        if (a1 < ny) c1 += in1[(size_t)a1 * nx + x] ? 1 : 0;
+        if (s1 >= 0) c1 -= in1[(size_t)s1 * nx + x] ? 1 : 0;
+        if (a2 < ny) c2 += in2[(size_t)a2 * nx + x] ? 1 : 0;
+        if (s2 >= 0) c2 -= in2[(size_t)s2 * nx + x] ? 1 : 0;
+    }
+}
+
+__global__ __launch_bounds__(256) void k_hp_colany4_x2(const uint8_t* __restrict__ in1, const uint8_t* __restrict__ in2,
+                                                       int nx, int ny, int hw1, int hw2, int edge,
+                                                       uint8_t* __restrict__ out1, uint8_t* __restrict__ out2) {
+    const int x = (blockIdx.x * blockDim.x + threadIdx.x) * 4;
+    const int y0 = blockIdx.y * HP_COLSTRIP4, y1 = min(y0 + HP_COLSTRIP4, ny);
+    if (x >= nx) return;
+    const unsigned* p1 = reinterpret_cast<const unsigned*>(in1 + x);
+    const unsigned* p2 = reinterpret_cast<const unsigned*>(in2 + x);
+    const size_t pitch = (size_t)nx / 4;
+    auto nz = [](unsigned w, int k) -> int { return ((w >> (8 * k)) & 0xffu) ? 1 : 0; };
+    int c1[4] = {0, 0, 0, 0}, c2[4] = {0, 0, 0, 0};
+    auto window = [&](const unsigned* p, int hw, int (&cnt)[4]) {
+        const int j0 = max(y0 - hw, 0), j1 = min(y0 + hw, ny - 1);
+        for (int jb = j0; jb <= j1; jb += 8) {
+            unsigned w[8];
+#pragma unroll
+            for (int u = 0; u < 8; ++u) w[u] = (jb + u <= j1) ? p[(size_t)(jb + u) * pitch] : 0u;
+#pragma unroll
+            for (int u = 0; u < 8; ++u)
+#pragma unroll
+                for (int k = 0; k < 4; ++k) cnt[k] += nz(w[u], k);
+        }
+    };
+    window(p1, hw1, c1);
+    window(p2, hw2, c2);
+    for (int yb = y0; yb < y1; yb += 8) {
+        unsigned wa1[8], ws1[8], wa2[8], ws2[8];
+#pragma unroll
+        for (int u = 0; u < 8; ++u) {
+            const int a1 = yb + u + 1 + hw1, s1 = yb + u - hw1;
+            const int a2 = yb + u + 1 + hw2, s2 = yb + u - hw2;
+            wa1[u] = (a1 < ny) ? p1[(size_t)a1 * pitch] : 0u;
+            ws1[u] = (s1 >= 0) ? p1[(size_t)s1 * pitch] : 0u;
+            wa2[u] = (a2 < ny) ? p2[(size_t)a2 * pitch] : 0u;
+            ws2[u] = (s2 >= 0) ? p2[(size_t)s2 * pitch] : 0u;
+        }
+#pragma unroll
+        for (int u = 0; u < 8; ++u) {
+            const int y = yb + u;
+            if (y < y1) {
+                unsigned o1 = 0, o2 = 0;
+#pragma unroll
+                for (int k = 0; k < 4; ++k) {
+                    unsigned v1 = c1[k] > 0, v2 = c2[k] > 0;
+                    if (edge && (x + k < hw1 || x + k >= nx - hw1 || y < hw1 || y >= ny - hw1)) v1 = 1;
+                    if (edge && (x + k < hw2 || x + k >= nx - hw2 || y < hw2 || y >= ny - hw2)) v2 = 1;
+                    o1 |= v1 << (8 * k);
+                    o2 |= v2 << (8 * k);
+                }
+                *reinterpret_cast<unsigned*>(out1 + (size_t)y * nx + x) = o1;
+                *reinterpret_cast<unsigned*>(out2 + (size_t)y * nx + x) = o2;
+            }
+#pragma unroll
+            for (int k = 0; k < 4; ++k) {
+                c1[k] += nz(wa1[u], k) - nz(ws1[u], k);
+                c2[k] += nz(wa2[u], k) - nz(ws2[u], k);
+            }
+        }
+    }
+}
+
+static int hp_launch_colany_x2(zm_ctx* ctx, const uint8_t* in1, const uint8_t* in2, int nx, int ny, int hw1, int hw2,
+                               int edge, uint8_t* out1, uint8_t* out2) {
+    const bool col4 = (nx % 4 == 0) && (((uintptr_t)in1 | (uintptr_t)in2 | (uintptr_t)out1 | (uintptr_t)out2) & 3) == 0;
+    if (col4)
+        hipLaunchKernelGGL(k_hp_colany4_x2, dim3(zm_div_up(nx / 4, 256), zm_div_up(ny, HP_COLSTRIP4)), dim3(256), 0, ctx->stream,
+                           in1, in2, nx, ny, hw1, hw2, edge, out1, out2);
+    else
+        hipLaunchKernelGGL(k_hp_colany_x2, dim3(zm_div_up(nx, 256), zm_div_up(ny, HP_COLSTRIP)), dim3(256), 0, ctx->stream,
+                           in1, in2, nx, ny, hw1, hw2, edge, out1, out2);
+    ZM_HIP(hipGetLastError());
+    return 0;
+}
+
+extern "C" int zm_dilate_cols2_dev(zm_ctx* ctx, const uint8_t* in1, const uint8_t* in2, int nx, int ny, int hw1, int hw2,
+                                   int edge, uint8_t* out1, uint8_t* out2) {
+    ZM_CHECK(ctx && in1 && in2 && out1 && out2 && nx > 0 && ny > 0 && hw1 >= 0 && hw2 >= 0, "zm_dilate_cols2_dev: bad argument");
+    ZM_CHECK(in1 != out1 && in2 != out2 && in1 != out2 && in2 != out1, "zm_dilate_cols2_dev: not in place");
+    ZM_HIP(hipSetDevice(ctx->device));
+    return hp_launch_colany_x2(ctx, in1, in2, nx, ny, hw1, hw2, edge, out1, out2);
 }
 
 __global__ __launch_bounds__(256) void k_hp_cells(const hp_plan P, const float* __restrict__ ref,
@@ -2477,7 +2582,10 @@
     if (!split && (((uintptr_t)tmp8b & 3) == 0)) {
         hipLaunchKernelGGL(k_hp_valid_rows, dim3(ny), b256, rsh, st, sci, ref, bpm, nx, ny, (float)P.il, (float)P.iu,
                            (float)P.tl, (float)P.tu, hp->limits_dev, hp->limits_nsigma, P.hw, P.hwk, bad, tmp8, tmp8b);
-        if (col4) {
+        static const bool front_old = getenv("ZM_SUB_FRONT") && getenv("ZM_SUB_FRONT")[0] == '0';
+        if (!front_old) {
+            ZM_TRY(hp_launch_colany_x2(ctx, tmp8, tmp8b, nx, ny, P.hw, P.hwk, 1, dirty, outbad));
+        } else if (col4) {
             hipLaunchKernelGGL(k_hp_colany4, gc4, b256, 0, st, tmp8, nx, ny, P.hw, 1, dirty);
             hipLaunchKernelGGL(k_hp_colany4, gc4, b256, 0, st, tmp8b, nx, ny, P.hwk, 1, outbad);
         } else {
diff --git a/zuds-pipeline_amd/csrc/resample.hip b/zuds-pipeline_amd/csrc/resample.hip
--- a/zuds-pipeline_amd/csrc/resample.hip
+++ b/zuds-pipeline_amd/csrc/resample.hip
@@ -289,7 +289,7 @@
     int lnx, int lny, float fscale, float2* __restrict__ dst, int onx, int ony, int lds_cap,
     const int32_t* __restrict__ mask, const uint16_t* __restrict__ mbox, int32_t* __restrict__ macc,
     int mkind, int mfirst, int ntx, int ntiles, const float* __restrict__ taptab,
-    float* __restrict__ plane_a, float* __restrict__ plane_b, float pair_scale) {
+    float* __restrict__ plane_a, float* __restrict__ plane_b, float pair_scale, const zm_rs_fold fold) {
     extern __shared__ float4 smem4[];
     rs_hdr* HR = reinterpret_cast<rs_hdr*>(smem4);
     constexpr int TABF = (KIND == ZM_RESAMPLE_LANCZOS3) ? LZ_FLOATS : 0;
@@ -552,6 +552,14 @@
             }
             if (MASKOP == 1) {
                 macc[oidx] = mres;
+                if (fold.out_or) {
+                    int32_t m = mres;
+                    if (fold.smask)
+                        m |= fold.s16 ? (int32_t)reinterpret_cast<const int16_t*>(fold.smask)[oidx]
+                                      : reinterpret_cast<const int32_t*>(fold.smask)[oidx];
+                    fold.out_or[oidx] = m;
+                    if (fold.out_bpm) fold.out_bpm[oidx] = (m & fold.badsum) != 0;
+                }
             } else if (MASKOP == 2) {
                 int32_t a = aprev[0];
 #pragma unroll
@@ -604,7 +612,7 @@
                                 int spitch, const double2* lat, int lnx, int lny, float fscale,
                                 float2* dst, int onx, int ony, int lds_elems, const int32_t* mask,
                                 int32_t* macc, int mop, int mkind, int mfirst, float* plane_a, float* plane_b,
-                                float pair_scale) {
+                                float pair_scale, const zm_rs_fold& fold) {
     dim3 blk(256, 1, 1);
     const int ntx = grd.x, ntiles = grd.x * grd.y;
     uint16_t* mbox = nullptr;
@@ -627,13 +635,13 @@
     dim3 pgrd(std::min(ntiles, 256 * 4), 1, 1);
     if (mop == 0)
         hipLaunchKernelGGL((k_resample<KIND, 0>), pgrd, blk, shmem, ctx->stream, src, nx, ny, spitch, lat,
-                           lnx, lny, fscale, dst, onx, ony, lds_elems, mask, mbox, macc, mkind, mfirst, ntx, ntiles, taptab, plane_a, plane_b, pair_scale);
+                           lnx, lny, fscale, dst, onx, ony, lds_elems, mask, mbox, macc, mkind, mfirst, ntx, ntiles, taptab, plane_a, plane_b, pair_scale, fold);
     else if (mop == 1)
         hipLaunchKernelGGL((k_resample<KIND, 1>), pgrd, blk, shmem, ctx->stream, src, nx, ny, spitch, lat,
-                           lnx, lny, fscale, dst, onx, ony, lds_elems, mask, mbox, macc, mkind, mfirst, ntx, ntiles, taptab, plane_a, plane_b, pair_scale);
+                           lnx, lny, fscale, dst, onx, ony, lds_elems, mask, mbox, macc, mkind, mfirst, ntx, ntiles, taptab, plane_a, plane_b, pair_scale, fold);
     else
         hipLaunchKernelGGL((k_resample<KIND, 2>), pgrd, blk, shmem, ctx->stream, src, nx, ny, spitch, lat,
-                           lnx, lny, fscale, dst, onx, ony, lds_elems, mask, mbox, macc, mkind, mfirst, ntx, ntiles, taptab, plane_a, plane_b, pair_scale);
+                           lnx, lny, fscale, dst, onx, ony, lds_elems, mask, mbox, macc, mkind, mfirst, ntx, ntiles, taptab, plane_a, plane_b, pair_scale, fold);
     ZM_HIP(hipGetLastError());
     return 0;
 }
@@ -641,8 +649,16 @@
 int zm_launch_resample(zm_ctx* ctx, const float2* src, int nx, int ny, int spitch,
                        const double2* lat, int lnx, int lny, int kernel, float fscale,
                        float2* dst, int onx, int ony, int lds_elems, const int32_t* mask,
-                       int32_t* macc, int mop, int mkind, int mfirst, float* plane_a, float* plane_b, float pair_scale) {
+                       int32_t* macc, int mop, int mkind, int mfirst, float* plane_a, float* plane_b, float pair_scale,
+                       const zm_rs_fold* fold_in) {
     dim3 blk(256, 1, 1), grd(zm_div_up(onx, TW), zm_div_up(ony, TH), 1);
+    zm_rs_fold fold = {nullptr, nullptr, nullptr, 0, 0};
+    if (fold_in) {
+        ZM_CHECK(mask && macc && mop == 1 && fold_in->out_or && kernel != ZM_RESAMPLE_NEAREST && ctx->edge == ZM_EDGE_ZERO &&
+                 ctx->mask_resample == ZM_MASKRES_OR,
+                 "zm_launch_resample: the bad-pixel fold takes a stored mask (mop 1), LANCZOS3 / BILINEAR and the default conventions");
+        fold = *fold_in;
+    }
     ZM_CHECK(pair_scale == 0.f || (kernel != ZM_RESAMPLE_NEAREST && plane_a && plane_b && ctx->edge == ZM_EDGE_ZERO && mop != 2),
              "zm_launch_resample: a pair of images takes LANCZOS3 / BILINEAR, two output planes, the default edge rule and no mask accumulation");
     dim3 rgrd(zm_div_up(onx, TW), zm_div_up(ony, RTH), 1);
@@ -655,11 +671,11 @@
         if (kernel == ZM_RESAMPLE_LANCZOS3)
             ZM_TRY(launch_resample_kind<ZM_RESAMPLE_LANCZOS3>(ctx, rgrd, shmem, src, nx, ny, spitch, lat, lnx,
                                                               lny, fscale, dst, onx, ony, lds_elems, mask,
-                                                              macc, mop_img, mkind, mfirst, plane_a, plane_b, pair_scale));
+                                                              macc, mop_img, mkind, mfirst, plane_a, plane_b, pair_scale, fold));
         else
             ZM_TRY(launch_resample_kind<ZM_RESAMPLE_BILINEAR>(ctx, rgrd, shmem, src, nx, ny, spitch, lat, lnx,
                                                               lny, fscale, dst, onx, ony, lds_elems, mask,
-                                                              macc, mop_img, mkind, mfirst, plane_a, plane_b, pair_scale));
+                                                              macc, mop_img, mkind, mfirst, plane_a, plane_b, pair_scale, fold));
         if (trunc)
             ZM_TRY(zm_launch_resample_rim(ctx, src, nx, ny, spitch, lat, lnx, lny, kernel, fscale, dst, plane_a, plane_b, onx,
                                           ony, mask, macc, mop_img, mkind));
diff --git a/zuds-pipeline_amd/csrc/select_bracket.hip b/zuds-pipeline_amd/csrc/select_bracket.hip
--- a/zuds-pipeline_amd/csrc/select_bracket.hip
+++ b/zuds-pipeline_amd/csrc/select_bracket.hip
@@ -197,12 +197,13 @@
     __shared__ rs2_lds L;
     const int im = blockIdx.x, tid = threadIdx.x;
     const float4* __restrict__ img = reinterpret_cast<const float4*>(B.im[im].img);
-    const int4* __restrict__ mask = reinterpret_cast<const int4*>(B.im[im].mask);
+    const void* __restrict__ mask = B.im[im].mask;
+    const int m16 = B.im[im].m16;
     float4* __restrict__ sp = reinterpret_cast<float4*>(samp) + (size_t)im * RS2_SAMPLE4;
     const int64_t stride = (B.n / 4) / RS2_SAMPLE4;
     const int64_t q = rs2_sample_pos(tid, stride);
     const float4 v = img[q];
-    const int4 m = mask ? mask[q] : make_int4(0, 0, 0, 0);
+    const int4 m = mask ? rs_mask4(mask, m16, q) : make_int4(0, 0, 0, 0);
     uint32_t key[RS2_NK];
     uint32_t vm = 0;
     const float qnan = __uint_as_float(0x7fc00000u);
@@ -238,7 +239,8 @@
     __shared__ __attribute__((aligned(16))) uint32_t stage[RS2_BINS * RS2_SUB];
     const int im = blockIdx.y, tid = threadIdx.x, lane = tid & 63, wave = tid >> 6;
     const float* __restrict__ img = B.im[im].img;
-    const int32_t* __restrict__ mask = B.im[im].mask;
+    const void* __restrict__ mask = B.im[im].mask;
+    const int m16 = B.im[im].m16;
     rs2_state* S = st + im;
     const uint32_t lo = S->lo, span_m1 = S->span_m1, mul = S->mul;
     const float centre = S->centre;
@@ -298,7 +300,7 @@
             v[u] = make_float4(0.f, 0.f, 0.f, 0.f);
             m[u] = make_int4(0, 0, 0, 0);
             if (q < n4) v[u] = reinterpret_cast<const float4*>(img)[q];
-            if (VMODE != 2 && mask && q < n4) m[u] = reinterpret_cast<const int4*>(mask)[q];
+            if (VMODE != 2 && mask && q < n4) m[u] = rs_mask4(mask, m16, q);
         }
     };
     auto work = [&](int64_t q0, const float4 (&v)[RS2_UNROLL], const int4 (&m)[RS2_UNROLL], uint32_t xw) {
@@ -352,7 +354,7 @@
         const int64_t p = 4 * n4 + lane;
         const bool in = lane < (int)(n & 3);
         const float x = in ? img[p] : 0.f;
-        const int mk = (in && mask) ? mask[p] : 0;
+        const int mk = (in && mask) ? rs_mask1(mask, m16, p) : 0;
         unsigned long long ok[4] = {__builtin_amdgcn_ballot_w64(in && mk == 0 && x == x), 0ull, 0ull, 0ull};
         group(make_float4(x, 0.f, 0.f, 0.f), ok);
     }
@@ -420,7 +422,7 @@
     unsigned long long res[5];
 };
 
-__device__ inline float rescue_select(const float* __restrict__ img, const int32_t* __restrict__ mask, int64_t n,
+__device__ inline float rescue_select(const float* __restrict__ img, const void* __restrict__ mask, int m16, int64_t n,
                                       int mode, float centre, unsigned long long& count, rs2_rescue_lds& L) {
     const int tid = threadIdx.x;
     uint32_t prefix[2] = {0u, 0u}, pmask = 0u;
@@ -437,7 +439,7 @@
         unsigned int run = 0;
         for (int64_t p = tid; p < n; p += RS2_THREADS) {
             float v = img[p];
-            if ((mask && mask[p] != 0) || !(v == v)) continue;
+            if ((mask && rs_mask1(mask, m16, p) != 0) || !(v == v)) continue;
             if (mode == 1) v = fabsf(v - centre);
             const uint32_t key = f2key(v);
             const uint32_t hi = key & pmask;
@@ -608,10 +610,10 @@
         if (lfail) {
             unsigned long long cnt = S->count;
             float m0 = S->median;
-            if (lfail & RS2_FAIL_MED) m0 = rescue_select(B.im[im].img, B.im[im].mask, B.n, 0, 0.f, cnt, R);
+            if (lfail & RS2_FAIL_MED) m0 = rescue_select(B.im[im].img, B.im[im].mask, B.im[im].m16, B.n, 0, 0.f, cnt, R);
             __syncthreads();
             unsigned long long c2 = 0;
-            const float mad = cnt ? rescue_select(B.im[im].img, B.im[im].mask, B.n, 1, m0, c2, R) : 0.f;
+            const float mad = cnt ? rescue_select(B.im[im].img, B.im[im].mask, B.im[im].m16, B.n, 1, m0, c2, R) : 0.f;
             o[0] = m0;
             o[1] = 1.4826 * (double)mad;
             o[2] = (double)cnt;
diff --git a/zuds-pipeline_amd/csrc/select_dev.h b/zuds-pipeline_amd/csrc/select_dev.h
--- a/zuds-pipeline_amd/csrc/select_dev.h
+++ b/zuds-pipeline_amd/csrc/select_dev.h
@@ -15,8 +15,20 @@
 
 struct rs_image {
     const float* img;
-    const int32_t* mask;
+    const void* mask;
+    int m16;
 };
+
+__device__ inline int4 rs_mask4(const void* mask, int m16, int64_t q) {
+    if (m16) {
+        const short4 v = reinterpret_cast<const short4*>(mask)[q];
+        return make_int4(v.x, v.y, v.z, v.w);
+    }
+    return reinterpret_cast<const int4*>(mask)[q];
+}
+__device__ inline int32_t rs_mask1(const void* mask, int m16, int64_t p) {
+    return m16 ? (int32_t)reinterpret_cast<const int16_t*>(mask)[p] : reinterpret_cast<const int32_t*>(mask)[p];
+}
 
 struct rs_batch {
     rs_image im[ZM_RS_MAXIMG];
diff --git a/zuds-pipeline_amd/csrc/zm_internal.h b/zuds-pipeline_amd/csrc/zm_internal.h
--- a/zuds-pipeline_amd/csrc/zm_internal.h
+++ b/zuds-pipeline_amd/csrc/zm_internal.h
@@ -189,11 +189,19 @@
 int zm_get_sync_events(zm_ctx* ctx, int n, hipEvent_t** out);
 hipStream_t zm_ctx_aux(zm_ctx* ctx);
 int zm_launch_var_scale(zm_ctx* ctx, const float* bstats, const float* vstats, float* out);
+struct zm_rs_fold {
+    const void* smask;
+    int32_t* out_or;
+    uint8_t* out_bpm;
+    int32_t badsum;
+    int s16;
+};
 int zm_launch_resample(zm_ctx* ctx, const float2* src, int nx, int ny, int spitch,
                        const double2* lat, int lnx, int lny, int kernel, float fscale,
                        float2* dst, int onx, int ony, int lds_elems, const int32_t* mask,
                        int32_t* macc, int mop, int mkind, int mfirst,
-                       float* plane_a = nullptr, float* plane_b = nullptr, float pair_scale = 0.f);
+                       float* plane_a = nullptr, float* plane_b = nullptr, float pair_scale = 0.f,
+                       const zm_rs_fold* fold = nullptr);
 int zm_launch_prep_pair(zm_ctx* ctx, const float* a, const float* b, int nx, int ny, float2* dst, int spitch);
 int zm_launch_resample_mask(zm_ctx* ctx, const int32_t* mask, int nx, int ny,
                             const double2* lat, int lnx, int lny, int kernel,
diff --git a/zuds-pipeline_amd/device.py b/zuds-pipeline_amd/device.py
--- a/zuds-pipeline_amd/device.py
+++ b/zuds-pipeline_amd/device.py
@@ -6,6 +6,9 @@
 from . import _lib
 from ._lib import check, wcs_struct
 from .engine import coadd_params, get_engine
+
+
+SUB_FRONT = os.environ.get('ZM_SUB_FRONT', '1') != '0'
 
 
 def _torch():
@@ -270,16 +273,35 @@
                                           nx, ny, 128, 3, None, None, self.scibkgsub.data_ptr(), None), 'sci background')
                 check(L.zm_add_scalar_dev(e2.ctx, self.scibkgsub.data_ptr(), self.BKG_VAL, self.n), 'pedestal')
                 bk_done = self._bk_stream.record_event()
+        front = SUB_FRONT
+        mtype = _lib.MASKTYPE_I16 if sci_mask.dtype == self.torch.int16 else _lib.MASKTYPE_I32
+        kws = dict(hotpants_kws or {})
+        host_limits = os.environ.get('ZM_HOST_LIMITS') == '1' or 'il' in kws or 'tl' in kws
+        if not host_limits and getattr(self, '_lim_dev', None) is None:
+            self._lim_dev = self.torch.zeros(6, dtype=self.torch.float64, device=self.device)
+        sci_side = front and side and sci_ready is not None and not host_limits
+        if sci_side:
+            with self.torch.cuda.stream(self._bk_stream):
+                check(L.zm_median_mad_async_dev(self._bk_engine.ctx, self.scibkgsub.data_ptr(), sci_mask.data_ptr(), mtype,
+                                                self.n, self._lim_dev.data_ptr()), 'sci bkg estimate')
+                bk_done = self._bk_stream.record_event()
         with self.torch.cuda.stream(self.stream):
-            if sci_mask.dtype == self.torch.int16:
+            if not front and sci_mask.dtype == self.torch.int16:
                 if getattr(self, '_scimask32', None) is None:
                     self._scimask32 = self.torch.empty(self.shape, dtype=self.torch.int32, device=self.device)
                 check(L.zm_mask_widen_dev(ctx, sci_mask.data_ptr(), self.n, self._scimask32.data_ptr()),
                       'zm_mask_widen_dev')
                 sci_mask = self._scimask32
+                mtype = _lib.MASKTYPE_I32
             pair = os.environ.get('ZM_ALIGN_PAIR', '1') != '0' and int(self.engine.query('edge')) == 0 and \
                 int(self.engine.query('mask_resample')) == 0
-            if pair:
+            if pair and front:
+                check(L.zm_align_sub_dev(ctx, ref.data_ptr(), ref_rms.data_ptr(), ref_mask.data_ptr(),
+                                         C.byref(self.wref), C.byref(self.wsci), LAN, fs.value, fs_rms.value,
+                                         self.ref_al.data_ptr(), self.refrms_al.data_ptr(),
+                                         self.refmask_al.data_ptr(), sci_mask.data_ptr(), mtype, self.BAD_SUM,
+                                         self.submask.data_ptr(), self.bpm.data_ptr()), 'align ref + rms + submask')
+            elif pair:
                 check(L.zm_align_pair_dev(ctx, ref.data_ptr(), ref_rms.data_ptr(), ref_mask.data_ptr(),
                                           C.byref(self.wref), C.byref(self.wsci), LAN, fs.value, fs_rms.value,
                                           self.ref_al.data_ptr(), self.refrms_al.data_ptr(),
@@ -289,9 +311,10 @@
                                         C.byref(self.wref), C.byref(self.wsci), LAN, fs.value,
                                         self.ref_al.data_ptr(), self.ref_al_w.data_ptr(),
                                         self.refmask_al.data_ptr()), 'align ref')
-            check(L.zm_mask_bad_dev(ctx, self.refmask_al.data_ptr(), sci_mask.data_ptr(),
-                                    self.BAD_SUM, self.n, self.submask.data_ptr(),
-                                    self.bpm.data_ptr()), 'submask')
+            if not (pair and front):
+                check(L.zm_mask_bad_typed_dev(ctx, self.refmask_al.data_ptr(), sci_mask.data_ptr(), mtype,
+                                              self.BAD_SUM, self.n, self.submask.data_ptr(),
+                                              self.bpm.data_ptr()), 'submask')
             if subtract_back and not side:
                 check(L.zm_background_dev(ctx, sci.data_ptr(),
                                           sci_wgt.data_ptr() if sci_wgt is not None else None,
@@ -309,10 +332,10 @@
                 check(L.zm_resample_dev(ctx, ref_rms.data_ptr(), None, None, C.byref(self.wref),
                                         C.byref(self.wsci), LAN, fs_rms.value, self.refrms_al.data_ptr(),
                                         self.refrms_al_w.data_ptr(), None), 'align ref rms')
-            kws = dict(hotpants_kws or {})
-            user_limits = 'il' in kws or 'tl' in kws
-            if os.environ.get('ZM_HOST_LIMITS') == '1' or user_limits:
+            if host_limits:
                 mm = (C.c_double * 4)()
+                if mtype == _lib.MASKTYPE_I16:
+                    sci_mask = sci_mask.to(self.torch.int32)
                 check(L.zm_median_mad2_dev(ctx, scim.data_ptr(), sci_mask.data_ptr(),
                                            self.ref_al.data_ptr(), self.refmask_al.data_ptr(),
                                            self.n, mm), 'sci / ref bkg')
@@ -321,11 +344,13 @@
                 p = hp_params(**job_params(seeing, nx, ny, nreg_side, self._limits['il'],
                                            self._limits['tl'], hotpants_kws))
             else:
-                if getattr(self, '_lim_dev', None) is None:
-                    self._lim_dev = self.torch.zeros(6, dtype=self.torch.float64, device=self.device)
-                check(L.zm_median_mad2_async_dev(ctx, scim.data_ptr(), sci_mask.data_ptr(),
-                                                 self.ref_al.data_ptr(), self.refmask_al.data_ptr(),
-                                                 self.n, self._lim_dev.data_ptr()), 'sci / ref bkg')
+                if sci_side:
+                    check(L.zm_median_mad_async_dev(ctx, self.ref_al.data_ptr(), self.refmask_al.data_ptr(),
+                                                    _lib.MASKTYPE_I32, self.n, self._lim_dev.data_ptr() + 24), 'ref bkg')
+                else:
+                    check(L.zm_median_mad2_typed_async_dev(ctx, scim.data_ptr(), sci_mask.data_ptr(), mtype,
+                                                           self.ref_al.data_ptr(), self.refmask_al.data_ptr(),
+                                                           _lib.MASKTYPE_I32, self.n, self._lim_dev.data_ptr()), 'sci / ref bkg')
                 if getattr(self, '_lim_host', None) is None:
                     self._lim_host = self.torch.zeros(6, dtype=self.torch.float64).pin_memory()
                 self._lim_host.copy_(self._lim_dev, non_blocking=True)
```

New measurement: 49060 Mpix/s, median of 6. Within noise of the previous version (+0.6%).
